# GDMCF/GDMCF

Measured on AMD Instinct MI355X. Metric: training users/sec, higher is better.
Workload: dtype f32; 1 GPU; yelp-shape synthetic rows, batch=400/GPU, dims=[1000], T=5, noise_scale=0.01, linear-var, mean_type=x0, reweight, AdamW lr=1e-5 (BASELINE configs[1]); n_items=34395, global_batch=400, parallelism=dp1, batch_rows=device CSR rows (CsrBatch)

## Files before the change

gdmcf_amd/_lib.py:

```python
import ctypes
import os
import re
from ctypes import c_char_p, c_double, c_float, c_int, c_int64, c_size_t, c_uint64, c_void_p

_HERE = os.path.dirname(os.path.abspath(__file__))
LIB_PATH = os.path.join(_HERE, "csrc", "libgdmcf_hip.so")
HEADER_PATH = os.path.normpath(os.path.join(_HERE, "..", "include", "gdmcf_hip.h"))

P = c_void_p
_CTYPES = {"int": c_int, "int64_t": c_int64, "uint64_t": c_uint64, "size_t": c_size_t, "float": c_float, "double": c_double}


def _uncomment(text):
    return re.sub(r"/\*.*?\*/", " ", text, flags=re.S)


def _code(text):
    return re.sub(r'^[ \t]*(#.*|extern\s+"C"\s*\{|\})[ \t]*$', "", _uncomment(text), flags=re.M)


def _ctype(ctype, where):
    words = re.sub(r"\bconst\b", " ", ctype).replace("*", " * ").split()
    if "*" in words:
        return c_char_p if words == ["char", "*"] else c_void_p
    if " ".join(words) not in _CTYPES:
        raise ImportError(f"gdmcf_hip.h: no ctypes type for '{' '.join(ctype.split())}' in the declaration of {where}")
    return _CTYPES[" ".join(words)]


def _declarator(decl, where):
    m = re.fullmatch(r"\s*(.*[\s*])(\w+)\s*", decl, flags=re.S)
    if not m:
        raise ImportError(f"gdmcf_hip.h: cannot read '{decl.strip()}' in the declaration of {where}")
    return m.groups()


def parse_functions(text):
    code = _code(text)
    out = {}
    for ret, name, params in re.findall(r"([\w\s*]+?)\b(gdmcf_\w+)\s*\(([^()]*)\)\s*;", code):
        params = [] if params.strip() in ("", "void") else params.split(",")
        out[name] = (_ctype(ret, name), [_ctype(_declarator(p, name)[0], name) for p in params])
    mentioned = re.findall(r"(gdmcf_\w+)\s*\(", code)
    if len(mentioned) != len(out):
        raise ImportError(f"gdmcf_hip.h: {len(mentioned)} gdmcf_*( but {len(out)} declarations read; unreadable: "
                          f"{sorted(set(mentioned) - set(out)) or 'none, a name is repeated'}")
    return out


def parse_constants(text):
    text = _uncomment(text)
    out = {n: int(v) for n, v in re.findall(r"^\s*#\s*define\s+(GDMCF_\w+)\s+\(?\s*(-?\d+)\s*\)?\s*$", text, flags=re.M)}
    for body in re.findall(r"\benum\s*\{([^}]*)\}", text):
        for member in filter(str.strip, body.split(",")):
            m = re.fullmatch(r"\s*(\w+)\s*=\s*(-?\d+)\s*", member)
            if not m:
                raise ImportError(f"gdmcf_hip.h: enum member '{member.strip()}' is not `NAME = integer`")
            out[m.group(1)] = int(m.group(2))
    return out


def parse_structs(text):
    out = {}
    for name, body in re.findall(r"\btypedef\s+struct\s+(\w+)\s*\{([^}]*)\}\s*\1\s*;", _code(text)):
        out[name] = []
        for line in filter(str.strip, body.split(";")):
            first, *more = line.split(",")
            ctype, member = _declarator(first, "struct " + name)
            if more and "*" in line:
                raise ImportError(f"gdmcf_hip.h: struct {name}: '{line.strip()}' must declare one pointer member per line")
            out[name] += [(m.strip(), _ctype(ctype, "struct " + name)) for m in [member] + more]
    return out


try:
    with open(HEADER_PATH) as _f:
        _HEADER = _f.read()
except OSError as e:
    raise ImportError(f"{HEADER_PATH} is missing: gdmcf_amd._lib derives its ctypes binding from the C header, which sits "
                      "beside the package in the source tree.") from e
_SIGNATURES = parse_functions(_HEADER)
EXPORTED_SYMBOLS = tuple(_SIGNATURES)
CONSTANTS = parse_constants(_HEADER)
GDMCF_OK, E_SHAPE, E_ARG, E_UNSUPPORTED, E_HIP, E_WORKSPACE, N_TABLES = (
    CONSTANTS["GDMCF_" + n] for n in ("OK", "E_SHAPE", "E_ARG", "E_UNSUPPORTED", "E_HIP", "E_WORKSPACE", "N_TABLES"))
TABLE_NAMES = (
    "betas", "alphas_cumprod", "alphas_cumprod_prev", "alphas_cumprod_next", "sqrt_alphas_cumprod",
    "sqrt_one_minus_alphas_cumprod", "log_one_minus_alphas_cumprod", "sqrt_recip_alphas_cumprod",
    "sqrt_recipm1_alphas_cumprod", "posterior_variance", "posterior_log_variance_clipped",
    "posterior_mean_coef1", "posterior_mean_coef2",
)


class GdDwAdamw(ctypes.Structure):
    _fields_ = parse_structs(_HEADER)["GdDwAdamw"]


class GdKnTail(ctypes.Structure):
    _fields_ = parse_structs(_HEADER)["GdKnTail"]


_lib = None


def load():
    global _lib
    if _lib is not None:
        return _lib
    if not os.path.exists(LIB_PATH):
        raise ImportError(
            f"{LIB_PATH} is missing: build it with `python -m gdmcf_amd.build` (hipcc, gfx950). "
            "gdmcf_amd has no CPU / PyTorch fallback.")
    lib = ctypes.CDLL(LIB_PATH)
    for name, (res, args) in _SIGNATURES.items():
        fn = getattr(lib, name)
        fn.restype = res
        fn.argtypes = args
    if lib.gdmcf_version() != 1:
        raise ImportError("libgdmcf_hip.so ABI version mismatch; rebuild with `python -m gdmcf_amd.build --force`")
    _lib = lib
    return lib


_EXC = {E_SHAPE: AssertionError, E_ARG: ValueError, E_UNSUPPORTED: NotImplementedError, E_HIP: RuntimeError,
        E_WORKSPACE: RuntimeError}


def check(rc):
    if rc != GDMCF_OK:
        msg = load().gdmcf_last_error().decode(errors="replace")
        raise _EXC.get(rc, RuntimeError)(msg or f"gdmcf error {rc}")


def ptr(t):
    return None if t is None else t.data_ptr()


def require_gpu(t, what):
    if not t.is_cuda:
        raise RuntimeError(f"gdmcf_amd: {what} must live on the MI355X (got device '{t.device}'); "
                           "the HIP path has no CPU fallback")


def shadow_info(data_ptr):
    p16 = ctypes.c_void_p()
    rows, cols, ld = ctypes.c_int64(), ctypes.c_int64(), ctypes.c_int64()
    if not load().gdmcf_bf16_shadow_info(data_ptr, ctypes.byref(p16), ctypes.byref(rows), ctypes.byref(cols), ctypes.byref(ld)):
        return None
    return int(p16.value), int(rows.value), int(cols.value), int(ld.value)


def stream_ptr():
    import torch
    return torch.cuda.current_stream().cuda_stream


def philox_randn(shape, device, seed, offset, stream_id=4, out=None):
    import torch
    rows, cols = int(shape[0]), int(shape[1])
    if out is None:
        out = torch.empty(rows, cols, dtype=torch.float32, device=device)
    require_gpu(out, "philox_randn output")
    check(load().gdmcf_randn_f32(out.data_ptr(), out.stride(0), rows, cols, int(stream_id), int(seed) & (2 ** 64 - 1),
                                 int(offset) & (2 ** 64 - 1), stream_ptr()))
    return out


def schedule_tables(kind, noise_scale, noise_min, noise_max, steps, beta_fixed=True):
    import numpy as np
    out = np.zeros((N_TABLES, steps), dtype=np.float64)
    rc = load().gdmcf_schedule_build(kind, float(noise_scale), float(noise_min), float(noise_max), int(steps),
                                     int(bool(beta_fixed)), out.ctypes.data_as(c_void_p))
    check(rc)
    return out


class Bf16Shadow:

    def __init__(self, t, sync=True):
        import weakref

        import torch
        require_gpu(t, "bf16 shadow source")
        if t.dim() != 2 or t.dtype != torch.float32 or t.stride(1) != 1:
            raise RuntimeError("gdmcf_amd: a bf16 shadow needs a 2-D float32 tensor with unit column stride")
        self.rows, self.cols = t.shape
        self.ptr = t.data_ptr()
        self.ld = t.stride(0)
        self.buf = torch.zeros((self.rows + 63) // 64 * 64, (self.cols + 63) // 64 * 64, dtype=torch.bfloat16,
                               device=t.device)
        self._lib = load()
        self._fin = weakref.finalize(self, self._lib.gdmcf_bf16_shadow_clear, self.ptr)
        self.register()
        if sync:
            self.sync()

    def register(self):
        check(self._lib.gdmcf_bf16_shadow_set(self.ptr, self.buf.data_ptr(), self.rows, self.cols, self.buf.stride(0)))

    def unregister(self):
        self._lib.gdmcf_bf16_shadow_clear(self.ptr)

    def sync(self):
        check(self._lib.gdmcf_bf16_shadow_sync(self.ptr, self.ld, stream_ptr()))

    def close(self):
        self._fin()
```

gdmcf_amd/csrc/gemm_dr_kn.hip:

```cpp
#include <stdlib.h>

#include "gemm_dr.h"
#include "tail_job.h"

namespace {

#ifndef GD_KN_EVERY
#define GD_KN_EVERY 4
#endif
template <int NL>
__global__ __launch_bounds__(256, 1) void dr_kn_kernel(const DrArgs d, const GdTailJob job) {
    constexpr int TMB = 5;
    const GdGemm& g = d.g;
    const int lane = threadIdx.x & 63;
    const int wave = __builtin_amdgcn_readfirstlane(threadIdx.x >> 6);
    const int r = lane & 15, q = lane >> 4;
    const int nblk = gridDim.x, per = nblk >> 3;
    const int slot = (nblk & 7) == 0 ? ((int)(blockIdx.x & 7) * per + (int)(blockIdx.x >> 3)) : (int)blockIdx.x;
    const int wl = slot * 4 + wave;
    const int n_waves = nblk * 4;
    const int ntiles = d.tiles_m * d.tiles_n;
    const int CPS = d.ksp;
    const int total_chunks = (g.K + 15) >> 4;
    const int ntasks = ntiles * g.splits;
    if (job.on && slot == (ntasks + 3) >> 2) {
        extern __shared__ __attribute__((aligned(16))) unsigned char kn_lds[];
        gd_tail_job_run(job, kn_lds);
        return;
    }
    const __amdgpu_buffer_rsrc_t srdA = __builtin_amdgcn_make_buffer_rsrc(const_cast<float*>(g.A), 0, (int)(((int64_t)(g.M - 1) * g.lda + g.K) * 4), 0x00020000);
    const __amdgpu_buffer_rsrc_t srdB = __builtin_amdgcn_make_buffer_rsrc(const_cast<float*>(g.B), 0, (int)(((int64_t)(g.K - 1) * g.ldb + g.N) * 4), 0x00020000);
    const uint32_t ldb16 = (uint32_t)g.ldb * 64u;
    for (int task = wl; task < ntasks; task += n_waves) {
        const int split = task / ntiles, tile = task - split * ntiles;
        const int tm = tile % d.tiles_m, tn = tile / d.tiles_m;
        const int m0 = tm * (16 * TMB), n0 = tn * (64 * NL);
        const int c_lo = split * CPS;
        uint32_t offA[TMB], offB[4][NL];
#pragma unroll
        for (int a = 0; a < TMB; ++a) offA[a] = (uint32_t)(((int64_t)min(m0 + 16 * a + r, g.M - 1) * g.lda + 4 * q) * 4);
#pragma unroll
        for (int s = 0; s < 4; ++s)
#pragma unroll
            for (int l = 0; l < NL; ++l) {
                const int n = n0 + 64 * l + 4 * r;
                offB[s][l] = n < g.N ? (uint32_t)(((int64_t)(4 * q + s) * g.ldb + n) * 4) : 0x80000000u;
            }
        f32x4 acc[TMB][NL][4];
#pragma unroll
        for (int a = 0; a < TMB; ++a)
#pragma unroll
            for (int l = 0; l < NL; ++l)
#pragma unroll
                for (int e = 0; e < 4; ++e) acc[a][l][e] = f32x4{0.f, 0.f, 0.f, 0.f};
        f32x4 xa[2][TMB], xb[2][4][NL];
        {
            const uint32_t ka = (uint32_t)c_lo * 64u, kb = (uint32_t)c_lo * ldb16;
#pragma unroll
            for (int a = 0; a < TMB; ++a) xa[0][a] = __builtin_bit_cast(f32x4, __builtin_amdgcn_raw_buffer_load_b128(srdA, offA[a], ka, 0));
#pragma unroll
            for (int s = 0; s < 4; ++s)
#pragma unroll
                for (int l = 0; l < NL; ++l)
                    xb[0][s][l] = __builtin_bit_cast(f32x4, __builtin_amdgcn_raw_buffer_load_b128(srdB, offB[s][l], kb, 0));
        }
#define GD_KN_CHUNK(PAR, c)                                                                                            \
        {                                                                                                              \
            const bool more = (c) + 1 < c_lo + CPS && (c) + 1 < total_chunks;                                          \
            const uint32_t ka = more ? (uint32_t)((c) + 1) * 64u : 0x80000000u;                                        \
            const uint32_t kb = more ? (uint32_t)((c) + 1) * ldb16 : 0x80000000u;                                      \
            if ((c) * 16 + 15 >= g.K) {  \
                _Pragma("unroll") for (int e = 0; e < 4; ++e) {                                                        \
                    const bool keep = (c) * 16 + 4 * q + e < g.K;                                                      \
                    _Pragma("unroll") for (int a = 0; a < TMB; ++a) xa[PAR][a][e] = keep ? xa[PAR][a][e] : 0.f;        \
                }                                                                                                      \
            }                                                                                                          \
                    \
            _Pragma("unroll") for (int a = 0; a < TMB; ++a) asm volatile("" : "+v"(xa[PAR][a]));                       \
            _Pragma("unroll") for (int s = 0; s < 4; ++s)                                                              \
                _Pragma("unroll") for (int l = 0; l < NL; ++l) asm volatile("" : "+v"(xb[PAR][s][l]));                 \
            __builtin_amdgcn_sched_barrier(0);                                                                         \
            _Pragma("unroll") for (int s = 0; s < 4; ++s) {                                                            \
                _Pragma("unroll") for (int n = 0; n < TMB * NL * 4; ++n) {                                             \
                    const int a = n / (NL * 4), l = (n / 4) % NL, e = n % 4;                                           \
                    acc[a][l][e] = __builtin_amdgcn_mfma_f32_16x16x4f32(xa[PAR][a][s], xb[PAR][s][l][e], acc[a][l][e], 0, 0, 0); \
                    const int idx = s * (TMB * NL * 4) + n;                                                            \
                    if (idx % GD_KN_EVERY == 2 && idx / GD_KN_EVERY < TMB + 4 * NL) {                                  \
                        const int ld = idx / GD_KN_EVERY;                                                              \
                        __builtin_amdgcn_sched_barrier(0);                                                             \
                        if (ld < TMB)                                                                                  \
                            xa[(PAR) ^ 1][ld] = __builtin_bit_cast(f32x4, __builtin_amdgcn_raw_buffer_load_b128(srdA, offA[ld], ka, 0)); \
                        else                                                                                           \
                            xb[(PAR) ^ 1][(ld - TMB) / NL][(ld - TMB) % NL] = __builtin_bit_cast(                      \
                                f32x4, __builtin_amdgcn_raw_buffer_load_b128(srdB, offB[(ld - TMB) / NL][(ld - TMB) % NL], kb, 0)); \
                        __builtin_amdgcn_sched_barrier(0);                                                             \
                    }                                                                                                  \
                }                                                                                                      \
                __builtin_amdgcn_sched_barrier(0);                                                                     \
            }                                                                                                          \
        }
        for (int c = c_lo; c < c_lo + CPS && c < total_chunks; c += 2) {
            GD_KN_CHUNK(0, c);
            GD_KN_CHUNK(1, c + 1);
        }
#undef GD_KN_CHUNK
        float* __restrict__ slab = g.C + (int64_t)split * g.slab_stride;
#pragma unroll
        for (int a = 0; a < TMB; ++a)
#pragma unroll
            for (int t = 0; t < 4; ++t) {
                const int m = m0 + 16 * a + 4 * q + t;
                if (m >= g.M) continue;
#pragma unroll
                for (int l = 0; l < NL; ++l) {
                    const int n = n0 + 64 * l + 4 * r;
                    const f32x4 v = {acc[a][l][0][t], acc[a][l][1][t], acc[a][l][2][t], acc[a][l][3][t]};
                    if (n + 3 < g.ldc) {
                        *reinterpret_cast<f32x4*>(slab + (int64_t)m * g.ldc + n) = v;
                    } else {
                        for (int e = 0; e < 4; ++e)
                            if (n + e < g.N) slab[(int64_t)m * g.ldc + n + e] = v[e];
                    }
                }
            }
    }
}

}

int gd_dr_kn_splits(int M, int N, int K) {
    if (!dr_routes().kn || M < 16 || N < 64 || K < 4096) return 0;
    const long tiles = (long)gd_cdiv(M, 80) * gd_cdiv(N, 128);
    if ((long)gd_cdiv(M, 80) * 80 * 100 > (long)M * 112) return 0;
    if ((long)gd_cdiv(N, 128) * 128 * 100 > (long)N * 112) return 0;
    const long slots = 4L * dr_cu_count();
    if (tiles > slots) return 0;
    int splits = (int)(slots / tiles);
    const int total_chunks = gd_cdiv(K, 16);
    if (splits > total_chunks / 8) splits = total_chunks / 8;
    if (splits < 2 || splits > 64) return splits > 64 ? 64 : 0;
    return splits;
}

static bool kn_idle_workgroup(int ntasks, int n_cu) { return gd_cdiv(ntasks, 4) < n_cu; }

#ifndef GD_KN_TAIL_DEFAULT
#define GD_KN_TAIL_DEFAULT 1
#endif

static int kn_launch(GdGemm& g, const GdTailJob* job, hipStream_t s) {
    if (!dr_routes().kn) return GD_DR_NOT_TAKEN;
    const int splits = gd_dr_kn_splits(g.M, g.N, g.K);
    const size_t need = (size_t)splits * g.M * g.ldc * sizeof(float);
    const bool ok = splits > 0 && g.ldc >= g.N && (g.ldc & 3) == 0 && g.ws_cap >= need && g.slab_stride >= (int64_t)g.M * g.ldc &&
                (int64_t)g.M * g.lda * 4 < ((int64_t)1 << 31) && (int64_t)g.K * g.ldb * 4 < ((int64_t)1 << 31) && g.lda >= g.K && g.ldb >= g.N &&
                (reinterpret_cast<uintptr_t>(g.B) & 15) == 0 && (g.ldb & 3) == 0 && (reinterpret_cast<uintptr_t>(g.C) & 15) == 0;
    if (!ok) return GD_DR_NOT_TAKEN;
    DrArgs d = {};
    const int n_cu = dr_cu_count();
    const int total_chunks = gd_cdiv(g.K, 16);
    const int cps = (gd_cdiv(total_chunks, splits) + 1) & ~1;
    const int real_splits = gd_cdiv(total_chunks, cps);
    d.tiles_m = gd_cdiv(g.M, 80);
    d.tiles_n = gd_cdiv(g.N, 128);
    d.ksp = cps;
    GdTailJob none = {};
    size_t lds = 0;
    if (job) {
        const char* env = getenv("GDMCF_KN_TAIL");
        const bool tail_on = env ? atoi(env) != 0 : GD_KN_TAIL_DEFAULT != 0;
        lds = lt_lds_bytes(job->T, job->H, job->B);
        if (!tail_on || !job->on || !kn_idle_workgroup(d.tiles_m * d.tiles_n * real_splits, n_cu) || lds > GD_LT_LDS_MAX)
            return GD_DR_NOT_TAKEN;
        static bool attr_set = false;
        if (!gd_allow_big_lds(dr_kn_kernel<2>, lds, &attr_set, "gemm_dr_kn")) return GDMCF_E_HIP;
    }
    g.splits = real_splits;
    g.kchunk = cps * 16;
    g.tiles_m = d.tiles_m;
    g.tiles_n = d.tiles_n;
    d.g = g;
    {
        GdProfScope prof(g.prof_tag, 2.0 * g.M * g.N * g.K, s);
        hipLaunchKernelGGL((dr_kn_kernel<2>), dim3(n_cu), dim3(256), lds, s, d, job ? *job : none);
    }
    t_gd_last_gemm = 5;
    return gd_launch_status("gemm_dr_kn");
}

int gd_dr_kn_launch(GdGemm& g, hipStream_t s) { return kn_launch(g, nullptr, s); }
int gd_dr_kn_launch_tail(GdGemm& g, const GdTailJob& job, hipStream_t s) { return kn_launch(g, &job, s); }

int gdmcf_debug_kn_tail_rides(int M, int N, int K) {
    const int splits = gd_dr_kn_splits(M, N, K);
    if (splits <= 0) return 0;
    const int total_chunks = gd_cdiv(K, 16);
    const int cps = (gd_cdiv(total_chunks, splits) + 1) & ~1;
    return kn_idle_workgroup(gd_cdiv(M, 80) * gd_cdiv(N, 128) * gd_cdiv(total_chunks, cps), dr_cu_count()) ? 1 : 0;
}
```

gdmcf_amd/csrc/linear.hip:

```cpp
#include <stdlib.h>

#include "common.h"
#include "tail_job.h"

int gd_splitk_reduce(const float* slabs, int64_t slab_stride, int splits, int64_t ld_slab, int M, int N, int mode,
                     const float* bias, const float* rowscale, const float* aact, int64_t ldact, int act, float* out,
                     int64_t ldo, hipStream_t s);
int gd_colsum(const float* dZ, int64_t ld, const float* rs, int M, int N, float* db, hipStream_t s);
int gd_rowpart_reduce(const float* rowpart, int ld, int M, int nt, float* rowsum, hipStream_t s);

namespace {

static const int TARGET_WGS = getenv("GDMCF_TARGET_WGS") ? atoi(getenv("GDMCF_TARGET_WGS")) : 760;

thread_local int t_gemm_prec = GDMCF_GEMM_F32;
thread_local int t_loss_parts = 0;

int pick_class(int M, int N, bool fused, int prec) {
    if (prec == GDMCF_GEMM_BF16 && M > 128) {
        const long pad = (long)gd_cdiv(M, 208) * 208;
        const long tiles = (pad / 208) * gd_cdiv(N, 256);
        const long rounds = (tiles + 255) / 256;
        if (pad * 10 <= (long)M * 11 && pad / 208 <= 2 && (!fused || tiles * 100 >= rounds * 256 * 85)) return 3;
    }
    if (prec == GDMCF_GEMM_F32X3 && M > 128 && N >= 128) {
        const long pad = (long)gd_cdiv(M, 208) * 208;
        if (pad * 10 <= (long)M * 11) return 4;
    }
    return gd_pick_shape_class(M, N);
}

int pick_class_dw(int M, int N, int prec, bool fused_adamw = false) {
    static const int forced = getenv("GDMCF_BF16_DW_CLASS") ? atoi(getenv("GDMCF_BF16_DW_CLASS")) : -1;
    if (prec == GDMCF_GEMM_BF16 && forced >= 0) return forced;
    if (prec == GDMCF_GEMM_BF16 && fused_adamw && M >= 160 && N >= 256) return 0;
    if (prec == GDMCF_GEMM_BF16 && M >= 416 && N >= 512) {
        const long tiles = (long)gd_cdiv(M, 208) * gd_cdiv(N, 256);
        const long rounds = (tiles + 255) / 256;
        if (tiles * 100 >= rounds * 256 * 85) return 3;
    }
    return gd_pick_shape_class(M, N);
}

void attach_result_shadow(GdGemm& g) {
    GdShadow c;
    if (g.bf16 == 1 && gd_shadow_lookup(g.C, &c) && c.rows == g.M && c.cols >= g.N) {
        g.C16 = c.p16;
        g.ldc16 = c.ld16;
    }
}

void attach_shadows(GdGemm& g, int layA, int layB) {
    if (g.bf16 != 1) return;
    GdShadow a, b;
    if (!gd_shadow_lookup(g.A, &a) || !gd_shadow_lookup(g.B, &b)) return;
    const bool okA = layA == GD_LAY_KC ? (a.rows == g.M && a.cols == g.K) : (a.rows == g.K && a.cols == g.M);
    const bool okB = layB == GD_LAY_KC ? (b.rows == g.N && b.cols == g.K) : (b.rows == g.K && b.cols == g.N);
    if (!okA || !okB) return;
    g.A16 = a.p16; g.lda16 = a.ld16;
    g.B16 = b.p16; g.ldb16 = b.ld16;
}

int pick_splits(int M, int N, int K, int cls, int prec) {
    const int bk = prec == GDMCF_GEMM_BF16 ? 64 : 32;
    const int tiles = gd_cdiv(M, gd_gemm_tile_m(cls)) * gd_cdiv(N, gd_gemm_tile_n(cls));
    int s = (cls >= 3 ? 256 : TARGET_WGS) / tiles;
    const int max_by_k = K / (8 * bk);
    if (s > max_by_k) s = max_by_k;
    if (s < 1) s = 1;
    if (s > 64) s = 64;
    return s;
}

inline int64_t round4(int64_t x) { return (x + 3) & ~(int64_t)3; }

float* bias_col_request(int a_scale_col, int64_t lda, const float* rowscale, int K, float* db) {
    static const int on = getenv("GDMCF_BIAS_COL") ? atoi(getenv("GDMCF_BIAS_COL")) : 1;
    if (!on || !a_scale_col || db == nullptr || t_gemm_prec != GDMCF_GEMM_F32 || lda <= K) return nullptr;
    return db;
}

int dw_adamw_setup(const GdDwAdamw& e, GdGemm& g, int& cls) {
    GD_CHECK_SHAPE(e.M > 0 && e.N > 0 && e.K > 0 && e.lddz >= e.N && e.lda >= e.K && e.ldw >= e.K, "linear_bwd_weight_adamw: bad shape");
    GD_CHECK_ARG(e.W && e.exp_avg && e.exp_avg_sq && e.step >= 1, "linear_bwd_weight_adamw: optimizer state missing");
    const int M = e.M, N = e.N, K = e.K;
    cls = pick_class_dw(N, K, t_gemm_prec, true);
    g = GdGemm{};
    g.bf16 = t_gemm_prec;
    g.A = e.dZ; g.lda = e.lddz; g.B = e.A; g.ldb = e.lda; g.M = N; g.N = K; g.K = M; g.splits = 1;
    g.m_fastest = gd_cdiv(N, gd_gemm_tile_m(cls)) <= gd_cdiv(K, gd_gemm_tile_n(cls));
    g.C = e.W; g.ldc = e.ldw; g.aux = e.exp_avg; g.aux2 = e.exp_avg_sq; g.prof_tag = 5;
    g.adam = gd_adam_hyper(e.lr, e.beta1, e.beta2, e.eps, e.weight_decay, e.step, e.grad_scale);
    g.adam_dev = t_gd_step_state ? &t_gd_step_state->hyper : nullptr;
    attach_result_shadow(g);
    attach_shadows(g, GD_LAY_MC, GD_LAY_MC);
    g.out2 = bias_col_request(e.a_scale_col, e.lda, e.rowscale, K, e.db);
    return GDMCF_OK;
}

int dw_adamw_finish(const GdDwAdamw& e, bool asked, const GdGemm& g, hipStream_t s) {
    if (asked && g.out2 == nullptr) return GDMCF_OK;
    if (e.db) return gd_colsum(e.dZ, e.lddz, e.rowscale, e.M, e.N, e.db, s);
    return GDMCF_OK;
}

}

extern "C" {

int gdmcf_gemm_precision(int mode) {
    const int prev = t_gemm_prec;
    if (mode == GDMCF_GEMM_F32 || mode == GDMCF_GEMM_BF16 || mode == GDMCF_GEMM_F32X3) t_gemm_prec = mode;
    return prev;
}

size_t gdmcf_linear_ws_bytes(int M, int N, int K) {
    if (M <= 0 || N <= 0 || K <= 0) return 0;
    size_t need = 0;
    for (int prec = GDMCF_GEMM_F32; prec <= GDMCF_GEMM_F32X3; ++prec) {
        const int cf = pick_class(M, N, false, prec), cb = pick_class(M, K, false, prec);
        size_t f = (size_t)pick_splits(M, N, K, cf, prec) * M * round4(N);
        if (prec == GDMCF_GEMM_F32) {
            const size_t fk = (size_t)gd_dr_kn_splits(M, N, K) * M * round4(N);
            f = f > fk ? f : fk;
            const size_t ff = (size_t)gd_dr_fat_slab_plan(M, N, K, nullptr, nullptr) * M * round4(N);
            f = f > ff ? f : ff;
        }
        size_t b = (size_t)pick_splits(M, K, N, cb, prec) * M * round4(K);
        if (prec == GDMCF_GEMM_F32) {
            const size_t bk = (size_t)gd_dr_kn_splits(M, K, N) * M * round4(K);
            b = b > bk ? b : bk;
        }
        need = need > f ? need : f;
        need = need > b ? need : b;
    }
    return need * sizeof(float) + 256;
}

int gdmcf_debug_fat_slab_plan(int M, int N, int K, int* nb, int* splits, int* cps) {
    int nb_ = 0, cps_ = 0;
    const int sp = (t_gemm_prec == GDMCF_GEMM_F32 && M > 0 && N > 0 && K > 0) ? gd_dr_fat_slab_plan(M, N, K, &nb_, &cps_) : 0;
    if (nb) *nb = nb_;
    if (splits) *splits = sp;
    if (cps) *cps = cps_;
    return sp > 0;
}

int gdmcf_loss_tiles(int N) { return gd_cdiv(N, 16); }

int gdmcf_linear_fwd_f32(const float* A, int64_t lda, const float* W, int64_t ldw, const float* bias, int act, int M,
                         int N, int K, float* C, int64_t ldc, void* ws, size_t ws_bytes, void* stream) {
    GD_CHECK_SHAPE(M > 0 && N > 0 && K > 0 && lda >= K && ldw >= K && ldc >= N, "linear_fwd: bad shape");
    GD_CHECK_ARG(act == 0 || act == 1, "linear_fwd: bad activation");
    hipStream_t s = (hipStream_t)stream;
    const int cls = pick_class(M, N, false, t_gemm_prec);
    const int splits = pick_splits(M, N, K, cls, t_gemm_prec);
    GdGemm g = {};
    g.bf16 = t_gemm_prec;
    g.A = A; g.lda = lda; g.B = W; g.ldb = ldw; g.M = M; g.N = N; g.K = K;
    g.m_fastest = gd_cdiv(M, gd_gemm_tile_m(cls)) <= gd_cdiv(N, gd_gemm_tile_n(cls));
    g.bias = bias; g.act = act; g.prof_tag = 1;
    if (splits == 1) {
        g.splits = 1; g.C = C; g.ldc = ldc;
        attach_result_shadow(g);
        attach_shadows(g, GD_LAY_KC, GD_LAY_KC);
        return gd_gemm_launch(GD_LAY_KC, GD_LAY_KC, GD_EPI_BIAS_ACT, cls, g, s);
    }
    const int64_t lds_ = round4(N);
    const size_t need = (size_t)splits * M * lds_ * sizeof(float);
    if (ws == nullptr || ws_bytes < need) {
        gdmcf_set_error("linear_fwd: workspace %zu < %zu bytes", ws_bytes, need);
        return GDMCF_E_WORKSPACE;
    }
    g.splits = splits; g.C = (float*)ws; g.ldc = lds_; g.slab_stride = (int64_t)M * lds_;
    g.ws_cap = ws_bytes;
    attach_shadows(g, GD_LAY_KC, GD_LAY_KC);
    int rc = gd_gemm_launch(GD_LAY_KC, GD_LAY_KC, GD_EPI_SLAB, cls, g, s);
    if (rc) return rc;
    const int real_splits = gd_cdiv(K, g.kchunk);
    return gd_splitk_reduce((const float*)ws, g.slab_stride, real_splits, lds_, M, N, 0, bias, nullptr, nullptr, 0,
                            act, C, ldc, s);
}

int gdmcf_linear_fwd_wt_f32(const float* A, int64_t lda, const float* Wt, int64_t ldwt, const float* bias, int act, int M, int N,
                            int K, float* C, int64_t ldc, void* ws, size_t ws_bytes, void* stream) {
    GD_CHECK_SHAPE(M > 0 && N > 0 && K > 0 && lda >= K && ldwt >= N && ldc >= N, "linear_fwd_wt: bad shape");
    GD_CHECK_ARG(act == 0 || act == 1, "linear_fwd_wt: bad activation");
    if (t_gemm_prec != GDMCF_GEMM_F32) {
        gdmcf_set_error("linear_fwd_wt: float32 GEMM mode only (the bf16 / f32x3 modes keep the weight in its own orientation)");
        return GDMCF_E_UNSUPPORTED;
    }
    hipStream_t s = (hipStream_t)stream;
    const int cls = pick_class(M, N, false, t_gemm_prec);
    const int splits = pick_splits(M, N, K, cls, t_gemm_prec);
    const int64_t lds_ = round4(N);
    const size_t need = (size_t)splits * M * lds_ * sizeof(float);
    if (ws == nullptr || ws_bytes < need) {
        gdmcf_set_error("linear_fwd_wt: workspace %zu < %zu bytes", ws_bytes, need);
        return GDMCF_E_WORKSPACE;
    }
    GdGemm g = {};
    g.A = A; g.lda = lda; g.B = Wt; g.ldb = ldwt; g.M = M; g.N = N; g.K = K;
    g.m_fastest = gd_cdiv(M, gd_gemm_tile_m(cls)) <= gd_cdiv(N, gd_gemm_tile_n(cls));
    g.splits = splits; g.C = (float*)ws; g.ldc = lds_; g.slab_stride = (int64_t)M * lds_; g.prof_tag = 1;
    g.ws_cap = ws_bytes;
    int rc = gd_gemm_launch(GD_LAY_KC, GD_LAY_MC, GD_EPI_SLAB, cls, g, s);
    if (rc) return rc;
    const int real_splits = gd_cdiv(K, g.kchunk);
    return gd_splitk_reduce((const float*)ws, g.slab_stride, real_splits, lds_, M, N, 0, bias, nullptr, nullptr, 0, act, C, ldc, s);
}

int gdmcf_linear_loss_fwd_f32(const float* A, int64_t lda, const float* W, int64_t ldw, const float* bias,
                              const float* target, int64_t ldt, const float* alpha, int M, int N, int K, float* out,
                              int64_t ldo, float* diff, int64_t ldd, float* rowpart, float* rowsum, void* stream) {
    GD_CHECK_SHAPE(M > 0 && N > 0 && K > 0 && lda >= K && ldw >= K && ldt >= N && ldd >= N, "linear_loss_fwd: bad shape");
    GD_CHECK_SHAPE(out == nullptr || ldo >= N, "linear_loss_fwd: ldo < N");
    hipStream_t s = (hipStream_t)stream;
    const int cls = pick_class(M, N, true, t_gemm_prec);
    GdGemm g = {};
    g.bf16 = t_gemm_prec;
    g.A = A; g.lda = lda; g.B = W; g.ldb = ldw; g.M = M; g.N = N; g.K = K; g.splits = 1;
    g.m_fastest = gd_cdiv(M, gd_gemm_tile_m(cls)) <= gd_cdiv(N, gd_gemm_tile_n(cls));
    g.bias = bias; g.aux = target; g.ldaux = ldt; g.r0 = alpha; g.out2 = out; g.ldout2 = ldo;
    g.prof_tag = 2;
    g.C = diff; g.ldc = ldd; g.rowpart = rowpart; g.ld_rowpart = gdmcf_loss_tiles(N);
    attach_result_shadow(g);
    attach_shadows(g, GD_LAY_KC, GD_LAY_KC);
    int rc = gd_gemm_launch(GD_LAY_KC, GD_LAY_KC, GD_EPI_LOSS, cls, g, s);
    if (rc) return rc;
    t_loss_parts = g.tiles_n;
    if (rowsum == nullptr) return GDMCF_OK;
    return gd_rowpart_reduce(rowpart, g.ld_rowpart, M, g.tiles_n, rowsum, s);
}

int gdmcf_linear_loss_fwd_bits_f32(const float* A, int64_t lda, const float* W, int64_t ldw, const float* bias,
                                   const uint32_t* target_bits, int64_t ldbits, const float* alpha, int M, int N, int K,
                                   float* out, int64_t ldo, float* diff, int64_t ldd, float* rowpart, float* rowsum,
                                   void* stream) {
    GD_CHECK_SHAPE(M > 0 && N > 0 && K > 0 && lda >= K && ldw >= K && ldd >= N, "linear_loss_fwd_bits: bad shape");
    GD_CHECK_SHAPE(out == nullptr || ldo >= N, "linear_loss_fwd_bits: ldo < N");
    GD_CHECK_ARG(target_bits && ldbits >= (N + 31) / 32, "linear_loss_fwd_bits: target bitmap missing / ldbits < ceil(N/32)");
    hipStream_t s = (hipStream_t)stream;
    const int cls = pick_class(M, N, true, t_gemm_prec);
    GdGemm g = {};
    g.bf16 = t_gemm_prec;
    g.A = A; g.lda = lda; g.B = W; g.ldb = ldw; g.M = M; g.N = N; g.K = K; g.splits = 1;
    g.m_fastest = gd_cdiv(M, gd_gemm_tile_m(cls)) <= gd_cdiv(N, gd_gemm_tile_n(cls));
    g.bias = bias; g.aux = nullptr; g.ldaux = 0; g.aux_bits = target_bits; g.ldbits = ldbits; g.r0 = alpha; g.out2 = out;
    g.ldout2 = ldo; g.prof_tag = 2;
    g.C = diff; g.ldc = ldd; g.rowpart = rowpart; g.ld_rowpart = gdmcf_loss_tiles(N);
    attach_result_shadow(g);
    attach_shadows(g, GD_LAY_KC, GD_LAY_KC);
    int rc = gd_gemm_launch(GD_LAY_KC, GD_LAY_KC, GD_EPI_LOSS, cls, g, s);
    if (rc) return rc;
    t_loss_parts = g.tiles_n;
    if (rowsum == nullptr) return GDMCF_OK;
    return gd_rowpart_reduce(rowpart, g.ld_rowpart, M, g.tiles_n, rowsum, s);
}

int gdmcf_linear_posterior_fwd_f32(const float* A, int64_t lda, const float* W, int64_t ldw, const float* bias,
                                   const float* x_t, int64_t ldxt, const float* c1, const float* c2, const float* r1,
                                   const float* r2, const float* sigma, const float* z, int64_t ldz, int M, int N,
                                   int K, float* x_next, int64_t ldxn, float* pred_out, int64_t ldp, void* stream) {
    GD_CHECK_SHAPE(M > 0 && N > 0 && K > 0 && lda >= K && ldw >= K && ldxt >= N && ldxn >= N, "linear_posterior_fwd: bad shape");
    GD_CHECK_ARG(c1 && c2, "linear_posterior_fwd: c1/c2 missing");
    GD_CHECK_ARG((r1 == nullptr) == (r2 == nullptr), "linear_posterior_fwd: r1/r2 must both be set or both NULL");
    GD_CHECK_ARG(z == nullptr || (sigma != nullptr && ldz >= N), "linear_posterior_fwd: sigma missing");
    hipStream_t s = (hipStream_t)stream;
    const int cls = pick_class(M, N, true, t_gemm_prec);
    GdGemm g = {};
    g.bf16 = t_gemm_prec;
    g.A = A; g.lda = lda; g.B = W; g.ldb = ldw; g.M = M; g.N = N; g.K = K; g.splits = 1;
    g.m_fastest = gd_cdiv(M, gd_gemm_tile_m(cls)) <= gd_cdiv(N, gd_gemm_tile_n(cls));
    g.bias = bias; g.aux = x_t; g.ldaux = ldxt; g.aux2 = z; g.ldaux2 = ldz;
    g.r0 = c1; g.r1 = c2; g.r2 = r1; g.r3 = r2; g.r4 = sigma;
    g.out2 = pred_out; g.ldout2 = ldp; g.C = x_next; g.ldc = ldxn; g.prof_tag = 3;
    attach_result_shadow(g);
    attach_shadows(g, GD_LAY_KC, GD_LAY_KC);
    return gd_gemm_launch(GD_LAY_KC, GD_LAY_KC, GD_EPI_POST, cls, g, s);
}

int gdmcf_linear_bwd_input_f32(const float* dZ, int64_t lddz, const float* W, int64_t ldw, const float* rowscale,
                               const float* Aact, int64_t ldact, int act, int M, int N, int K, float* dA,
                               int64_t ldda, void* ws, size_t ws_bytes, void* stream) {
    GD_CHECK_SHAPE(M > 0 && N > 0 && K > 0 && lddz >= N && ldw >= K && ldda >= K, "linear_bwd_input: bad shape");
    GD_CHECK_ARG(act == 0 || (act == 1 && Aact && ldact >= K), "linear_bwd_input: activation output missing");
    hipStream_t s = (hipStream_t)stream;
    const int cls = pick_class(M, K, false, t_gemm_prec);
    const int splits = pick_splits(M, K, N, cls, t_gemm_prec);
    const int64_t lds_ = round4(K);
    const size_t need = (size_t)splits * M * lds_ * sizeof(float);
    if (ws == nullptr || ws_bytes < need) {
        gdmcf_set_error("linear_bwd_input: workspace %zu < %zu bytes", ws_bytes, need);
        return GDMCF_E_WORKSPACE;
    }
    GdGemm g = {};
    g.bf16 = t_gemm_prec;
    g.A = dZ; g.lda = lddz; g.B = W; g.ldb = ldw; g.M = M; g.N = K; g.K = N;
    g.m_fastest = gd_cdiv(M, gd_gemm_tile_m(cls)) <= gd_cdiv(K, gd_gemm_tile_n(cls));
    g.splits = splits; g.C = (float*)ws; g.ldc = lds_; g.slab_stride = (int64_t)M * lds_; g.prof_tag = 4;
    g.ws_cap = ws_bytes;
    attach_shadows(g, GD_LAY_KC, GD_LAY_MC);
    int rc = gd_gemm_launch(GD_LAY_KC, GD_LAY_MC, GD_EPI_SLAB, cls, g, s);
    if (rc) return rc;
    const int real_splits = gd_cdiv(N, g.kchunk);
    return gd_splitk_reduce((const float*)ws, g.slab_stride, real_splits, lds_, M, K, 1, nullptr, rowscale, Aact,
                            ldact, act, dA, ldda, s);
}

int gdmcf_loss_parts_last(void) { return t_loss_parts; }

int gdmcf_kn_tail_run(const GdKnTail* tail, int M, void* stream) {
    GD_CHECK_ARG(tail != nullptr, "kn_tail_run: tail missing");
    const GdKnTail& t = *tail;
    GD_CHECK_SHAPE(M > 0 && t.nt > 0 && t.ld_rowpart >= t.nt, "kn_tail_run: bad shape");
    GD_CHECK_ARG(t.rowpart && t.rowsum, "kn_tail_run: null pointer");
    int rc = gd_rowpart_reduce(t.rowpart, t.ld_rowpart, M, t.nt, t.rowsum, (hipStream_t)stream);
    if (rc) return rc;
    rc = gdmcf_row_loss_finish_mean_f64(t.rowsum, t.rowdiv, t.alpha, t.ts, t.weight_t, t.pt, M, t.T, t.H, t.Lt_history, t.Lt_count,
                                        t.update_history, t.loss_unscaled, t.loss, t.gradcoef, t.loss_mean, t.rowscale_mean, stream);
    if (rc) return rc;
    return gdmcf_rowscale_f32(t.A, t.lda, t.rowscale, M, t.Ka, t.out, t.ldo, stream);
}

int gdmcf_linear_bwd_input_tail_f32(const float* dZ, int64_t lddz, const float* W, int64_t ldw, const float* rowscale,
                                    const float* Aact, int64_t ldact, int act, int M, int N, int K, float* dA, int64_t ldda,
                                    void* ws, size_t ws_bytes, const GdKnTail* tail, void* stream) {
    GD_CHECK_SHAPE(M > 0 && N > 0 && K > 0 && lddz >= N && ldw >= K && ldda >= K, "linear_bwd_input_tail: bad shape");
    GD_CHECK_ARG(act == 0 || (act == 1 && Aact && ldact >= K), "linear_bwd_input_tail: activation output missing");
    GD_CHECK_ARG(tail != nullptr, "linear_bwd_input_tail: tail missing");
    const GdKnTail& t = *tail;
    GD_CHECK_SHAPE(t.nt > 0 && t.ld_rowpart >= t.nt && t.T > 0 && t.H > 0 && t.Ka > 0 && t.lda >= t.Ka && t.ldo >= t.Ka,
                   "linear_bwd_input_tail: bad tail shape");
    GD_CHECK_ARG(t.rowpart && t.rowsum && t.rowdiv && t.ts && t.weight_t && t.pt && t.loss_unscaled && t.loss && t.A && t.rowscale && t.out,
                 "linear_bwd_input_tail: null pointer");
    GD_CHECK_ARG(!t.update_history || (t.Lt_history && t.Lt_count), "linear_bwd_input_tail: update_history without the history");
    GD_CHECK_ARG(!t.rowscale_mean || t.gradcoef, "linear_bwd_input_tail: rowscale_mean needs gradcoef");
    GD_CHECK_ARG(lt_lds_bytes(t.T, t.H, M) <= GD_LT_LDS_MAX, "linear_bwd_input_tail: T*H and B too large for the LDS-resident FIFO update (150 KiB)");
    hipStream_t s = (hipStream_t)stream;
    const int64_t lds_ = round4(K);
    if (t_gemm_prec == GDMCF_GEMM_F32 && ws != nullptr) {
        GdGemm g = {};
        g.A = dZ; g.lda = lddz; g.B = W; g.ldb = ldw; g.M = M; g.N = K; g.K = N;
        g.C = (float*)ws; g.ldc = lds_; g.slab_stride = (int64_t)M * lds_; g.prof_tag = 4;
        g.ws_cap = ws_bytes;
        GdShadow sh;
        const bool has16 = gd_shadow_lookup(t.out, &sh) && sh.rows == M && sh.cols == t.Ka;
        GdTailJob j = {};
        j.on = 1; j.B = M;
        j.rowpart = t.rowpart; j.ld_rowpart = t.ld_rowpart; j.nt = t.nt; j.rowsum = t.rowsum;
        j.rowdiv = t.rowdiv; j.alpha = t.alpha; j.gradcoef = t.gradcoef; j.ts = t.ts; j.weight_t = t.weight_t; j.pt = t.pt;
        j.T = t.T; j.H = t.H; j.update = t.update_history; j.hist = t.Lt_history; j.cnt = t.Lt_count; j.lu = t.loss_unscaled;
        j.loss = t.loss; j.loss_mean = t.loss_mean; j.rowscale_mean = t.rowscale_mean; j.inv_b = 1.0f / (float)M;
        j.K = t.Ka; j.A = t.A; j.lda = t.lda; j.rs = t.rowscale; j.out = t.out; j.ldo = t.ldo;
        j.out16 = has16 ? (unsigned short*)sh.p16 : nullptr; j.ldo16 = has16 ? sh.ld16 : 0; j.bias_col = t.ldo > t.Ka;
        const int rc = gd_dr_kn_launch_tail(g, j, s);
        if (rc != GD_DR_NOT_TAKEN) {
            if (rc) return rc;
            return gd_splitk_reduce((const float*)ws, g.slab_stride, gd_cdiv(N, g.kchunk), lds_, M, K, 1, nullptr, rowscale, Aact, ldact,
                                    act, dA, ldda, s);
        }
    }
    const int rc = gdmcf_kn_tail_run(tail, M, stream);
    if (rc) return rc;
    return gdmcf_linear_bwd_input_f32(dZ, lddz, W, ldw, rowscale, Aact, ldact, act, M, N, K, dA, ldda, ws, ws_bytes, stream);
}

int gdmcf_linear_bwd_weight_f32(const float* dZ, int64_t lddz, const float* A, int64_t lda, const float* rowscale,
                                int a_scale_col, int M, int N, int K, float* dW, int64_t lddw, float* db, int accumulate,
                                void* stream) {
    GD_CHECK_SHAPE(M > 0 && N > 0 && K > 0 && lddz >= N && lda >= K && lddw >= K, "linear_bwd_weight: bad shape");
    hipStream_t s = (hipStream_t)stream;
    const int cls = pick_class_dw(N, K, t_gemm_prec);
    GdGemm g = {};
    g.bf16 = t_gemm_prec;
    g.A = dZ; g.lda = lddz; g.B = A; g.ldb = lda; g.M = N; g.N = K; g.K = M; g.splits = 1;
    g.m_fastest = gd_cdiv(N, gd_gemm_tile_m(cls)) <= gd_cdiv(K, gd_gemm_tile_n(cls));
    g.C = dW; g.ldc = lddw; g.accumulate = accumulate; g.prof_tag = 5;
    attach_shadows(g, GD_LAY_MC, GD_LAY_MC);
    g.out2 = bias_col_request(a_scale_col, lda, rowscale, K, db);
    const bool asked = g.out2 != nullptr;
    int rc = gd_gemm_launch(GD_LAY_MC, GD_LAY_MC, GD_EPI_STORE, cls, g, s);
    if (rc) return rc;
    if (asked && g.out2 == nullptr) return GDMCF_OK;
    if (db) return gd_colsum(dZ, lddz, rowscale, M, N, db, s);
    return GDMCF_OK;
}

int gdmcf_linear_bwd_weight_adamw_f32(const float* dZ, int64_t lddz, const float* A, int64_t lda, const float* rowscale,
                                      int a_scale_col, int M, int N, int K, float* W, int64_t ldw, float* exp_avg, float* exp_avg_sq,
                                      float* db, float lr, float beta1, float beta2, float eps, float weight_decay,
                                      int step, float grad_scale, void* stream) {
    const GdDwAdamw e = {dZ, lddz, A, lda, rowscale, a_scale_col, M, N, K, W, ldw, exp_avg, exp_avg_sq, db,
                         lr, beta1, beta2, eps, weight_decay, step, grad_scale};
    GdGemm g;
    int cls;
    int rc = dw_adamw_setup(e, g, cls);
    if (rc) return rc;
    const bool asked = g.out2 != nullptr;
    rc = gd_gemm_launch(GD_LAY_MC, GD_LAY_MC, GD_EPI_ADAMW, cls, g, (hipStream_t)stream);
    if (rc) return rc;
    return dw_adamw_finish(e, asked, g, (hipStream_t)stream);
}

int gdmcf_linear_bwd_weight_adamw_multi_f32(const GdDwAdamw* list, int n, void* stream) {
    GD_CHECK_ARG(n >= 0 && (n == 0 || list), "linear_bwd_weight_adamw_multi: bad list");
    hipStream_t s = (hipStream_t)stream;
    constexpr int MAXN = 4;
    for (int i0 = 0; i0 < n; i0 += MAXN) {
        const int k = n - i0 < MAXN ? n - i0 : MAXN;
        GdGemm g[MAXN];
        bool asked[MAXN];
        int cls;
        for (int j = 0; j < k; ++j) {
            const int rc = dw_adamw_setup(list[i0 + j], g[j], cls);
            if (rc) return rc;
            asked[j] = g[j].out2 != nullptr;
        }
        int rc = gd_gemm_dr_adamw_multi(g, k, s);
        if (rc == GD_DR_NOT_TAKEN) {
            for (int j = 0; j < k; ++j) {
                const GdDwAdamw& e = list[i0 + j];
                rc = gdmcf_linear_bwd_weight_adamw_f32(e.dZ, e.lddz, e.A, e.lda, e.rowscale, e.a_scale_col, e.M, e.N, e.K, e.W,
                                                       e.ldw, e.exp_avg, e.exp_avg_sq, e.db, e.lr, e.beta1, e.beta2, e.eps,
                                                       e.weight_decay, e.step, e.grad_scale, stream);
                if (rc) return rc;
            }
            continue;
        }
        if (rc) return rc;
        for (int j = 0; j < k; ++j) {
            rc = dw_adamw_finish(list[i0 + j], asked[j], g[j], s);
            if (rc) return rc;
        }
    }
    return GDMCF_OK;
}

}
```

gdmcf_amd/csrc/reduce.hip:

```cpp
#include "tail_job.h"

namespace {

__global__ __launch_bounds__(256) void splitk_reduce_kernel(const float* __restrict__ slabs, int64_t slab_stride,
                                                            int splits, int64_t ld_slab, int M, int N, int mode,
                                                            const float* __restrict__ bias,
                                                            const float* __restrict__ rowscale,
                                                            const float* __restrict__ aact, int64_t ldact, int act,
                                                            float* __restrict__ out, int64_t ldo,
                                                            unsigned short* __restrict__ out16, int64_t ldo16, int vec) {
    const int m = blockIdx.y;
    const int n0 = (blockIdx.x * 256 + threadIdx.x) * 4;
    if (n0 >= N) return;
    float sv[4] = {0.f, 0.f, 0.f, 0.f};
    const float* p = slabs + (int64_t)m * ld_slab + n0;
    if (vec && n0 + 3 < N) {
        for (int k0 = 0; k0 < splits; k0 += 8) {
            f32x4 t[8];
#pragma unroll
            for (int u = 0; u < 8; ++u)
                t[u] = (k0 + u < splits) ? *reinterpret_cast<const f32x4*>(p + (int64_t)(k0 + u) * slab_stride)
                                         : f32x4{0.f, 0.f, 0.f, 0.f};
#pragma unroll
            for (int u = 0; u < 8; ++u)
                if (k0 + u < splits) { sv[0] += t[u].x; sv[1] += t[u].y; sv[2] += t[u].z; sv[3] += t[u].w; }
        }
    } else {
        for (int k = 0; k < splits; ++k)
            for (int j = 0; j < 4; ++j)
                if (n0 + j < N) sv[j] += p[(int64_t)k * slab_stride + j];
    }
    const float rs = (mode != 0 && rowscale) ? rowscale[m] : 1.f;
#pragma unroll
    for (int j = 0; j < 4; ++j) {
        const int n = n0 + j;
        if (n >= N) break;
        float s = sv[j];
        if (mode == 0) {
            if (bias) s += bias[n];
            if (act == 1) s = tanhf(s);
        } else {
            if (rowscale) s *= rs;
            if (act == 1) {
                const float h = aact[(int64_t)m * ldact + n];
                s *= (1.f - h * h);
            }
        }
        out[(int64_t)m * ldo + n] = s;
        if (out16) out16[(int64_t)m * ldo16 + n] = gd_bf16_bits(s);
    }
}

__global__ __launch_bounds__(256) void rowscale_kernel(const float* __restrict__ A, int64_t lda,
                                                       const float* __restrict__ rs, int M, int K,
                                                       float* __restrict__ out, int64_t ldo,
                                                       unsigned short* __restrict__ out16, int64_t ldo16, int bias_col) {
    gd_rowscale_rows<1>(A, lda, rs, M, K, out, ldo, out16, ldo16, bias_col, blockIdx.x, gridDim.x, blockIdx.y, gridDim.y);
}

__global__ __launch_bounds__(256) void colsum_kernel(const float* __restrict__ dZ, int64_t ld,
                                                     const float* __restrict__ rs, int M, int N,
                                                     float* __restrict__ db) {
    __shared__ float part[4][64];
    const int lane = threadIdx.x & 63, wave = threadIdx.x >> 6;
    const int n = blockIdx.x * 64 + lane;
    const int nc = min(n, N - 1);
    float s = 0.f;
    int m = wave;
    for (; m + 28 < M; m += 32) {
        float v[8];
#pragma unroll
        for (int j = 0; j < 8; ++j) v[j] = dZ[(int64_t)(m + 4 * j) * ld + nc] * (rs ? rs[m + 4 * j] : 1.f);
#pragma unroll
        for (int j = 0; j < 8; ++j) s += v[j];
    }
    for (; m < M; m += 4) s += dZ[(int64_t)m * ld + nc] * (rs ? rs[m] : 1.f);
    part[wave][lane] = s;
    __syncthreads();
    if (wave == 0 && n < N) db[n] = ((part[0][lane] + part[1][lane]) + part[2][lane]) + part[3][lane];
}

__global__ __launch_bounds__(256) void rowpart_reduce_kernel(const float* __restrict__ rowpart, int ld, int M, int nt,
                                                             float* __restrict__ rowsum) {
    gd_rowpart_reduce_rows<1>(rowpart, ld, M, nt, rowsum, blockIdx.x, gridDim.x);
}

typedef __bf16 gd_bf16x2 __attribute__((ext_vector_type(2)));
__device__ __forceinline__ unsigned gd_pack_bf16(float lo, float hi) {
    gd_bf16x2 v;
    v[0] = (__bf16)lo;
    v[1] = (__bf16)hi;
    return __builtin_bit_cast(unsigned, v);
}
typedef unsigned int gd_u32x4 __attribute__((ext_vector_type(4)));

__global__ __launch_bounds__(256) void cast_bf16_kernel(const float* __restrict__ src, int64_t ld, unsigned short* __restrict__ dst,
                                                        int64_t ld16, int64_t rows, int64_t cols) {
    const int64_t groups = (cols + 7) / 8;
    const int64_t total = rows * groups;
    for (int64_t u = (int64_t)blockIdx.x * blockDim.x + threadIdx.x; u < total; u += (int64_t)gridDim.x * blockDim.x) {
        const int64_t r = u / groups, c = (u - r * groups) * 8;
        const float* p = src + r * ld + c;
        float e[8];
#pragma unroll
        for (int i = 0; i < 8; ++i) e[i] = (c + i < cols) ? p[i] : 0.f;
        gd_u32x4 w;
        w.x = gd_pack_bf16(e[0], e[1]);
        w.y = gd_pack_bf16(e[2], e[3]);
        w.z = gd_pack_bf16(e[4], e[5]);
        w.w = gd_pack_bf16(e[6], e[7]);
        *reinterpret_cast<gd_u32x4*>(dst + r * ld16 + c) = w;
    }
}
}

extern "C" {

int gdmcf_rowscale_f32(const float* A, int64_t lda, const float* rowscale, int M, int K, float* out, int64_t ldo,
                       void* stream) {
    GD_CHECK_SHAPE(M > 0 && K > 0 && lda >= K && ldo >= K, "rowscale: bad shape");
    GdShadow sh;
    const bool has16 = gd_shadow_lookup(out, &sh) && sh.rows == M && sh.cols == K;
    const int bias_col = ldo > K;
    hipLaunchKernelGGL(rowscale_kernel, dim3(gd_cdiv(K, 1024), M), dim3(256), 0, (hipStream_t)stream, A, lda,
                       rowscale, M, K, out, ldo, has16 ? (unsigned short*)sh.p16 : nullptr, has16 ? sh.ld16 : 0, bias_col);
    return gd_launch_status("rowscale");
}

}

int gd_splitk_reduce(const float* slabs, int64_t slab_stride, int splits, int64_t ld_slab, int M, int N, int mode,
                     const float* bias, const float* rowscale, const float* aact, int64_t ldact, int act, float* out,
                     int64_t ldo, hipStream_t s) {
    GdShadow sh;
    const bool has16 = gd_shadow_lookup(out, &sh) && sh.rows == M && sh.cols == N;
    const int vec = (ld_slab % 4 == 0) && (slab_stride % 4 == 0) && gd_aligned16(slabs);
    hipLaunchKernelGGL(splitk_reduce_kernel, dim3(gd_cdiv(N, 1024), M), dim3(256), 0, s, slabs, slab_stride,
                       splits, ld_slab, M, N, mode, bias, rowscale, aact, ldact, act, out, ldo,
                       has16 ? (unsigned short*)sh.p16 : nullptr, has16 ? sh.ld16 : 0, vec);
    return gd_launch_status("splitk_reduce");
}

int gd_colsum(const float* dZ, int64_t ld, const float* rs, int M, int N, float* db, hipStream_t s) {
    hipLaunchKernelGGL(colsum_kernel, dim3(gd_cdiv(N, 64)), dim3(256), 0, s, dZ, ld, rs, M, N, db);
    return gd_launch_status("colsum");
}

int gd_rowpart_reduce(const float* rowpart, int ld, int M, int nt, float* rowsum, hipStream_t s) {
    hipLaunchKernelGGL(rowpart_reduce_kernel, dim3(gd_cdiv(M, 4)), dim3(256), 0, s, rowpart, ld, M, nt, rowsum);
    return gd_launch_status("rowpart_reduce");
}

int gd_cast_bf16(const float* src, int64_t ld, void* dst, int64_t ld16, int64_t rows, int64_t cols, hipStream_t s) {
    const int64_t total = rows * ((cols + 7) / 8);
    const int64_t blocks = (total + 255) / 256;
    hipLaunchKernelGGL(cast_bf16_kernel, dim3((unsigned)(blocks < 16384 ? blocks : 16384)), dim3(256), 0, s, src, ld,
                       (unsigned short*)dst, ld16, rows, cols);
    return gd_launch_status("cast_bf16");
}
```

gdmcf_amd/csrc/rows.hip:

```cpp
#include "common.h"

namespace {

__device__ __forceinline__ float block_sum_256(float v, float* red) {
#pragma unroll
    for (int o = 32; o > 0; o >>= 1) v += __shfl_down(v, o, 64);
    __syncthreads();
    if ((threadIdx.x & 63) == 0) red[threadIdx.x >> 6] = v;
    __syncthreads();
    return red[0] + red[1] + red[2] + red[3];
}

__global__ __launch_bounds__(256) void row_norms_kernel(const float* __restrict__ X, int64_t ld, int cols,
                                                       float* __restrict__ norm, float* __restrict__ inv_norm) {
    __shared__ float red[4];
    const float* x = X + (int64_t)blockIdx.x * ld;
    float ss = 0.f;
    const int c4 = cols & ~3;
    for (int c = threadIdx.x * 4; c < c4; c += 1024) {
        const f32x4 t = *reinterpret_cast<const f32x4_u4*>(x + c);
        ss += t.x * t.x + t.y * t.y + t.z * t.z + t.w * t.w;
    }
    if (threadIdx.x < cols - c4) ss += x[c4 + threadIdx.x] * x[c4 + threadIdx.x];
    const float n = sqrtf(block_sum_256(ss, red));
    if (threadIdx.x == 0) {
        if (norm) norm[blockIdx.x] = n;
        if (inv_norm) inv_norm[blockIdx.x] = 1.f / n;
    }
}

template <bool ADAM_>
__global__ __launch_bounds__(256) void normalize_rows_bwd_kernel(const float* __restrict__ dY, int64_t lddy,
                                                                const float* __restrict__ Y, int64_t ldy,
                                                                const float* __restrict__ inv_norm, int cols,
                                                                float* __restrict__ dX, int64_t lddx,
                                                                float* __restrict__ exp_avg, float* __restrict__ exp_avg_sq,
                                                                GdAdamHyper h, const GdStepState* step_state) {
    __shared__ float red[4];
    if (ADAM_ && step_state) h = step_state->hyper;
    const float* dy = dY + (int64_t)blockIdx.x * lddy;
    const float* y = Y + (int64_t)blockIdx.x * ldy;
    float* dx = dX + (int64_t)blockIdx.x * lddx;
    float* mr = ADAM_ ? exp_avg + (int64_t)blockIdx.x * lddx : nullptr;
    float* vr = ADAM_ ? exp_avg_sq + (int64_t)blockIdx.x * lddx : nullptr;
    const float rn = inv_norm[blockIdx.x];
    if (cols <= 4096 && (cols & 3) == 0) {
        f32x4 a[4], b[4];
        float dot = 0.f;
#pragma unroll
        for (int k = 0; k < 4; ++k) {
            const int c = (threadIdx.x + 256 * k) * 4;
            a[k] = b[k] = f32x4{0.f, 0.f, 0.f, 0.f};
            if (c < cols) {
                a[k] = *reinterpret_cast<const f32x4_u4*>(dy + c);
                b[k] = *reinterpret_cast<const f32x4_u4*>(y + c);
            }
            dot += a[k].x * b[k].x + a[k].y * b[k].y + a[k].z * b[k].z + a[k].w * b[k].w;
        }
        dot = block_sum_256(dot, red);
#pragma unroll
        for (int k = 0; k < 4; ++k) {
            const int c = (threadIdx.x + 256 * k) * 4;
            if (c >= cols) continue;
            const f32x4 g = (a[k] - b[k] * dot) * rn;
            if (!ADAM_) {
                *reinterpret_cast<f32x4_u4*>(dx + c) = g;
                continue;
            }
            f32x4 pp = *reinterpret_cast<const f32x4_u4*>(dx + c);
            f32x4 mm = *reinterpret_cast<const f32x4_u4*>(mr + c);
            f32x4 vv = *reinterpret_cast<const f32x4_u4*>(vr + c);
#pragma unroll
            for (int j = 0; j < 4; ++j) {
                float pj = pp[j], mj = mm[j], vj = vv[j];
                gd_adam_elem(pj, g[j], mj, vj, h);
                pp[j] = pj;
                mm[j] = mj;
                vv[j] = vj;
            }
            *reinterpret_cast<f32x4_u4*>(dx + c) = pp;
            *reinterpret_cast<f32x4_u4*>(mr + c) = mm;
            *reinterpret_cast<f32x4_u4*>(vr + c) = vv;
        }
        return;
    }
    float dot = 0.f;
    for (int c = threadIdx.x; c < cols; c += 256) dot += dy[c] * y[c];
    dot = block_sum_256(dot, red);
    for (int c = threadIdx.x; c < cols; c += 256) {
        const float g = (dy[c] - y[c] * dot) * rn;
        if (ADAM_)
            gd_adam_elem(dx[c], g, mr[c], vr[c], h);
        else
            dx[c] = g;
    }
}

__global__ __launch_bounds__(256) void tanh_bwd_kernel(const float* __restrict__ dA, int64_t ldd, const float* __restrict__ A,
                                                      int64_t lda, const float* __restrict__ extra, int64_t lde,
                                                      const float* __restrict__ scale, int N, float* __restrict__ out,
                                                      int64_t ldo) {
    const int m = blockIdx.y, n = blockIdx.x * 256 + threadIdx.x;
    if (n >= N) return;
    float g = dA[(int64_t)m * ldd + n];
    if (extra) g += scale[0] * extra[(int64_t)m * lde + n];
    const float a = A[(int64_t)m * lda + n];
    out[(int64_t)m * ldo + n] = g * (1.f - a * a);
}

__global__ __launch_bounds__(256) void gather_rows_kernel(const float* __restrict__ src, int64_t lds,
                                                         const int64_t* __restrict__ index, int cols,
                                                         float* __restrict__ dst, int64_t ldd) {
    const float* s = src + index[blockIdx.x] * lds;
    float* d = dst + (int64_t)blockIdx.x * ldd;
    for (int c = threadIdx.x; c < cols; c += 256) d[c] = s[c];
}

__global__ __launch_bounds__(256) void scatter_add_rows_kernel(const float* __restrict__ src, int64_t lds,
                                                              const int64_t* __restrict__ index, int cols,
                                                              float* __restrict__ dst, int64_t ldd) {
    const float* s = src + (int64_t)blockIdx.x * lds;
    float* d = dst + index[blockIdx.x] * ldd;
    for (int c = threadIdx.x; c < cols; c += 256) atomicAdd(d + c, s[c]);
}

constexpr int SCATTER_ADAM_ROWS = 16;

__global__ __launch_bounds__(256) void scatter_rows_adamw_kernel(const float* __restrict__ src, int64_t lds,
                                                                const int64_t* __restrict__ index, int n, int rows, int cols,
                                                                float* __restrict__ W, int64_t ldw, float* __restrict__ exp_avg,
                                                                float* __restrict__ exp_avg_sq, GdAdamHyper h,
                                                                const GdStepState* step_state) {
    __shared__ int slot[SCATTER_ADAM_ROWS];
    if (step_state) h = step_state->hyper;
    const int64_t r0 = (int64_t)blockIdx.x * SCATTER_ADAM_ROWS;
    if (threadIdx.x < SCATTER_ADAM_ROWS) slot[threadIdx.x] = -1;
    __syncthreads();
    for (int j = threadIdx.x; j < n; j += 256) {
        const int64_t r = index[j] - r0;
        if (r >= 0 && r < SCATTER_ADAM_ROWS) slot[r] = j;
    }
    __syncthreads();
    const int nr = (int)min((int64_t)SCATTER_ADAM_ROWS, rows - r0);
    const bool vec = ((cols | ldw | lds) & 3) == 0 &&
                     ((reinterpret_cast<uintptr_t>(W) | reinterpret_cast<uintptr_t>(exp_avg) |
                       reinterpret_cast<uintptr_t>(exp_avg_sq) | reinterpret_cast<uintptr_t>(src)) & 15u) == 0;
    if (vec) {
        const int c4 = cols >> 2;
        for (int it = threadIdx.x; it < nr * c4; it += 256) {
            const int rr = it / c4, c = (it - rr * c4) * 4;
            const int j = slot[rr];
            const int64_t o = (r0 + rr) * ldw + c;
            f32x4 gg = {0.f, 0.f, 0.f, 0.f};
            if (j >= 0) gg = gg + *reinterpret_cast<const f32x4*>(src + (int64_t)j * lds + c);
            f32x4 pp = __builtin_nontemporal_load(reinterpret_cast<f32x4*>(W + o));
            f32x4 mm = __builtin_nontemporal_load(reinterpret_cast<f32x4*>(exp_avg + o));
            f32x4 vv = __builtin_nontemporal_load(reinterpret_cast<f32x4*>(exp_avg_sq + o));
#pragma unroll
            for (int q = 0; q < 4; ++q) {
                float pq = pp[q], mq = mm[q], vq = vv[q];
                gd_adam_elem(pq, gg[q], mq, vq, h);
                pp[q] = pq;
                mm[q] = mq;
                vv[q] = vq;
            }
            __builtin_nontemporal_store(pp, reinterpret_cast<f32x4*>(W + o));
            __builtin_nontemporal_store(mm, reinterpret_cast<f32x4*>(exp_avg + o));
            __builtin_nontemporal_store(vv, reinterpret_cast<f32x4*>(exp_avg_sq + o));
        }
        return;
    }
    for (int it = threadIdx.x; it < nr * cols; it += 256) {
        const int rr = it / cols, c = it - rr * cols;
        const int j = slot[rr];
        const int64_t o = (r0 + rr) * ldw + c;
        float g = 0.f;
        if (j >= 0) g = g + src[(int64_t)j * lds + c];
        gd_adam_elem(W[o], g, exp_avg[o], exp_avg_sq[o], h);
    }
}

__global__ __launch_bounds__(256) void emb_gather_w_kernel(const float* __restrict__ W1, int64_t ldw, int I, int E, int N,
                                                           float* __restrict__ W1e) {
    const int idx = blockIdx.x * 256 + threadIdx.x;
    if (idx < N * E) W1e[idx] = W1[(int64_t)(idx / E) * ldw + I + (idx % E)];
}

__global__ __launch_bounds__(256) void emb_bwd_demb_kernel(const float* __restrict__ dZ1, int64_t lddz,
                                                           const float* __restrict__ W1e, int E, int N,
                                                           float* __restrict__ demb) {
    const int m = blockIdx.x;
    const int lane = threadIdx.x & 63, wave = threadIdx.x >> 6;
    for (int e = wave; e < E; e += 4) {
        float s = 0.f;
        for (int n = lane; n < N; n += 64) s += dZ1[(int64_t)m * lddz + n] * W1e[(int64_t)n * E + e];
        for (int o = 32; o > 0; o >>= 1) s += __shfl_xor(s, o);
        if (lane == 0) demb[(int64_t)m * E + e] = s;
    }
}

__global__ __launch_bounds__(64) void emb_bwd_w_kernel(const float* __restrict__ demb, const float* __restrict__ temb,
                                                       int M, int E, float* __restrict__ dWe,
                                                       float* __restrict__ dbe) {
    const int idx = blockIdx.x, lane = threadIdx.x;
    float s = 0.f;
    if (idx < E * E) {
        const int e = idx / E, f = idx % E;
        for (int m = lane; m < M; m += 64) s += demb[(int64_t)m * E + e] * temb[(int64_t)m * E + f];
    } else {
        const int e = idx - E * E;
        for (int m = lane; m < M; m += 64) s += demb[(int64_t)m * E + e];
    }
    for (int o = 32; o > 0; o >>= 1) s += __shfl_xor(s, o);
    if (lane == 0) {
        if (idx < E * E) dWe[idx] = s;
        else dbe[idx - E * E] = s;
    }
}

__global__ __launch_bounds__(256) void densify_rows_kernel(const int64_t* __restrict__ indptr,
                                                           const int32_t* __restrict__ indices,
                                                           const float* __restrict__ values,
                                                           const int64_t* __restrict__ row_ids, int I,
                                                           float* __restrict__ out, int64_t ldo) {
    const int b = blockIdx.x;
    float* row = out + (int64_t)b * ldo;
    const bool al = ((reinterpret_cast<uintptr_t>(row) & 15u) == 0);
    if (al) {
        for (int i = threadIdx.x * 4; i + 3 < I; i += 1024) *reinterpret_cast<f32x4*>(row + i) = f32x4{0.f, 0.f, 0.f, 0.f};
        for (int i = (I & ~3) + threadIdx.x; i < I; i += 256) row[i] = 0.f;
    } else {
        for (int i = threadIdx.x; i < I; i += 256) row[i] = 0.f;
    }
    __syncthreads();
    const int64_t u = row_ids ? row_ids[b] : b;
    for (int64_t j = indptr[u] + threadIdx.x; j < indptr[u + 1]; j += 256) {
        const int c = indices[j];
        if (c >= 0 && c < I) row[c] = values ? values[j] : 1.f;
    }
}

__global__ __launch_bounds__(256) void scale_kernel(const float* __restrict__ a, int64_t n, float s,
                                                    float* __restrict__ out) {
    const int64_t i = (int64_t)blockIdx.x * 256 + threadIdx.x;
    if (i < n) out[i] = a[i] * s;
}

}

extern "C" {

int gdmcf_row_norms_f32(const float* X, int64_t ld, int rows, int cols, float* norm, float* inv_norm, void* stream) {
    GD_CHECK_SHAPE(rows > 0 && cols > 0 && ld >= cols, "row_norms: bad shape");
    GD_CHECK_ARG(X && (norm || inv_norm), "row_norms: null pointer");
    hipLaunchKernelGGL(row_norms_kernel, dim3(rows), dim3(256), 0, (hipStream_t)stream, X, ld, cols, norm, inv_norm);
    return gd_launch_status("row_norms");
}

int gdmcf_normalize_rows_bwd_f32(const float* dY, int64_t lddy, const float* Y, int64_t ldy, const float* inv_norm, int rows,
                                 int cols, float* dX, int64_t lddx, void* stream) {
    GD_CHECK_SHAPE(rows > 0 && cols > 0 && lddy >= cols && ldy >= cols && lddx >= cols, "normalize_rows_bwd: bad shape");
    GD_CHECK_ARG(dY && Y && inv_norm && dX, "normalize_rows_bwd: null pointer");
    hipLaunchKernelGGL(normalize_rows_bwd_kernel<false>, dim3(rows), dim3(256), 0, (hipStream_t)stream, dY, lddy, Y, ldy,
                       inv_norm, cols, dX, lddx, nullptr, nullptr, GdAdamHyper{}, nullptr);
    return gd_launch_status("normalize_rows_bwd");
}

int gdmcf_normalize_rows_bwd_adamw_f32(const float* dY, int64_t lddy, const float* Y, int64_t ldy, const float* inv_norm,
                                       int rows, int cols, float* X, int64_t ldx, float* exp_avg, float* exp_avg_sq, float lr,
                                       float beta1, float beta2, float eps, float weight_decay, int step, float grad_scale,
                                       void* stream) {
    GD_CHECK_SHAPE(rows > 0 && cols > 0 && lddy >= cols && ldy >= cols && ldx >= cols, "normalize_rows_bwd_adamw: bad shape");
    GD_CHECK_ARG(dY && Y && inv_norm && X && exp_avg && exp_avg_sq && step >= 1, "normalize_rows_bwd_adamw: null pointer");
    const GdAdamHyper h = gd_adam_hyper(lr, beta1, beta2, eps, weight_decay, step, grad_scale);
    {
        GdProfScope prof(6, 32.0 * (double)rows * cols, (hipStream_t)stream);
        hipLaunchKernelGGL(normalize_rows_bwd_kernel<true>, dim3(rows), dim3(256), 0, (hipStream_t)stream, dY, lddy, Y, ldy,
                           inv_norm, cols, X, ldx, exp_avg, exp_avg_sq, h, t_gd_step_state);
    }
    return gd_launch_status("normalize_rows_bwd_adamw");
}

int gdmcf_tanh_bwd_f32(const float* dA, int64_t ldd, const float* A, int64_t lda, const float* extra, int64_t lde,
                       const float* scale, int M, int N, float* out, int64_t ldo, void* stream) {
    GD_CHECK_SHAPE(M > 0 && N > 0 && ldd >= N && lda >= N && ldo >= N && (!extra || lde >= N), "tanh_bwd: bad shape");
    GD_CHECK_ARG(dA && A && out && (!extra || scale), "tanh_bwd: null pointer");
    hipLaunchKernelGGL(tanh_bwd_kernel, dim3(gd_cdiv(N, 256), M), dim3(256), 0, (hipStream_t)stream, dA, ldd, A, lda, extra, lde,
                       scale, N, out, ldo);
    return gd_launch_status("tanh_bwd");
}

int gdmcf_gather_rows_f32(const float* src, int64_t lds, const int64_t* index, int n, int cols, float* dst, int64_t ldd,
                          void* stream) {
    GD_CHECK_SHAPE(n > 0 && cols > 0 && lds >= cols && ldd >= cols, "gather_rows: bad shape");
    GD_CHECK_ARG(src && index && dst, "gather_rows: null pointer");
    hipLaunchKernelGGL(gather_rows_kernel, dim3(n), dim3(256), 0, (hipStream_t)stream, src, lds, index, cols, dst, ldd);
    return gd_launch_status("gather_rows");
}

int gdmcf_scatter_add_rows_f32(const float* src, int64_t lds, const int64_t* index, int n, int cols, float* dst, int64_t ldd,
                               void* stream) {
    GD_CHECK_SHAPE(n > 0 && cols > 0 && lds >= cols && ldd >= cols, "scatter_add_rows: bad shape");
    GD_CHECK_ARG(src && index && dst, "scatter_add_rows: null pointer");
    hipLaunchKernelGGL(scatter_add_rows_kernel, dim3(n), dim3(256), 0, (hipStream_t)stream, src, lds, index, cols, dst, ldd);
    return gd_launch_status("scatter_add_rows");
}

int gdmcf_scatter_rows_adamw_f32(const float* src, int64_t lds, const int64_t* index, int n, int rows, int cols, float* W,
                                 int64_t ldw, float* exp_avg, float* exp_avg_sq, float lr, float beta1, float beta2, float eps,
                                 float weight_decay, int step, float grad_scale, void* stream) {
    GD_CHECK_SHAPE(n >= 0 && rows > 0 && cols > 0 && ldw >= cols && (n == 0 || lds >= cols), "scatter_rows_adamw: bad shape");
    GD_CHECK_ARG(W && exp_avg && exp_avg_sq && (n == 0 || (src && index)) && step >= 1, "scatter_rows_adamw: null pointer");
    const GdAdamHyper h = gd_adam_hyper(lr, beta1, beta2, eps, weight_decay, step, grad_scale);
    {
        GdProfScope prof(6, 24.0 * (double)rows * cols, (hipStream_t)stream);
        hipLaunchKernelGGL(scatter_rows_adamw_kernel, dim3(gd_cdiv(rows, SCATTER_ADAM_ROWS)), dim3(256), 0, (hipStream_t)stream,
                           src, lds, index, n, rows, cols, W, ldw, exp_avg, exp_avg_sq, h, t_gd_step_state);
    }
    return gd_launch_status("scatter_rows_adamw");
}

int gdmcf_emb_bwd_f32(const float* dZ1, int64_t lddz, const float* W1, int64_t ldw, int I, int E, const float* temb,
                      int M, int N, float* demb_ws, float* dWe, float* dbe, void* stream) {
    GD_CHECK_SHAPE(M > 0 && N > 0 && E > 0 && I >= 0 && ldw >= I + E && lddz >= N, "emb_bwd: bad shape");
    GD_CHECK_ARG(dZ1 && W1 && temb && demb_ws && dWe && dbe, "emb_bwd: null pointer");
    hipStream_t s = (hipStream_t)stream;
    float* W1e = demb_ws + (size_t)M * E;
    hipLaunchKernelGGL(emb_gather_w_kernel, dim3(gd_cdiv(N * E, 256)), dim3(256), 0, s, W1, ldw, I, E, N, W1e);
    hipLaunchKernelGGL(emb_bwd_demb_kernel, dim3(M), dim3(256), 0, s, dZ1, lddz, W1e, E, N, demb_ws);
    hipLaunchKernelGGL(emb_bwd_w_kernel, dim3(E * E + E), dim3(64), 0, s, demb_ws, temb, M, E, dWe, dbe);
    return gd_launch_status("emb_bwd");
}

int gdmcf_densify_rows_f32(const int64_t* indptr, const int32_t* indices, const float* values, const int64_t* row_ids,
                           int B, int I, float* out, int64_t ldo, void* stream) {
    GD_CHECK_SHAPE(B > 0 && I > 0 && ldo >= I, "densify_rows: bad shape");
    GD_CHECK_ARG(indptr && indices && out, "densify_rows: null pointer");
    hipLaunchKernelGGL(densify_rows_kernel, dim3(B), dim3(256), 0, (hipStream_t)stream, indptr, indices, values, row_ids,
                       I, out, ldo);
    return gd_launch_status("densify_rows");
}

int gdmcf_scale_f32(const float* acc, int64_t n, float scale, float* out, void* stream) {
    GD_CHECK_SHAPE(n > 0, "scale: empty");
    GD_CHECK_ARG(acc && out, "scale: null pointer");
    hipLaunchKernelGGL(scale_kernel, dim3((unsigned)((n + 255) / 256)), dim3(256), 0, (hipStream_t)stream, acc, n,
                       scale, out);
    return gd_launch_status("scale");
}

}
```

gdmcf_amd/csrc/tail_job.h:

```cpp
#pragma once

#include "common.h"

namespace {

template <int U>
__device__ __forceinline__ void gd_rowpart_reduce_rows(const float* __restrict__ rowpart, int ld, int M, int nt,
                                                       float* __restrict__ rowsum, int blk, int nblk) {
    const int lane = threadIdx.x & 63, step = nblk * 4;
    for (int m0 = blk * 4 + (int)(threadIdx.x >> 6); m0 < M; m0 += step * U) {
        float s[U];
#pragma unroll
        for (int u = 0; u < U; ++u) s[u] = 0.f;
        for (int j = lane; j < nt; j += 64) {
#pragma unroll
            for (int u = 0; u < U; ++u) s[u] += rowpart[(int64_t)min(m0 + u * step, M - 1) * ld + j];
        }
#pragma unroll
        for (int u = 0; u < U; ++u) {
            for (int o = 32; o > 0; o >>= 1) s[u] += __shfl_xor(s[u], o);
            if (lane == 0 && m0 + u * step < M) rowsum[m0 + u * step] = s[u];
        }
    }
}

template <int U>
__device__ __forceinline__ void gd_rowscale_rows(const float* __restrict__ A, int64_t lda, const float* __restrict__ rs, int M, int K,
                                                 float* __restrict__ out, int64_t ldo, unsigned short* __restrict__ out16,
                                                 int64_t ldo16, int bias_col, int bx, int nbx, int by, int nby) {
    for (int kb = bx; kb * 1024 < K; kb += nbx) {
        const int k = (kb * 256 + (int)threadIdx.x) * 4;
        for (int m0 = by; m0 < M; m0 += nby * U) {
            float r[U];
            f32x4 t[U];
#pragma unroll
            for (int u = 0; u < U; ++u) {
                const int m = min(m0 + u * nby, M - 1);
                r[u] = rs[m];
                const float* a = A + (int64_t)m * lda + k;
                if (k + 3 < K) {
                    t[u] = *reinterpret_cast<const f32x4_u4*>(a);
                } else {
                    for (int j = 0; j < 4; ++j) t[u][j] = k + j < K ? a[j] : 0.f;
                }
            }
#pragma unroll
            for (int u = 0; u < U; ++u) {
                const int m = m0 + u * nby;
                if (m >= M) break;
                if (bias_col && kb == 0 && threadIdx.x == 0) out[(int64_t)m * ldo + K] = r[u];
                if (k >= K) continue;
                float* o = out + (int64_t)m * ldo + k;
                const float v[4] = {t[u].x * r[u], t[u].y * r[u], t[u].z * r[u], t[u].w * r[u]};
                if (k + 3 < K) {
                    *reinterpret_cast<f32x4_u4*>(o) = f32x4{v[0], v[1], v[2], v[3]};
                } else {
                    for (int j = 0; j < 4; ++j)
                        if (k + j < K) o[j] = v[j];
                }
                if (out16)
                    for (int j = 0; j < 4; ++j)
                        if (k + j < K) out16[(int64_t)m * ldo16 + k + j] = gd_bf16_bits(v[j]);
            }
        }
    }
}

__device__ __forceinline__ void lt_history_parallel(const int64_t* __restrict__ ts, const double* __restrict__ lu, int B, int T, int H,
                                                    double* hist, int64_t* cnt, unsigned char* lds_raw) {
    double* old = reinterpret_cast<double*>(lds_raw);
    int* n_t = reinterpret_cast<int*>(old + (size_t)T * H);
    int* c0 = n_t + T;
    int* tsl = c0 + T;
    const int tid = threadIdx.x, nth = blockDim.x;
    for (int i = tid; i < T * H; i += nth) old[i] = hist[i];
    for (int t = tid; t < T; t += nth) {
        n_t[t] = 0;
        c0[t] = (int)cnt[t];
    }
    for (int b = tid; b < B; b += nth) tsl[b] = (int)ts[b];
    __syncthreads();
    for (int b = tid; b < B; b += nth) atomicAdd(&n_t[tsl[b]], 1);
    __syncthreads();
    for (int i = tid; i < T * H; i += nth) {
        const int t = i / H, j = i % H;
        const int drop = max(0, c0[t] + n_t[t] - H);
        if (j < c0[t] && j - drop >= 0) hist[(int64_t)t * H + (j - drop)] = old[i];
    }
    for (int b = tid; b < B; b += nth) {
        const int t = tsl[b];
        int rank = 0;
        for (int p = 0; p < b; ++p) rank += (tsl[p] == t);
        const int drop = max(0, c0[t] + n_t[t] - H);
        const int pos = c0[t] + rank - drop;
        if (pos >= 0) hist[(int64_t)t * H + pos] = lu[b];
    }
    for (int t = tid; t < T; t += nth) cnt[t] = (int64_t)min(H, c0[t] + n_t[t]);
}

__device__ __forceinline__ void gd_row_loss_finish_block(const float* __restrict__ rowsum, const float* __restrict__ rowdiv,
                                                         const float* __restrict__ alpha, float* __restrict__ gradcoef,
                                                         const int64_t* __restrict__ ts, const double* __restrict__ weight_t,
                                                         const double* __restrict__ pt, int B, int T, int H, double* hist,
                                                         int64_t* cnt, int update, double* __restrict__ lu, double* __restrict__ loss,
                                                         double* __restrict__ loss_mean, float* __restrict__ rowscale_mean,
                                                         float inv_b, unsigned char* fin_lds) {
    double part = 0.0;
    for (int b = threadIdx.x; b < B; b += 256) {
        const float mse = rowsum[b] / rowdiv[b];
        const double l = weight_t[ts[b]] * (double)mse;
        lu[b] = l;
        const double lb = l / pt[b];
        loss[b] = lb;
        part += lb;
        if (gradcoef) {
            const float gc = (float)(2.0 * (alpha ? (double)alpha[b] : 1.0) * weight_t[ts[b]] / (pt[b] * (double)rowdiv[b]));
            gradcoef[b] = gc;
            if (rowscale_mean) rowscale_mean[b] = gc * inv_b;
        }
    }
    if (loss_mean) {
        double* s_part = reinterpret_cast<double*>(fin_lds);
        for (int o = 32; o > 0; o >>= 1) part += __shfl_xor(part, o);
        if ((threadIdx.x & 63) == 0) s_part[threadIdx.x >> 6] = part;
        __syncthreads();
        if (threadIdx.x == 0) *loss_mean = (((s_part[0] + s_part[1]) + s_part[2]) + s_part[3]) / (double)B;
    }
    __syncthreads();
    if (update) lt_history_parallel(ts, lu, B, T, H, hist, cnt, fin_lds);
}

}

struct GdTailJob {
    int on;
    int B;
    const float* rowpart;
    int ld_rowpart, nt;
    float* rowsum;
    const float* rowdiv;
    const float* alpha;
    float* gradcoef;
    const int64_t* ts;
    const double* weight_t;
    const double* pt;
    int T, H, update;
    double* hist;
    int64_t* cnt;
    double* lu;
    double* loss;
    double* loss_mean;
    float* rowscale_mean;
    float inv_b;
    int K;
    const float* A;
    int64_t lda;
    const float* rs;
    float* out;
    int64_t ldo;
    unsigned short* out16;
    int64_t ldo16;
    int bias_col;
};

namespace {

__device__ __forceinline__ void gd_tail_job_run(const GdTailJob& j, unsigned char* lds) {
    gd_rowpart_reduce_rows<8>(j.rowpart, j.ld_rowpart, j.B, j.nt, j.rowsum, 0, 1);
    __syncthreads();
    gd_row_loss_finish_block(j.rowsum, j.rowdiv, j.alpha, j.gradcoef, j.ts, j.weight_t, j.pt, j.B, j.T, j.H, j.hist, j.cnt, j.update,
                             j.lu, j.loss, j.loss_mean, j.rowscale_mean, j.inv_b, lds);
    __syncthreads();
    gd_rowscale_rows<8>(j.A, j.lda, j.rs, j.B, j.K, j.out, j.ldo, j.out16, j.ldo16, j.bias_col, 0, 1, 0, 1);
}

inline size_t lt_lds_bytes(int T, int H, int B) { return (size_t)T * H * 8 + (size_t)T * 8 + (size_t)B * 4 + 16; }
constexpr size_t GD_LT_LDS_MAX = 150 * 1024;

template <class K>
bool gd_allow_big_lds(K* kernel, size_t lds, bool* done, const char* who) {
    if (*done || lds <= 48 * 1024) return true;
    *done = hipFuncSetAttribute(reinterpret_cast<const void*>(kernel), hipFuncAttributeMaxDynamicSharedMemorySize, 160 * 1024) == hipSuccess;
    if (!*done) gdmcf_set_error("%s: hipFuncSetAttribute failed", who);
    return *done;
}

}

int gd_dr_kn_launch_tail(GdGemm& g, const GdTailJob& job, hipStream_t s);
```

gdmcf_amd/engine.py:

```python

import ctypes
import os

import torch

from . import _lib
from . import engine_core as core
from .engine_core import EngineBase, _Bufs, _ceil64, with_precision


class DenoiserEngine(EngineBase):
    def __init__(self, model):
        super().__init__(model)
        self._wshadow = {}
        self.input_grad_first = False
        self.weight_waiters = {}
        self.static_grads = False
        self._grad_bufs = {}
        self._gemm_side = os.environ.get("GDMCF_GEMM_SIDE", "0") == "1"
        self._side2 = None
        self._side2_used = False
        self._wt_on = os.environ.get("GDMCF_FWD_WT", "1") == "1"
        self.defer_tail = False
        self._pending_tail = None

    def _grad_like(self, p):
        if not self.static_grads:
            return torch.empty_like(p)
        g = self._grad_bufs.get(id(p))
        if g is None or g.shape != p.shape or g.device != p.device:
            g = self._grad_bufs[id(p)] = torch.empty_like(p)
        return g

    def _use_weight(self, w):
        fn = self.weight_waiters.pop(id(w), None) if self.weight_waiters else None
        if fn is not None:
            fn()
            rec = self._wshadow.get(id(w))
            if rec is not None and rec[1] != w._version:
                rec[0].sync()
                rec[1] = w._version

    def flush_weight_waiters(self):
        self._flush_tail()
        while self.weight_waiters:
            self.weight_waiters.popitem()[1]()

    def _defers_tail(self, spec, layers, B):
        if not self.defer_tail or type(self) is not DenoiserEngine or self.gemm_dtype != "f32" or spec["eps_mode"]:
            return False
        if (self.grad_sink is not None and not self.input_grad_first) or len(layers) < 2:
            return False
        n, k = layers[-1][0].shape
        return bool(self.lib.gdmcf_debug_kn_tail_rides(B, k, n))

    def _flush_tail(self):
        pend, self._pending_tail = self._pending_tail, None
        if pend is not None:
            core.tail_job_run(self.lib, pend[0], pend[1], _lib.stream_ptr())

    def _shadows_on(self, bufs, layers):
        if self.gemm_dtype != "bf16":
            if bufs.shadows is not None:
                for sh in bufs.shadows:
                    sh.close()
                bufs.shadows = None
                bufs.sh_xin2 = None
            for sh, _ in self._wshadow.values():
                sh.close()
            self._wshadow = {}
            return
        if bufs.shadows is None:
            I, E = self.I, self.E
            mk = lambda t, cols: _lib.Bf16Shadow(t[:, :cols], sync=False)
            sh = [mk(bufs.xin, I + E), mk(bufs.diff, I)]
            for (w, _, _), a, d in zip(layers[:-1], bufs.acts, bufs.dzs):
                sh += [mk(a, w.shape[0]), mk(d, w.shape[0])]
            sh.append(mk(bufs.hs, layers[-1][0].shape[1]))
            bufs.shadows = sh
            bufs.sh_xin = sh[0]
        live = {id(w) for w, _, _ in layers}
        for key in [k for k in self._wshadow if k not in live]:
            self._wshadow.pop(key)[0].close()
        for w, _, _ in layers:
            rec = self._wshadow.get(id(w))
            if rec is None or rec[0].ptr != w.data_ptr():
                self._use_weight(w)
                if rec is not None:
                    rec[0].close()
                self._wshadow[id(w)] = [_lib.Bf16Shadow(w.detach()), w._version]
            elif id(w) in self.weight_waiters:
                continue
            elif rec[1] != w._version:
                rec[0].sync()
                rec[1] = w._version

    def _layers(self):
        layers = self.model.layer_list()
        self._check_params(layers)
        return layers

    def buffers(self, B, device):
        key = (B, str(device))
        b = self._bufs.get(key)
        if b is not None:
            return b
        layers = self.model.layer_list()
        f32 = dict(dtype=torch.float32, device=device)
        b = _Bufs()
        b.ldk = _ceil64(self.I + self.E)
        b.xin = torch.zeros(B, b.ldk, **f32)
        b.xin2 = None
        b.acts = [torch.zeros(B, _ceil64(w.shape[0]), **f32) for (w, _, _) in layers[:-1]]
        b.dzs = [torch.zeros(B, _ceil64(w.shape[0]), **f32) for (w, _, _) in layers[:-1]]
        b.hs = torch.zeros(B, _ceil64(layers[-1][0].shape[1]), **f32)
        b.shadows = None
        self._shared_buffers(b, B, device, layers[-1][0].shape[0], layers[0][0].shape[0], [w for w, _, _ in layers])
        self._bufs[key] = b
        return b

    def _prep(self, bufs, x, ts, ca, cb, noise, drop_mask, training, xt_out=None, xin=None):
        xin = bufs.xin if xin is None else xin
        keepalive = self._prep_input(bufs, x, self.I, xin, ts, ca, cb, noise, drop_mask, training, xt_out=xt_out)
        if xin is bufs.xin:
            bufs.xin_ones = True
        return keepalive

    def _train_input(self, bufs, spec, xt_out):
        return self._prep(bufs, spec["x_start"], spec["ts"], spec["ca"], spec["cb"], spec["noise"], spec["drop_mask"],
                          self.model.training, xt_out=xt_out)

    def _prep_csr(self, bufs, batch, ts, ca, cb, noise, drop_mask, training):
        m = self.model
        B, I = batch.shape
        if getattr(bufs, "x0bits", None) is None:
            bufs.x0bits = torch.zeros(B, (I + 31) // 32, dtype=torch.int32, device=batch.device)
        self.offset += 1
        keepalive = core.prep_input_csr(self.lib, batch, ts, ca, cb, noise, drop_mask, float(m.drop.p), training, self.seed,
                                        self.offset, m.emb_layer, self.E, bufs.xin, bufs.temb, bufs.x0bits, _lib.stream_ptr())
        bufs.xin_ones = True
        return keepalive

    def _train_input_csr(self, bufs, spec):
        return self._prep_csr(bufs, spec["csr"], spec["ts"], spec["ca"], spec["cb"], spec["noise"], spec["drop_mask"],
                              self.model.training)

    def _hidden_forward(self, bufs, layers, B, xin=None, frozen=False, csr=None):
        lib, st = self.lib, _lib.stream_ptr()
        A = bufs.xin if xin is None else xin
        for li, (w, bias, act) in enumerate(layers[:-1]):
            N, K = w.shape
            out = bufs.acts[li]
            self._use_weight(w)
            if li == 0 and csr is not None:
                self._gather_first_layer(bufs, csr, w, bias, act, A, B, out, st)
            elif frozen and self._wt_on and self.gemm_dtype == "f32" and K >= 4096 and w.numel() >= (1 << 20):
                wt = self._transposed(w)
                _lib.check(lib.gdmcf_linear_fwd_wt_f32(A.data_ptr(), A.stride(0), wt.data_ptr(), wt.stride(0), bias.data_ptr(), act, B, N, K,
                                                       out.data_ptr(), out.stride(0), bufs.ws.data_ptr(), bufs.ws_bytes, st))
            else:
                core.linear_fwd(lib, bufs, A, w, bias, act, B, N, K, out, st)
            A = out
        return A

    @with_precision
    def train_forward(self, spec):
        self._flush_tail()
        x0, ts = spec["x_start"], spec["ts"]
        csr = spec.get("csr")
        B, dev = (csr.shape[0], csr.device) if csr is not None else (x0.shape[0], x0.device)
        layers = self._layers()
        bufs = self.buffers(B, dev)
        self._shadows_on(bufs, layers)
        lib, st = self.lib, _lib.stream_ptr()
        self.version += 1
        eps_mode = spec["eps_mode"]
        xt_out = None
        if eps_mode:
            if bufs.xt is None:
                bufs.xt = torch.zeros(B, bufs.ldi, dtype=torch.float32, device=dev)
            xt_out = bufs.xt
        if csr is not None:
            keepalive = self._train_input_csr(bufs, spec)
        else:
            keepalive = self._train_input(bufs, spec, xt_out)
        x0c = keepalive[0]
        alpha = None
        if eps_mode:
            target, alpha, rowdiv = self._eps_target(bufs, spec, ts, x0c, keepalive[1])
        else:
            target = x0c
            rowdiv = bufs.rowdiv_mse
        A = self._hidden_forward(bufs, layers, B)
        w, bias, _ = layers[-1]
        N, K = w.shape
        self._use_weight(w)
        defer = self._defers_tail(spec, layers, B)
        if csr is not None:
            nt = core.loss_layer_bits(lib, bufs, A, w, bias, bufs.x0bits, None, B, N, K, st, reduce=not defer)
        else:
            nt = core.loss_layer(lib, bufs, A, w, bias, target, alpha, B, N, K, st, reduce=not defer)
        tail = None
        if defer:
            loss, self.last_loss_mean, tail = core.loss_tail_job(lib, bufs, spec, B, rowdiv, alpha, nt, A, K)
            self._pending_tail = (tail, B)
        else:
            loss, self.last_loss_mean = core.loss_tail(lib, bufs, spec, B, rowdiv, alpha, st, mean=True)
        self._saved = dict(kind="train", B=B, bufs=bufs, layers=layers, tail=tail,
                           keepalive=(keepalive, target, alpha, rowdiv, spec["pt"]))
        return loss

    @with_precision
    def train_backward(self, gloss):
        sv = self._saved
        if sv is None or sv.get("kind") != "train":
            raise RuntimeError("gdmcf_amd: train_backward without a preceding training_losses")
        bufs = sv["bufs"]
        tail = sv.get("tail")
        if tail is not None and self._pending_tail is not None and self._pending_tail[0] is tail:
            if isinstance(gloss, float) and gloss == 1.0 / sv["B"]:
                self._pending_tail = None
                return self._backward(sv, bufs.diff, bufs.rowscale_mean, tail=tail)
            self._flush_tail()
        if isinstance(gloss, float) and gloss == 1.0 / sv["B"] and getattr(bufs, "rowscale_mean", None) is not None:
            rowscale = bufs.rowscale_mean
        else:
            rowscale = self._rowscale_of(bufs, gloss)
        return self._backward(sv, bufs.diff, rowscale)

    @with_precision
    def forward_plain(self, x, timesteps, training, drop_mask=None):
        self.flush_weight_waiters()
        B, dev = x.shape[0], x.device
        layers = self._layers()
        bufs = self.buffers(B, dev)
        self._shadows_on(bufs, layers)
        lib, st = self.lib, _lib.stream_ptr()
        self.version += 1
        ts = timesteps.to(device=dev, dtype=torch.int64).contiguous()
        keepalive = self._prep(bufs, x, ts, None, None, None, drop_mask, training)
        A = self._hidden_forward(bufs, layers, B)
        w, bias, act = layers[-1]
        N, K = w.shape
        out = torch.empty(B, N, dtype=torch.float32, device=dev)
        core.linear_fwd(lib, bufs, A, w, bias, act, B, N, K, out, st)
        self._saved = dict(kind="plain", B=B, bufs=bufs, layers=layers, keepalive=(keepalive, ts))
        return out

    @with_precision
    def backward_plain(self, gout):
        sv = self._saved
        g = gout.to(torch.float32)
        if g.stride(-1) != 1:
            g = g.contiguous()
        return self._backward(sv, g, None)

    def _backward(self, sv, dz_last, rowscale, tail=None):
        lib, st = self.lib, _lib.stream_ptr()
        bufs, layers, B = sv["bufs"], sv["layers"], sv["B"]
        m = self.model
        L = len(layers)
        grads_w = [None] * L
        grads_b = [None] * L
        dWe = dbe = None
        fused = self.fused_opt if self.grad_sink is None else None
        dz, rs = dz_last, rowscale
        dw_queue = [] if (fused is not None and self.gemm_dtype == "f32" and os.environ.get("GDMCF_DW_MULTI", "1") != "0") else None

        def input_grad(li, w, A_prev):
            nonlocal dWe, dbe
            N, K = w.shape
            if li > 0:
                dprev = bufs.dzs[li - 1]
                if tail is not None and li == L - 1:
                    core.linear_bwd_input_tail(lib, bufs, dz, w, rs, A_prev, layers[li - 1][2], B, N, K, dprev, tail, st)
                else:
                    self._input_grad(bufs, B, w, N, K, dz, rs, A_prev, layers[li - 1][2], dprev, st)
                return dprev
            dWe = self._grad_like(m.emb_layer.weight)
            dbe = self._grad_like(m.emb_layer.bias)
            core.emb_bwd(lib, bufs, dz, w, self.I, self.E, B, N, dWe, dbe, st)
            return None

        def weight_grad(li, w, bias, A_prev):
            db = self._grad_like(bias)
            scol = int(rs is None and li == 0 and getattr(bufs, "xin_ones", False) and A_prev.stride(0) > w.shape[1])
            if tail is not None and li == L - 1:
                A_use, scol = bufs.hs, int(bufs.hs.stride(0) > w.shape[1])
            else:
                A_use, scol = self._row_scaled(bufs, B, w.shape[1], A_prev, rs, scol, st)
            fs = fused.fused_state(w) if fused is not None else None
            dW = self._grad_like(w) if fs is None else None
            if fs is None and self._gemm_side and self.grad_sink is None and li == L - 1 and L > 1:
                if self._side2 is None:
                    self._side2 = torch.cuda.Stream()
                self._side2.wait_stream(torch.cuda.current_stream())
                with torch.cuda.stream(self._side2):
                    self._weight_grad(bufs, B, w, dz, rs, A_use, scol, dW, db, None, _lib.stream_ptr())
                self._side2_used = True
            else:
                self._weight_grad(bufs, B, w, dz, rs, A_use, scol, dW, db, fs, st, queue=dw_queue)
            grads_w[li], grads_b[li] = dW, db
            if self.grad_sink is not None:
                self.grad_sink(w, dW)
                self.grad_sink(bias, db)
                grads_w[li] = grads_b[li] = None

        for li in range(L - 1, -1, -1):
            w, bias, _ = layers[li]
            A_prev = bufs.acts[li - 1] if li > 0 else bufs.xin
            if fused is not None or self.input_grad_first or (tail is not None and li == L - 1):
                nxt = input_grad(li, w, A_prev)
                weight_grad(li, w, bias, A_prev)
            else:
                weight_grad(li, w, bias, A_prev)
                nxt = input_grad(li, w, A_prev)
            dz, rs = nxt, None
        if dw_queue:
            arr = (_lib.GdDwAdamw * len(dw_queue))(*[e for e, _ in dw_queue])
            _lib.check(lib.gdmcf_linear_bwd_weight_adamw_multi_f32(ctypes.addressof(arr), len(dw_queue), st))
            for _, w in dw_queue:
                torch.autograd.graph.increment_version(w)
        if self._side2_used:
            torch.cuda.current_stream().wait_stream(self._side2)
            self._side2_used = False
        if self.grad_sink is not None:
            self.grad_sink(m.emb_layer.weight, dWe)
            self.grad_sink(m.emb_layer.bias, dbe)
            dWe = dbe = None
        out = [dWe, dbe]
        for li in range(L):
            out += [grads_w[li], grads_b[li]]
        return out

    @with_precision
    def p_sample_loop(self, x_start, steps, T, tabs32, eps_mode, sampling_noise, noise0=None, step_noise=None,
                      capture=None, draw_noise=None, latent=False, stop=False, eps=None):
        m, lib = self.model, self.lib
        if draw_noise is None:
            def draw_noise(like):
                self.offset += 1
                return _lib.philox_randn(like.shape, like.device, self.seed, self.offset, 7)
        self.flush_weight_waiters()
        B, dev, I = x_start.shape[0], x_start.device, self.I
        from .data_utils import CsrBatch
        csr = x_start if isinstance(x_start, CsrBatch) else None
        if csr is not None and (steps != 0 or m.norm or self.gemm_dtype != "f32" or csr.csr.values is not None):
            raise RuntimeError("gdmcf_amd: the reverse loop takes CSR rows only for steps == 0, binary rows, norm=False and "
                               "float32 products (GaussianDiffusion.p_sample densifies the rest)")
        layers = self._layers()
        bufs = self.buffers(B, dev)
        self._shadows_on(bufs, layers)
        st = _lib.stream_ptr()
        self.version += 1
        if latent:
            if (eps_mode and eps is None) or sampling_noise or capture is not None or m.norm or self.gemm_dtype != "f32":
                raise RuntimeError("gdmcf_amd: the latent reverse loop takes the x0 target without sampling noise, capture or "
                                   "F.normalize, in float32 products (GaussianDiffusion._latent_reverse_ok)")
            return self._latent_loop(bufs, layers, x_start, csr, steps, T, tabs32, noise0, stop=stop, eps=eps if eps_mode else None)
        if bufs.xin2 is None:
            bufs.xin2 = torch.zeros_like(bufs.xin)
        if self.gemm_dtype == "bf16" and getattr(bufs, "sh_xin2", None) is None:
            bufs.sh_xin2 = _lib.Bf16Shadow(bufs.xin2[:, : I + self.E], sync=False)
            bufs.shadows.append(bufs.sh_xin2)
        norm = bool(m.norm)
        keep = []
        t_vec = torch.full((B,), max(steps - 1, 0), dtype=torch.int64, device=dev)
        ca = cb = None
        if steps > 0:
            ca, cb = tabs32["sqrt_ab"], tabs32["sqrt_1mab"]
        w, bias, _ = layers[-1]
        N, K = w.shape
        out = None

        stabs = core.step_tables(tabs32, T, B, ("c1", "c2", "r1", "r2", "sigma"), bufs.tab_cache)
        if getattr(bufs, "step_ts", None) is None or bufs.step_ts.shape[0] != T:
            bufs.step_ts = torch.arange(T, dtype=torch.int64, device=dev)[:, None].expand(T, B).contiguous()
        step_ts = bufs.step_ts

        def posterior(i, n, A, xt, xn):
            c1, c2 = stabs["c1"][i], stabs["c2"][i]
            r1 = r2 = sg = z = None
            if eps_mode:
                r1, r2 = stabs["r1"][i], stabs["r2"][i]
            if sampling_noise and i != 0:
                sg = stabs["sigma"][i]
                z = step_noise[n] if step_noise is not None else draw_noise(xt[:, :I])
                z = z.contiguous()
            pred = torch.empty(B, I, dtype=torch.float32, device=dev) if capture is not None else None
            core.posterior_fwd(lib, A, w, bias, xt, c1, c2, r1, r2, sg, z, B, N, K, xn, pred, st)
            keep.append((c1, c2, r1, r2, sg, z))
            if capture is not None:
                capture.setdefault("pred_xstart", []).append(pred)
                capture.setdefault("mean", []).append(xn[:, :I].clone())

        if not norm:
            cur, nxt = bufs.xin, bufs.xin2
            if csr is not None:
                keep.append(self._prep_csr(bufs, csr, t_vec, None, None, None, None, False))
            else:
                keep.append(self._prep(bufs, x_start, t_vec, ca, cb, noise0, None, False, xin=cur))
            bufs.xin_ones = False
            for n, i in enumerate(range(T - 1, -1, -1)):
                ts = step_ts[i]
                _lib.check(lib.gdmcf_dnn_emb_cols_f32(ts.data_ptr(), m.emb_layer.weight.data_ptr(),
                                                      m.emb_layer.bias.data_ptr(), self.E, B, I, cur.data_ptr(),
                                                      cur.stride(0), bufs.temb.data_ptr(), st))
                keep.append(ts)
                A = self._hidden_forward(bufs, layers, B, xin=cur, frozen=True, csr=csr if n == 0 else None)
                out = torch.empty(B, I, dtype=torch.float32, device=dev) if i == 0 else None
                posterior(i, n, A, cur, out if out is not None else nxt)
                cur, nxt = nxt, cur
        else:
            if bufs.xt is None:
                bufs.xt = torch.zeros(B, bufs.ldi, dtype=torch.float32, device=dev)
            xt = bufs.xt
            keep.append(self._prep(bufs, x_start, t_vec, ca, cb, noise0, None, False, xt_out=xt, xin=bufs.xin2))
            for n, i in enumerate(range(T - 1, -1, -1)):
                ts = step_ts[i]
                keep.append(self._prep(bufs, xt[:, :I], ts, None, None, None, None, False, xin=bufs.xin))
                A = self._hidden_forward(bufs, layers, B, xin=bufs.xin, frozen=True)
                out = torch.empty(B, I, dtype=torch.float32, device=dev) if i == 0 else None
                xn = out if out is not None else (bufs.diff if xt is bufs.xt else bufs.xt)
                posterior(i, n, A, xt, xn)
                xt = xn
        self._saved = None
        del keep
        return out

    def _latent_begin(self, bufs, layers, T, B, tabs32):
        for wl, _, _ in layers:
            self._use_weight(wl)
        (w1, b1, _), (w, bias, _), emb = layers[0], layers[-1], self.model.emb_layer
        ops = self._latent_operands(w1, b1, w, w.shape[1], bias, T, (w1, b1, w, bias, emb.weight, emb.bias))
        ld = _ceil64(w1.shape[0])
        if getattr(bufs, "lat_p", None) is None:
            bufs.lat_p = torch.zeros(B, ld, dtype=torch.float32, device=w1.device)
            bufs.lat_h = torch.zeros_like(bufs.lat_p)
        return ops, core.step_tables(tabs32, T, B, ("c1", "c2"), bufs.tab_cache), bufs.lat_p, ld

    def _latent_run(self, bufs, layers, ops, tabs, T, B, pre, p, e, x_T, **kw):
        (_, _, act1), (w, bias, _), lib, st = layers[0], layers[-1], self.lib, _lib.stream_ptr()

        def middle(n, i, A):
            for li in range(1, len(layers) - 1):
                wl, bl, al = layers[li]
                core.linear_fwd(lib, bufs, A, wl, bl, al, B, wl.shape[0], wl.shape[1], bufs.acts[li], st)
                A = bufs.acts[li]
            return A

        return self._latent_reverse(bufs, ops, T, B, w.shape[1], act1, pre, p, (bufs.acts[0], bufs.lat_h),
                                    middle if len(layers) > 2 else None, e, tabs["c1"], tabs["c2"], w, bias, x_T, **kw)

    def _latent_loop(self, bufs, layers, x_start, csr, steps, T, tabs32, noise0, stop=False, eps=None):
        lib, st, I = self.lib, _lib.stream_ptr(), self.I
        B, dev = x_start.shape[0], x_start.device
        w1 = layers[0][0]
        h1 = w1.shape[0]
        ops, tabs, p, _ = self._latent_begin(bufs, layers, T, B, tabs32)
        t_vec = torch.full((B,), max(steps - 1, 0), dtype=torch.int64, device=dev)
        if csr is not None:
            if stop:
                keep, self.offset = None, self.offset + 1
            else:
                keep = self._prep_csr(bufs, csr, t_vec, None, None, None, None, False)
            wt = self._transposed(w1)
            core.gather_fwd(lib, None, None, csr, wt, I, None, None, 0, None, 0, B, h1, p, st)
        else:
            ca, cb = (tabs32["sqrt_ab"], tabs32["sqrt_1mab"]) if steps > 0 else (None, None)
            keep = self._prep(bufs, x_start, t_vec, ca, cb, noise0, None, False, xin=bufs.xin)
            core.linear_fwd(lib, bufs, (bufs.xin.data_ptr(), bufs.xin.stride(0)), w1, None, 0, B, h1, I, p, st)
        bufs.xin_ones = False
        x0 = self._latent_run(bufs, layers, ops, tabs, T, B, p, p, ops.e, bufs.xin, stop=stop, eps=eps)
        self._saved = None
        del keep
        return x0
```

gdmcf_amd/engine_core.py:

```python
import collections
import ctypes
import functools

import torch

from . import _lib


def _ceil64(n):
    return (int(n) + 63) // 64 * 64


class _Bufs:
    pass


_GEMM_MODES = {k: _lib.CONSTANTS["GDMCF_GEMM_" + k.upper()] for k in ("f32", "bf16", "f32x3")}


def with_precision(fn):
    @functools.wraps(fn)
    def wrapped(self, *a, **kw):
        prev = self.lib.gdmcf_gemm_precision(_GEMM_MODES[self.gemm_dtype])
        try:
            return fn(self, *a, **kw)
        finally:
            self.lib.gdmcf_gemm_precision(prev)
    return wrapped


def _pl(a):
    if type(a) is tuple:
        return a
    return (None, 0) if a is None else (a.data_ptr(), a.stride(0))


def _f32_rows(t):
    return t if t.dtype == torch.float32 and t.stride(-1) == 1 else t.float().contiguous()


def _prep_modes(B, ca, noise, drop_mask, drop_p, training):
    noise_mode = 0
    if ca is not None:
        noise_mode = 1 if noise is not None else 2
        if noise is not None:
            noise = _f32_rows(noise)
    drop_mode, keep = 0, None
    if drop_mask is not None:
        drop_mode = 1
        keep = drop_mask.reshape(B, -1)
        keep = (keep if keep.dtype == torch.uint8 else (keep != 0).to(torch.uint8)).contiguous()
    elif training and drop_p > 0.0:
        drop_mode = 2
    return noise_mode, noise, drop_mode, keep


def prep_input(lib, x, I, ts, ca, cb, noise, drop_mask, drop_p, training, seed, offset, norm, emb, E, xin, xt_out, temb,
               rownorm, st):
    B = x.shape[0]
    x = _f32_rows(x)
    noise_mode, noise, drop_mode, keep = _prep_modes(B, ca, noise, drop_mask, drop_p, training)
    (nz, ldn), (kp, ldkp), (xi, ldx), (xo, ldxo) = _pl(noise), _pl(keep), _pl(xin), _pl(xt_out)
    _lib.check(lib.gdmcf_dnn_prep_input_f32(
        x.data_ptr(), x.stride(0), _lib.ptr(ts), _lib.ptr(ca), _lib.ptr(cb), noise_mode, nz, ldn, drop_mode, kp, ldkp, drop_p,
        seed, offset, int(bool(norm)), emb.weight.data_ptr() if emb is not None else None,
        emb.bias.data_ptr() if emb is not None else None, E, B, I, xi, ldx, xo, ldxo, _lib.ptr(temb), _lib.ptr(rownorm), st))
    return x, noise, keep


def prep_input_csr(lib, batch, ts, ca, cb, noise, drop_mask, drop_p, training, seed, offset, emb, E, xin, temb, x0bits, st):
    B, I = batch.shape
    noise_mode, noise, drop_mode, keep = _prep_modes(B, ca, noise, drop_mask, drop_p, training)
    (nz, ldn), (kp, ldkp) = _pl(noise), _pl(keep)
    c = batch.csr
    _lib.check(lib.gdmcf_dnn_prep_input_csr_f32(
        c.indptr.data_ptr(), c.indices.data_ptr(), batch.row_ids.data_ptr(), _lib.ptr(ts), _lib.ptr(ca), _lib.ptr(cb),
        noise_mode, nz, ldn, drop_mode, kp, ldkp, drop_p, seed, offset, emb.weight.data_ptr(), emb.bias.data_ptr(), E, B, I,
        xin.data_ptr(), xin.stride(0), temb.data_ptr(), x0bits.data_ptr(), x0bits.stride(0), st))
    return batch, noise, keep


def onehot_prep_input_csr(lib, batch, ts_U, discrete, sampled, seed, offset_noise, ts, drop_mask, drop_p, training,
                          offset_prep, emb, E, xin, temb, st, sampled_out=None, x0bits=None):
    B, I = batch.shape
    _, _, drop_mode, keep = _prep_modes(B, None, None, drop_mask, drop_p, training)
    (sp, lds), (kp, ldkp), (so, ldso), (xb, ldb) = _pl(sampled), _pl(keep), _pl(sampled_out), _pl(x0bits)
    c = batch.csr
    _lib.check(lib.gdmcf_onehot_prep_input_csr_f32(
        c.indptr.data_ptr(), c.indices.data_ptr(), batch.row_ids.data_ptr(), _lib.ptr(ts_U), float(discrete), sp, lds, seed,
        offset_noise, so, ldso, _lib.ptr(ts), drop_mode, kp, ldkp, drop_p, offset_prep,
        emb.weight.data_ptr() if emb is not None else None, emb.bias.data_ptr() if emb is not None else None, E, B, I,
        xin.data_ptr(), xin.stride(0), _lib.ptr(temb), xb, ldb, st))
    return batch, sampled, keep


def cat_prep_input_csr(lib, batch, ts_U, discrete, sampled, seed, offset_noise, ts, ca, cb, noise, drop_mask, drop_p, training,
                       offset_prep, cat, emb, E, xin, xt, temb, x0bits, clsbits, st):
    B, I = batch.shape
    noise_mode, noise, drop_mode, keep = _prep_modes(B, ca, noise, drop_mask, drop_p, training)
    (sp, lds), (nz, ldn), (kp, ldkp) = _pl(sampled), _pl(noise), _pl(keep)
    c = batch.csr
    _lib.check(lib.gdmcf_cat_prep_input_csr_f32(
        c.indptr.data_ptr(), c.indices.data_ptr(), batch.row_ids.data_ptr(), _lib.ptr(ts_U), float(discrete), sp, lds,
        offset_noise, ts.data_ptr(), _lib.ptr(ca), _lib.ptr(cb), noise_mode, nz, ldn, drop_mode, kp, ldkp, drop_p, seed,
        offset_prep, cat.weight.data_ptr(), cat.bias.data_ptr(), emb.weight.data_ptr(), emb.bias.data_ptr(), E, B, I,
        xin.data_ptr(), xin.stride(0), xt.data_ptr(), xt.stride(0), temb.data_ptr(), x0bits.data_ptr(), x0bits.stride(0),
        clsbits.data_ptr(), clsbits.stride(0), st))
    return batch, noise, keep, drop_mode


def cat_grad_bits(lib, dxin, xt, x0bits, clsbits, drop_mode, keep, drop_p, seed, offset, B, I, ws, ws_bytes, gw, gb, st):
    (kp, ldkp) = _pl(keep)
    _lib.check(lib.gdmcf_cat_grad_bits_f32(
        dxin.data_ptr(), dxin.stride(0), xt.data_ptr(), xt.stride(0), x0bits.data_ptr(), x0bits.stride(0), clsbits.data_ptr(),
        clsbits.stride(0), drop_mode, kp, ldkp, drop_p, seed, offset, B, I, ws.data_ptr(), ws_bytes, gw.data_ptr(), gb.data_ptr(),
        st))


def linear_fwd(lib, bufs, A, W, bias, act, B, N, K, out, st):
    (a, lda), (w, ldw), (o, ldo) = _pl(A), _pl(W), _pl(out)
    _lib.check(lib.gdmcf_linear_fwd_f32(a, lda, w, ldw, _lib.ptr(bias), act, B, N, K, o, ldo, bufs.ws.data_ptr(),
                                        bufs.ws_bytes, st))


def gather_fwd(lib, pre, base, batch, table, I, a, tblE, E, bias, act, B, N, out, st):
    (p, ldp), (tb, ldt), (ap, lda), (te, ldte), (o, ldo) = _pl(pre), _pl(table), _pl(a), _pl(tblE), _pl(out)
    c = batch.csr if batch is not None else None
    if c is None:
        tb, ldt = None, 0
    if E == 0:
        ap, lda, te, ldte = None, 0, None, 0
    _lib.check(lib.gdmcf_gather_fwd_f32(
        p, ldp, _lib.ptr(base), c.indptr.data_ptr() if c is not None else None, c.indices.data_ptr() if c is not None else None,
        batch.row_ids.data_ptr() if c is not None else None, tb, ldt, I, ap, lda, te, ldte, E, _lib.ptr(bias), act, B, N, o, ldo, st))


def latent_step(lib, A, M, v, p_cur, c1, c2, e, act, B, N, K, p_next, h_next, st):
    (a, lda), (m, ldm), (pc, ldpc), (pn, ldpn), (h, ldh) = _pl(A), _pl(M), _pl(p_cur), _pl(p_next), _pl(h_next)
    _lib.check(lib.gdmcf_latent_step_f32(a, lda, m, ldm, _lib.ptr(v), pc, ldpc, c1.data_ptr(), c2.data_ptr(), _lib.ptr(e), act,
                                         B, N, K, pn, ldpn, h, ldh, None, 0, st))


def latent_step_ex(lib, A, M, v, p_cur, c1, c2, r, e, act, B, N, K, p_next, h_next, acc, st):
    (a, lda), (m, ldm), (pc, ldpc), (pn, ldpn), (h, ldh), (rp, ldr) = _pl(A), _pl(M), _pl(p_cur), _pl(p_next), _pl(h_next), _pl(r)
    (qc, ldqc), (qn, ldqn) = (_pl(acc[0]), _pl(acc[3])) if acc is not None else ((None, 0), (None, 0))
    qa, qb = (acc[1].data_ptr(), acc[2].data_ptr()) if acc is not None else (None, None)
    _lib.check(lib.gdmcf_latent_step_ex_f32(a, lda, m, ldm, _lib.ptr(v), pc, ldpc, c1.data_ptr(), c2.data_ptr(), rp, ldr, _lib.ptr(e),
                                            act, B, N, K, pn, ldpn, h, ldh, qc, ldqc, qa, qb, qn, ldqn, None, 0, st))


def latent_acc(lib, q_cur, qa, A, qb, B, K, q_next, st):
    (qc, ldqc), (a, lda), (qn, ldqn) = _pl(q_cur), _pl(A), _pl(q_next)
    _lib.check(lib.gdmcf_latent_acc_f32(qc, ldqc, qa.data_ptr(), a, lda, qb.data_ptr(), B, K, qn, ldqn, st))


def cand_scores(lib, A, W, I, K, bias, scale, cand, ldcand, B, C, mask_ptrs, rows, out, st):
    (a, lda), (w, ldw), (o, ldo) = _pl(A), _pl(W), _pl(out)
    _lib.check(lib.gdmcf_cand_scores_f32(a, lda, w, ldw, I, K, _lib.ptr(bias), _lib.ptr(scale), cand.data_ptr(), ldcand, B, C,
                                         *mask_ptrs, _lib.ptr(rows), o, ldo, st))


def cand_pick(lib, dense, B, I, scale, cand, ldcand, C, mask_ptrs, rows, out, st):
    (d, ldd), (o, ldo) = _pl(dense), _pl(out)
    _lib.check(lib.gdmcf_cand_pick_f32(d, ldd, B, I, _lib.ptr(scale), cand.data_ptr(), ldcand, C, *mask_ptrs, _lib.ptr(rows), o,
                                       ldo, st))


def step_tables(tabs32, T, B, names, cache=None):
    key = (id(tabs32), int(T), int(B))
    rec = cache.get(names) if cache is not None else None
    if rec is None or rec[0] != key:
        rec = (key, {k: tabs32[k][:T, None].expand(T, B).contiguous() for k in names if k in tabs32})
        if cache is not None:
            cache[names] = rec
    return rec[1]


LatentProduct = collections.namedtuple("LatentProduct", "A second K bias scale")


class EpsTables:

    def __init__(self, c1, c2, r1, r2, T):
        import numpy as np
        c1, c2, r1, r2 = (np.asarray(t, dtype=np.float64)[:T] for t in (c1, c2, r1, r2))
        g, d = c1 * r1 + c2, c1 * r2
        G, D = 1.0, 0.0
        with np.errstate(all="ignore"):
            for t in range(T - 1, -1, -1):
                G, D = g[t] * G, g[t] * D + d[t]
            qa, qb = g.copy(), d.copy()
            qa[T - 1] = 0.0
            qa[0], qb[0] = qa[0] / D, qb[0] / D
        self.g, self.d, self.qa, self.qb = (t.astype(np.float32) for t in (g, d, qa, qb))
        self.G, self.D = float(np.float32(G)), float(np.float32(D))
        self.ok = bool(all(np.isfinite(t).all() for t in (self.g, self.d, self.qa, self.qb)) and np.isfinite(self.G)
                       and np.isfinite(self.D) and self.D > 0)
        self._dev = {}

    def on(self, device, B):
        rec, key = self._dev, (str(device), int(B))
        if key not in rec:
            def tab(a):
                return torch.from_numpy(a).to(device)[:, None].expand(len(a), B).contiguous()
            f = dict(dtype=torch.float32, device=device)
            rec[key] = dict(neg_d=tab(-self.d), g=tab(self.g), qa=tab(self.qa), qb=tab(self.qb), G=torch.full((B,), self.G, **f),
                            D=torch.full((B,), self.D, **f), one=torch.ones(B, **f), zero=torch.zeros(B, **f))
            rec[key]["qa0_neg"], rec[key]["qb0_neg"] = -rec[key]["qa"][0], -rec[key]["qb"][0]
        return rec[key]


def linear_bwd_input(lib, bufs, dz, W, rs, A_prev, act_prev, B, N, K, d_prev, st):
    (z, ldz), (w, ldw), (a, lda), (d, ldd) = _pl(dz), _pl(W), _pl(A_prev), _pl(d_prev)
    _lib.check(lib.gdmcf_linear_bwd_input_f32(z, ldz, w, ldw, _lib.ptr(rs), a, lda, act_prev, B, N, K, d, ldd,
                                              bufs.ws.data_ptr(), bufs.ws_bytes, st))


def linear_bwd_weight(lib, dz, A, rs, scol, B, N, K, dW, db, st):
    (z, ldz), (a, lda) = _pl(dz), _pl(A)
    _lib.check(lib.gdmcf_linear_bwd_weight_f32(z, ldz, a, lda, _lib.ptr(rs), scol, B, N, K, dW.data_ptr(), dW.stride(0),
                                               _lib.ptr(db), 0, st))


def adamw_args(fs, w):
    if fs["exp_avg"].stride() != w.stride() or fs["exp_avg_sq"].stride() != w.stride():
        raise RuntimeError("gdmcf_amd: the moments of a fused weight must share its leading dimension")
    return (fs["exp_avg"].data_ptr(), fs["exp_avg_sq"].data_ptr(), fs["lr"], fs["beta1"], fs["beta2"], fs["eps"],
            fs["weight_decay"], fs["step"], fs["grad_scale"])


def dw_adamw_args(dz, A, rs, scol, B, N, K, w, db, fs):
    (z, ldz), (a, lda) = _pl(dz), _pl(A)
    ad = adamw_args(fs, w)
    return (z, ldz, a, lda, _lib.ptr(rs), scol, B, N, K, w.data_ptr(), w.stride(0), ad[0], ad[1], _lib.ptr(db)) + ad[2:]


def linear_bwd_weight_adamw(lib, args, st):
    _lib.check(lib.gdmcf_linear_bwd_weight_adamw_f32(*args, st))


def rowscale(lib, A, rs, B, K, out, st):
    (a, lda), (o, ldo) = _pl(A), _pl(out)
    _lib.check(lib.gdmcf_rowscale_f32(a, lda, rs.data_ptr(), B, K, o, ldo, st))


def emb_bwd(lib, bufs, dz, W, I_cols, E, B, N, dWe, dbe, st):
    (z, ldz), (w, ldw) = _pl(dz), _pl(W)
    _lib.check(lib.gdmcf_emb_bwd_f32(z, ldz, w, ldw, I_cols, E, bufs.temb.data_ptr(), B, N, bufs.demb.data_ptr(),
                                     dWe.data_ptr(), dbe.data_ptr(), st))


def loss_layer(lib, bufs, A, W, bias, target, alpha, B, N, K, st, reduce=True):
    (a, lda), (w, ldw) = _pl(A), _pl(W)
    _lib.check(lib.gdmcf_linear_loss_fwd_f32(a, lda, w, ldw, _lib.ptr(bias), target.data_ptr(), target.stride(0),
                                             _lib.ptr(alpha), B, N, K, None, 0, bufs.diff.data_ptr(), bufs.ldi,
                                             bufs.rowpart.data_ptr(), bufs.rowsum.data_ptr() if reduce else None, st))
    return int(lib.gdmcf_loss_parts_last())


def loss_layer_bits(lib, bufs, A, W, bias, x0bits, alpha, B, N, K, st, reduce=True):
    (a, lda), (w, ldw) = _pl(A), _pl(W)
    _lib.check(lib.gdmcf_linear_loss_fwd_bits_f32(a, lda, w, ldw, _lib.ptr(bias), x0bits.data_ptr(), x0bits.stride(0),
                                                  _lib.ptr(alpha), B, N, K, None, 0, bufs.diff.data_ptr(), bufs.ldi,
                                                  bufs.rowpart.data_ptr(), bufs.rowsum.data_ptr() if reduce else None, st))
    return int(lib.gdmcf_loss_parts_last())


def loss_tail(lib, bufs, spec, B, rowdiv, alpha, st, mean=False):
    ts = spec["ts"]
    loss = torch.empty(B, dtype=torch.float64, device=ts.device)
    args = (bufs.rowsum.data_ptr(), rowdiv.data_ptr(), _lib.ptr(alpha), ts.data_ptr(), spec["weight_t"].data_ptr(),
            spec["pt"].data_ptr(), B, spec["T"], spec["H"], spec["Lt_history"].data_ptr(), spec["Lt_count"].data_ptr(),
            int(spec["update_history"]), bufs.lu.data_ptr(), loss.data_ptr(), bufs.gradcoef.data_ptr())
    if not mean:
        _lib.check(lib.gdmcf_row_loss_finish_f64(*args, st))
        return loss
    loss_mean = torch.empty((), dtype=torch.float64, device=ts.device)
    if getattr(bufs, "rowscale_mean", None) is None:
        bufs.rowscale_mean = torch.zeros(B, dtype=torch.float32, device=ts.device)
    _lib.check(lib.gdmcf_row_loss_finish_mean_f64(*args, loss_mean.data_ptr(), bufs.rowscale_mean.data_ptr(), st))
    return loss, loss_mean


def loss_tail_job(lib, bufs, spec, B, rowdiv, alpha, nt, A, K):
    ts = spec["ts"]
    loss = torch.empty(B, dtype=torch.float64, device=ts.device)
    loss_mean = torch.empty((), dtype=torch.float64, device=ts.device)
    if getattr(bufs, "rowscale_mean", None) is None:
        bufs.rowscale_mean = torch.zeros(B, dtype=torch.float32, device=ts.device)
    (a, lda) = _pl(A)
    job = _lib.GdKnTail(bufs.rowpart.data_ptr(), bufs.rowpart.stride(0), nt, bufs.rowsum.data_ptr(), rowdiv.data_ptr(),
                        _lib.ptr(alpha), ts.data_ptr(), spec["weight_t"].data_ptr(), spec["pt"].data_ptr(), spec["T"], spec["H"],
                        spec["Lt_history"].data_ptr(), spec["Lt_count"].data_ptr(), int(spec["update_history"]),
                        bufs.lu.data_ptr(), loss.data_ptr(), bufs.gradcoef.data_ptr(), loss_mean.data_ptr(),
                        bufs.rowscale_mean.data_ptr(), a, lda, bufs.rowscale_mean.data_ptr(), K, bufs.hs.data_ptr(),
                        bufs.hs.stride(0))
    job.refs = (loss, loss_mean, rowdiv, alpha, ts, spec["weight_t"], spec["pt"], spec["Lt_history"], spec["Lt_count"], A)
    return loss, loss_mean, job


def tail_job_run(lib, job, B, st):
    _lib.check(lib.gdmcf_kn_tail_run(ctypes.byref(job), B, st))


def linear_bwd_input_tail(lib, bufs, dz, W, rs, A_prev, act_prev, B, N, K, d_prev, job, st):
    (z, ldz), (w, ldw), (a, lda), (d, ldd) = _pl(dz), _pl(W), _pl(A_prev), _pl(d_prev)
    _lib.check(lib.gdmcf_linear_bwd_input_tail_f32(z, ldz, w, ldw, _lib.ptr(rs), a, lda, act_prev, B, N, K, d, ldd,
                                                   bufs.ws.data_ptr(), bufs.ws_bytes, ctypes.byref(job), st))


def posterior_fwd(lib, A, W, bias, x_t, c1, c2, r1, r2, sigma, z, B, N, K, x_next, pred, st):
    (a, lda), (w, ldw), (zp, ldz), (pp, ldp) = _pl(A), _pl(W), _pl(z), _pl(pred)
    _lib.check(lib.gdmcf_linear_posterior_fwd_f32(
        a, lda, w, ldw, _lib.ptr(bias), x_t.data_ptr(), x_t.stride(0), c1.data_ptr(), c2.data_ptr(), _lib.ptr(r1),
        _lib.ptr(r2), _lib.ptr(sigma), zp, ldz, B, N, K, x_next.data_ptr(), x_next.stride(0), pp, ldp, st))


class TrainLoss(torch.autograd.Function):

    @staticmethod
    def forward(ctx, eng, spec, *params):
        loss = eng.train_forward(spec)
        ctx.eng, ctx.version = eng, eng.version
        return loss

    @staticmethod
    def backward(ctx, gloss):
        eng = ctx.eng
        if ctx.version != eng.version:
            raise RuntimeError("gdmcf_amd: activations were overwritten by a later forward; "
                               "call backward before the next training_losses/forward")
        return (None, None, *eng.train_backward(gloss))


class EngineBase:
    supports_grad_sink = True

    def __init__(self, model):
        self.model = model
        self.lib = _lib.load()
        self.E = int(model.time_emb_dim)
        self.I = int(model.in_dims[0])
        self.version = 0
        self.seed = int(torch.initial_seed()) & 0xFFFFFFFFFFFFFFFF
        self.offset = 0
        self._bufs = {}
        self._saved = None
        self._wt = {}
        self._latent = None
        self.grad_sink = None
        self.fused_opt = None

    @property
    def gemm_dtype(self):
        return getattr(self.model, "gemm_dtype", "f32")

    def manual_seed(self, seed):
        self.seed = int(seed) & 0xFFFFFFFFFFFFFFFF
        self.offset = 0

    def _check_params(self, layers):
        what = type(self.model).__name__ + " parameters"
        for w, b, _ in layers:
            _lib.require_gpu(w, what)
            if not (w.stride(1) == 1 and w.stride(0) >= w.shape[1] and b.is_contiguous() and w.dtype == torch.float32):
                raise RuntimeError(f"gdmcf_amd: {what} must be float32 with unit column stride")

    def _transposed(self, w):
        rec = self._wt.get(id(w))
        if rec is None or rec[0] is not w or rec[1] != w._version or rec[2].device != w.device:
            n, k = w.shape
            buf = torch.zeros(k, (n + 31) // 32 * 32, dtype=torch.float32, device=w.device)
            buf[:, :n].copy_(w.detach().t())
            rec = self._wt[id(w)] = (w, w._version, buf)
        return rec[2]

    def _emb_table(self, w, bias, I_cols, T, st):
        m, lib, E, h, dev = self.model, self.lib, self.E, w.shape[0], w.device
        f32 = dict(dtype=torch.float32, device=dev)
        e = torch.zeros(T, _ceil64(h), **f32)
        if E == 0:
            e[:, :h].copy_(bias.detach()[None, :].expand(T, h))
            return e, None
        ew, eb = m.emb_layer.weight, m.emb_layer.bias
        xs = torch.zeros(T, _ceil64(4 + E), **f32)
        ts = torch.arange(T, dtype=torch.int64, device=dev)
        temb = torch.zeros(T, E, **f32)
        _lib.check(lib.gdmcf_dnn_emb_cols_f32(ts.data_ptr(), ew.data_ptr(), eb.data_ptr(), E, T, 4, xs.data_ptr(), xs.stride(0),
                                              temb.data_ptr(), st))
        we_t = torch.zeros(E, (h + 3) // 4 * 4, **f32)
        we_t[:, :h].copy_(w.detach()[:, I_cols:I_cols + E].t())
        gather_fwd(lib, None, None, None, None, I_cols, (xs.data_ptr() + 16, xs.stride(0)), we_t, E, bias, 0, T, h, e, st)
        return e, (xs, ts, temb, we_t)

    def _latent_operands(self, w1, bias1, second, K, b_out, T, entering, tables=()):
        lib, st = self.lib, _lib.stream_ptr()
        key = tuple((t.data_ptr(), t._version, str(t.device)) for t in entering) + (int(T), int(K), b_out is None)
        if self._latent is not None and self._latent[0] == key:
            return self._latent[1]
        h, I, dev = w1.shape[0], self.I, w1.device
        f32 = dict(dtype=torch.float32, device=dev)
        o, ws = _Bufs(), _Bufs()
        ws.ws_bytes = int(max(lib.gdmcf_linear_ws_bytes(h, I, K), lib.gdmcf_linear_ws_bytes(1, h, I)))
        ws.ws = torch.empty(max(ws.ws_bytes, 256), dtype=torch.uint8, device=dev)
        w1x = (w1.data_ptr(), w1.stride(0))
        o.M = torch.zeros(h, _ceil64(K), **f32)
        linear_bwd_input(lib, ws, w1x, second, None, None, 0, h, I, K, o.M, st)
        o.v = o.neg_b = None
        if b_out is not None:
            o.v = torch.zeros(h, **f32)
            linear_fwd(lib, ws, (b_out.data_ptr(), I), w1x, None, 0, 1, h, I, (o.v.data_ptr(), h), st)
            o.neg_b = -b_out.detach()
        ones = torch.ones(I, **f32)
        o.S = torch.zeros(h, **f32)
        linear_fwd(lib, ws, (ones.data_ptr(), I), w1x, None, 0, 1, h, I, (o.S.data_ptr(), h), st)
        o.keep_S = ones
        o.e, o.keep = self._emb_table(w1, bias1, I, T, st)
        o.tabs = [self._emb_table(w, b, cols, T, st) for w, b, cols in tables]
        self._latent = (key, o)
        return o

    def _latent_reverse(self, bufs, ops, T, B, K, act, pre, p, hpair, small, e, c1, c2, second, b_out, x_T, stop=False, eps=None,
                        r=None, c1_of=None, before_step=None):
        lib, st, I, dev, h = self.lib, _lib.stream_ptr(), self.I, p.device, ops.M.shape[0]
        s1, s2, Q = c1, c2, None
        if eps is not None:
            et = eps.on(dev, B)
            s1, s2, qa, qb = et["neg_d"], et["g"], et["qa"], et["qb"]
            if getattr(bufs, "lat_q", None) is None:
                bufs.lat_q = torch.zeros(B, _ceil64(K), dtype=torch.float32, device=dev)
            Q = bufs.lat_q
        if c1_of is not None:
            s1 = c1_of(s1)
        plain = r is None and Q is None
        hcur, hnxt = hpair
        gather_fwd(lib, pre, None, None, None, I, None, None, 0, e[T - 1], act, B, h, hcur, st)
        for n, i in enumerate(range(T - 1, -1, -1)):
            if before_step is not None:
                before_step(n, i)
            A = small(n, i, hcur) if small is not None else hcur
            if i == 0:
                break
            if plain:
                latent_step(lib, A, ops.M, ops.v, p, s1[i], s2[i], e[i - 1], act, B, h, K, p, hnxt, st)
            else:
                latent_step_ex(lib, A, ops.M, ops.v, p, s1[i], s2[i], r, e[i - 1], act, B, h, K, p, hnxt,
                               (Q, qa[i], qb[i], Q) if Q is not None else None, st)
            hcur, hnxt = hnxt, hcur
        if eps is not None:
            qa0, qb0 = (et["qa0_neg"], et["qb0_neg"]) if stop else (qa[0], qb[0])
            latent_acc(lib, Q, qa0, A, qb0, B, K, Q, st)
            if stop:
                return LatentProduct(Q, second, K, ops.neg_b, et["D"])
        elif stop:
            return LatentProduct(A, second, K, b_out, c1[0])
        x0 = torch.empty(B, I, dtype=torch.float32, device=dev)
        if eps is not None:
            posterior_fwd(lib, Q, second, b_out, x_T, et["one"], et["zero"], et["G"], et["D"], None, None, B, I, K, x0, None, st)
        else:
            posterior_fwd(lib, A, second, b_out, x_T, c1[0], c2[0], None, None, None, None, B, I, K, x0, None, st)
        return x0

    @with_precision
    def score_product(self, A, second, K, b_out, B, device):
        bufs = self.buffers(B, device)
        if getattr(bufs, "scores", None) is None:
            bufs.scores = torch.empty(B, self.I, dtype=torch.float32, device=device)
        self._grow_workspace(bufs, B, device, [(self.I, K)])
        linear_fwd(self.lib, bufs, A, second, b_out, 0, B, self.I, K, bufs.scores, _lib.stream_ptr())
        return bufs.scores

    def _gather_first_layer(self, bufs, batch, w, bias, act, xin, B, out, st):
        N, I, E = w.shape[0], self.I, self.E
        wt = self._transposed(w)
        emb_cols = (xin.data_ptr() + 4 * I, xin.stride(0))
        gather_fwd(self.lib, None, None, batch, wt, I, emb_cols, (wt.data_ptr() + 4 * I * wt.stride(0), wt.stride(0)), E, bias, act,
                   B, N, out, st)

    def _shared_buffers(self, b, B, device, n_loss, n_first, weights):
        lib, I, E = self.lib, self.I, self.E
        f32 = dict(dtype=torch.float32, device=device)
        b.temb = torch.zeros(B, max(E, 1), **f32)
        b.rownorm = torch.zeros(B, **f32)
        b.ldi = _ceil64(I)
        b.diff = torch.zeros(B, b.ldi, **f32)
        b.xt = None
        b.rowpart = torch.zeros(B, lib.gdmcf_loss_tiles(n_loss), **f32)
        b.rowsum = torch.zeros(B, **f32)
        b.gradcoef = torch.zeros(B, **f32)
        b.rowdiv_mse = torch.full((B,), float(I), **f32)
        b.lu = torch.zeros(B, dtype=torch.float64, device=device)
        b.demb = torch.zeros((B + n_first) * max(E, 1), **f32)
        b.ws_bytes = 0
        b.tab_cache = {}
        self._grow_workspace(b, B, device, [w.shape for w in weights])

    def _grow_workspace(self, b, B, device, shapes):
        ws = max([b.ws_bytes] + [self.lib.gdmcf_linear_ws_bytes(B, n, k) for n, k in shapes])
        if ws > b.ws_bytes or getattr(b, "ws", None) is None:
            b.ws_bytes = int(ws)
            b.ws = torch.empty(max(ws, 256), dtype=torch.uint8, device=device)

    def _prep_input(self, bufs, x, I, xin, ts, ca, cb, noise, drop_mask, training, xt_out=None):
        m = self.model
        self.offset += 1
        return prep_input(self.lib, x, I, ts, ca, cb, noise, drop_mask, float(m.drop.p), training, self.seed, self.offset,
                          m.norm, m.emb_layer, self.E, xin, xt_out, bufs.temb, bufs.rownorm, _lib.stream_ptr())

    def _eps_target(self, bufs, spec, ts, x0, noise):
        B, dev = ts.shape[0], ts.device
        x0 = _f32_rows(x0)
        target = noise if spec.get("noise_owned", False) else torch.empty(B, self.I, dtype=torch.float32, device=dev)
        alpha = torch.empty(B, dtype=torch.float32, device=dev)
        rowdiv = torch.empty(B, dtype=torch.float32, device=dev)
        _lib.check(self.lib.gdmcf_eps_target_f32(
            noise.data_ptr(), noise.stride(0), bufs.xt.data_ptr(), bufs.xt.stride(0), x0.data_ptr(), x0.stride(0), ts.data_ptr(),
            spec["r1_0"].data_ptr(), spec["r2_0"].data_ptr(), int(bool(spec.get("t0_likelihood", True))), B, self.I,
            target.data_ptr(), target.stride(0), alpha.data_ptr(), rowdiv.data_ptr(), _lib.stream_ptr()))
        return target, alpha, rowdiv

    def _rowscale_of(self, bufs, gloss):
        if isinstance(gloss, float):
            return bufs.gradcoef * gloss
        return (gloss.to(torch.float32) * bufs.gradcoef).contiguous()

    def _fused_state(self, w):
        fused = self.fused_opt if self.grad_sink is None else None
        return fused.fused_state(w) if fused is not None else None

    def _row_scaled(self, bufs, B, K, A, rs, scol, st):
        if rs is None:
            return A, scol
        rowscale(self.lib, A, rs, B, K, bufs.hs, st)
        return bufs.hs, int(bufs.hs.stride(0) > K)

    def _weight_grad(self, bufs, B, w, dz, rs, A, scol, dW, db, fs, st, queue=None):
        N, K = w.shape
        if fs is None:
            linear_bwd_weight(self.lib, dz, A, rs, scol, B, N, K, dW, db, st)
            return
        args = dw_adamw_args(dz, A, rs, scol, B, N, K, w, db, fs)
        if queue is not None:
            queue.append((_lib.GdDwAdamw(*args), w))
            return
        linear_bwd_weight_adamw(self.lib, args, st)
        if not (self.gemm_dtype == "bf16" and _lib.shadow_info(w.data_ptr()) is not None):
            torch.autograd.graph.increment_version(w)

    def _input_grad(self, bufs, B, W, N, K, dz, rs, A_prev, act_prev, d_prev, st):
        linear_bwd_input(self.lib, bufs, dz, W, rs, A_prev, act_prev, B, N, K, d_prev, st)
```

include/gdmcf_hip.h:

```cpp
#ifndef GDMCF_HIP_H
#define GDMCF_HIP_H
#include <stddef.h>
#include <stdint.h>

#ifdef __cplusplus
extern "C" {
#endif

#define GDMCF_OK 0
#define GDMCF_E_SHAPE (-1)
#define GDMCF_E_ARG (-2)
#define GDMCF_E_UNSUPPORTED (-3)
#define GDMCF_E_HIP (-4)
#define GDMCF_E_WORKSPACE (-5)

int gdmcf_version(void);
const char* gdmcf_last_error(void);
int gdmcf_device_info(int* n_cu, int* wave_size, char* arch_host, int arch_len);
int gdmcf_debug_last_gemm(void);
int gdmcf_debug_fat_slab_plan(int M, int N, int K, int* nb, int* splits, int* cps);
int gdmcf_debug_dr_tn_plan(int M, int N, int K, int64_t lddz, int64_t lda, int64_t ldw, int bias_col, int fused, int* depth,
                           int* ksp, int* tiles_m, int* tiles_n, int* m_fastest, int* has_bias);

int gdmcf_prof_enable(int on);
int gdmcf_prof_collect(int cap, int* tags_host, float* ms_host, double* work_host);

#define GDMCF_N_TABLES 13
int gdmcf_schedule_build(int kind, double noise_scale, double noise_min, double noise_max, int T,
                         int beta_fixed, double* out_tables_host);

int gdmcf_densify_rows_f32(const int64_t* indptr, const int32_t* indices, const float* values,
                           const int64_t* row_ids, int B, int I, float* out, int64_t ldo, void* stream);

int gdmcf_dnn_prep_input_f32(const float* x, int64_t ldx, const int64_t* ts, const float* ca,
                             const float* cb, int noise_mode, const float* noise, int64_t ldn,
                             int drop_mode, const uint8_t* keep, int64_t ldkeep, float drop_p,
                             uint64_t seed, uint64_t offset, int normalize, const float* emb_w,
                             const float* emb_b, int E, int B, int I, float* xin, int64_t ldxin,
                             float* xt_out, int64_t ldxt, float* temb_out, float* rownorm_ws,
                             void* stream);
int gdmcf_dnn_prep_input_csr_f32(const int64_t* indptr, const int32_t* indices, const int64_t* rows, const int64_t* ts,
                                 const float* ca, const float* cb, int noise_mode, const float* noise, int64_t ldn,
                                 int drop_mode, const uint8_t* keep, int64_t ldkeep, float drop_p, uint64_t seed,
                                 uint64_t offset, const float* emb_w, const float* emb_b, int E, int B, int I, float* xin,
                                 int64_t ldxin, float* temb_out, uint32_t* bits_out, int64_t ldbits, void* stream);

int gdmcf_onehot_noise_f32(const float* x0, int64_t ldx, const int64_t* ts, int B, int I, float discrete,
                           const uint8_t* sampled, int64_t lds, uint64_t seed, uint64_t offset,
                           float* xU, int64_t ldu, uint8_t* sampled_out, int64_t ldso, void* stream);
int gdmcf_onehot_prep_input_csr_f32(const int64_t* indptr, const int32_t* indices, const int64_t* rows, const int64_t* ts_U,
                                    float discrete, const uint8_t* sampled, int64_t lds, uint64_t seed, uint64_t offset_noise,
                                    uint8_t* sampled_out, int64_t ldso, const int64_t* ts, int drop_mode, const uint8_t* keep,
                                    int64_t ldkeep, float drop_p, uint64_t offset_prep, const float* emb_w, const float* emb_b,
                                    int E, int B, int I, float* xin, int64_t ldxin, float* temb_out, uint32_t* bits_out,
                                    int64_t ldbits, void* stream);

int gdmcf_randn_f32(float* out, int64_t ld, int rows, int cols, int stream_id, uint64_t seed, uint64_t offset, void* stream);

int gdmcf_eps_target_f32(const float* noise, int64_t ldn, const float* xt, int64_t ldxt, const float* x0, int64_t ldx0,
                         const int64_t* ts, const float* r1, const float* r2, int t0_likelihood, int B, int I, float* target,
                         int64_t ldt, float* alpha, float* rowdiv, void* stream);

int gdmcf_graph_guided_step_u8(uint8_t* graph, int64_t ldg, const int64_t* ts, int B, int I, float discrete,
                               const uint8_t* sampled_in, int64_t lds, const uint8_t* pick_in, const float* degree_prob,
                               int user_guided, uint64_t seed, uint64_t offset, uint8_t* sampled_out, int64_t ldso,
                               uint8_t* pick_out, void* stream);

int gdmcf_dnn_emb_cols_f32(const int64_t* ts, const float* emb_w, const float* emb_b, int E, int B,
                           int I, float* xin, int64_t ldxin, float* temb_out, void* stream);

enum { GDMCF_GEMM_F32 = 0, GDMCF_GEMM_BF16 = 1, GDMCF_GEMM_F32X3 = 2 };
int gdmcf_gemm_precision(int mode);
int gdmcf_bf16_shadow_set(const float* f32, void* bf16, int64_t rows, int64_t cols, int64_t ld_bf16);
int gdmcf_bf16_shadow_clear(const float* f32 );
void* gdmcf_bf16_shadow_get(const float* f32);
int gdmcf_bf16_shadow_info(const float* f32, void** bf16, int64_t* rows, int64_t* cols, int64_t* ld_bf16);
int gdmcf_bf16_shadow_sync(const float* f32, int64_t ld, void* stream);
size_t gdmcf_linear_ws_bytes(int M, int N, int K);
int gdmcf_linear_fwd_f32(const float* A, int64_t lda, const float* W, int64_t ldw,
                         const float* bias, int act, int M, int N, int K, float* C, int64_t ldc,
                         void* ws, size_t ws_bytes, void* stream);
int gdmcf_linear_fwd_wt_f32(const float* A, int64_t lda, const float* Wt, int64_t ldwt,
                            const float* bias, int act, int M, int N, int K, float* C, int64_t ldc,
                            void* ws, size_t ws_bytes, void* stream);
int gdmcf_gather_fwd_f32(const float* pre, int64_t ldpre, const float* base, const int64_t* indptr, const int32_t* indices,
                         const int64_t* rows, const float* table, int64_t ldt, int I, const float* a, int64_t lda,
                         const float* tblE, int64_t ldte, int E, const float* bias, int act, int B, int N, float* out, int64_t ldo,
                         void* stream);
int gdmcf_latent_step_f32(const float* A, int64_t lda, const float* M, int64_t ldm, const float* v,
                          const float* p_cur, int64_t ldpc, const float* c1, const float* c2, const float* e, int act,
                          int B, int N, int K, float* p_next, int64_t ldpn, float* h_next, int64_t ldh,
                          void* ws, size_t ws_bytes, void* stream);
size_t gdmcf_latent_step_ws_bytes(int B, int N, int K);
int gdmcf_latent_step_ex_f32(const float* A, int64_t lda, const float* M, int64_t ldm, const float* v,
                             const float* p_cur, int64_t ldpc, const float* c1, const float* c2, const float* r, int64_t ldr,
                             const float* e, int act, int B, int N, int K, float* p_next, int64_t ldpn, float* h_next,
                             int64_t ldh, const float* q_cur, int64_t ldqc, const float* qa, const float* qb, float* q_next,
                             int64_t ldqn, void* ws, size_t ws_bytes, void* stream);
int gdmcf_latent_acc_f32(const float* q_cur, int64_t ldqc, const float* qa, const float* A, int64_t lda, const float* qb,
                         int B, int K, float* q_next, int64_t ldqn, void* stream);
int gdmcf_loss_tiles(int N);
int gdmcf_linear_loss_fwd_f32(const float* A, int64_t lda, const float* W, int64_t ldw,
                              const float* bias, const float* target, int64_t ldt,
                              const float* alpha, int M, int N, int K, float* out, int64_t ldo,
                              float* diff, int64_t ldd, float* rowpart, float* rowsum,
                              void* stream);
int gdmcf_linear_loss_fwd_bits_f32(const float* A, int64_t lda, const float* W, int64_t ldw, const float* bias,
                                   const uint32_t* target_bits, int64_t ldbits, const float* alpha, int M, int N, int K,
                                   float* out, int64_t ldo, float* diff, int64_t ldd, float* rowpart, float* rowsum,
                                   void* stream);
int gdmcf_linear_posterior_fwd_f32(const float* A, int64_t lda, const float* W, int64_t ldw,
                                   const float* bias, const float* x_t, int64_t ldxt,
                                   const float* c1, const float* c2, const float* r1,
                                   const float* r2, const float* sigma, const float* z,
                                   int64_t ldz, int M, int N, int K, float* x_next,
                                   int64_t ldxn, float* pred_out, int64_t ldp, void* stream);
int gdmcf_linear_bwd_input_f32(const float* dZ, int64_t lddz, const float* W, int64_t ldw,
                               const float* rowscale, const float* Aact, int64_t ldact, int act,
                               int M, int N, int K, float* dA, int64_t ldda, void* ws,
                               size_t ws_bytes, void* stream);
typedef struct GdKnTail {
    const float* rowpart;
    int ld_rowpart, nt;
    float* rowsum;
    const float* rowdiv;
    const float* alpha;
    const int64_t* ts;
    const double* weight_t;
    const double* pt;
    int T, H;
    double* Lt_history;
    int64_t* Lt_count;
    int update_history;
    double* loss_unscaled;
    double* loss;
    float* gradcoef;
    double* loss_mean;
    float* rowscale_mean;
    const float* A;
    int64_t lda;
    const float* rowscale;
    int Ka;
    float* out;
    int64_t ldo;
} GdKnTail;
int gdmcf_linear_bwd_input_tail_f32(const float* dZ, int64_t lddz, const float* W, int64_t ldw, const float* rowscale,
                                    const float* Aact, int64_t ldact, int act, int M, int N, int K, float* dA, int64_t ldda,
                                    void* ws, size_t ws_bytes, const GdKnTail* tail, void* stream);
int gdmcf_kn_tail_run(const GdKnTail* tail, int M, void* stream);
int gdmcf_loss_parts_last(void);
int gdmcf_debug_kn_tail_rides(int M, int N, int K);
int gdmcf_linear_bwd_weight_f32(const float* dZ, int64_t lddz, const float* A, int64_t lda,
                                const float* rowscale, int a_scale_col, int M, int N, int K,
                                float* dW, int64_t lddw, float* db, int accumulate, void* stream);
int gdmcf_linear_bwd_weight_adamw_f32(const float* dZ, int64_t lddz, const float* A, int64_t lda,
                                      const float* rowscale, int a_scale_col, int M, int N, int K, float* W,
                                      int64_t ldw, float* exp_avg, float* exp_avg_sq, float* db, float lr,
                                      float beta1, float beta2, float eps, float weight_decay, int step,
                                      float grad_scale, void* stream);
typedef struct GdDwAdamw {
    const float* dZ;
    int64_t lddz;
    const float* A;
    int64_t lda;
    const float* rowscale;
    int a_scale_col, M, N, K;
    float* W;
    int64_t ldw;
    float* exp_avg;
    float* exp_avg_sq;
    float* db;
    float lr, beta1, beta2, eps, weight_decay;
    int step;
    float grad_scale;
} GdDwAdamw;
int gdmcf_linear_bwd_weight_adamw_multi_f32(const GdDwAdamw* list, int n, void* stream);
int gdmcf_rowscale_f32(const float* A, int64_t lda, const float* rowscale, int M, int K, float* out,
                       int64_t ldo, void* stream);
int gdmcf_row_norms_f32(const float* X, int64_t ld, int rows, int cols, float* norm, float* inv_norm,
                        void* stream);
int gdmcf_normalize_rows_bwd_f32(const float* dY, int64_t lddy, const float* Y, int64_t ldy,
                                 const float* inv_norm, int rows, int cols, float* dX, int64_t lddx,
                                 void* stream);
int gdmcf_tanh_bwd_f32(const float* dA, int64_t ldd, const float* A, int64_t lda, const float* extra,
                       int64_t lde, const float* scale, int M, int N, float* out, int64_t ldo,
                       void* stream);
int gdmcf_gather_rows_f32(const float* src, int64_t lds, const int64_t* index, int n, int cols, float* dst,
                          int64_t ldd, void* stream);
int gdmcf_scatter_add_rows_f32(const float* src, int64_t lds, const int64_t* index, int n, int cols,
                               float* dst, int64_t ldd, void* stream);
int gdmcf_normalize_rows_bwd_adamw_f32(const float* dY, int64_t lddy, const float* Y, int64_t ldy,
                                       const float* inv_norm, int rows, int cols, float* X, int64_t ldx,
                                       float* exp_avg, float* exp_avg_sq, float lr, float beta1, float beta2,
                                       float eps, float weight_decay, int step, float grad_scale, void* stream);
int gdmcf_scatter_rows_adamw_f32(const float* src, int64_t lds, const int64_t* index, int n, int rows, int cols,
                                 float* W, int64_t ldw, float* exp_avg, float* exp_avg_sq, float lr, float beta1,
                                 float beta2, float eps, float weight_decay, int step, float grad_scale,
                                 void* stream);
int gdmcf_emb_bwd_f32(const float* dZ1, int64_t lddz, const float* W1, int64_t ldw, int I, int E,
                      const float* temb, int M, int N, float* demb_ws, float* dWe, float* dbe,
                      void* stream);

int gdmcf_row_loss_finish_f64(const float* rowsum, const float* rowdiv, const float* alpha,
                              const int64_t* ts, const double* weight_t, const double* pt, int B,
                              int T, int H, double* Lt_history, int64_t* Lt_count,
                              int update_history, double* loss_unscaled, double* loss,
                              float* gradcoef, void* stream);
int gdmcf_row_loss_finish_mean_f64(const float* rowsum, const float* rowdiv, const float* alpha, const int64_t* ts,
                                   const double* weight_t, const double* pt, int B, int T, int H, double* Lt_history,
                                   int64_t* Lt_count, int update_history, double* loss_unscaled, double* loss,
                                   float* gradcoef, double* loss_mean, float* rowscale_mean, void* stream);
int gdmcf_lt_history_update(const int64_t* ts, const double* loss_unscaled, int B, int T, int H,
                            double* Lt_history, int64_t* Lt_count, void* stream);

int gdmcf_dp_pack_f64(const float* const* grads, const int64_t* counts, int n, const int64_t* ts,
                      const double* loss_unscaled, int B, int rank, int world, double* flat,
                      void* stream);
int gdmcf_dp_unpack_f64(const double* flat, float* const* grads, const int64_t* counts, int n, int B,
                        int world, int64_t* ts_all, double* loss_unscaled_all, void* stream);

int gdmcf_sample_timesteps(const double* Lt_history, const int64_t* Lt_count, int T, int H, int B,
                           double uniform_prob, uint64_t seed, uint64_t offset, int64_t* ts,
                           double* pt, double* p_out, void* stream);

int gdmcf_adamw_f32(const int64_t* table, int n_tensors, int total_blocks, float lr, float beta1,
                    float beta2, float eps, float weight_decay, int step, float grad_scale,
                    void* stream);
int gdmcf_adamw_bf16s_f32(const int64_t* table, const int64_t* shadow_table, int n_tensors, int total_blocks, float lr,
                          float beta1, float beta2, float eps, float weight_decay, int step, float grad_scale,
                          void* stream);

int gdmcf_topk_masked_f32(const float* pred, int64_t ldp, int B, int I, const int64_t* mask_indptr,
                          const int32_t* mask_indices, int k, int64_t* idx_out, float* val_out,
                          void* stream);
int gdmcf_topk_masked_rows_f32(const float* pred, int64_t ldp, int B, int I, const int64_t* indptr, const int32_t* indices,
                               const int64_t* indptr2, const int32_t* indices2, const int64_t* rows, const float* scale, int k,
                               int64_t* idx_out, float* val_out, void* stream);
int gdmcf_rank_targets_f32(const float* pred, int64_t ldp, int B, int I, const int64_t* indptr, const int32_t* indices,
                           const int64_t* indptr2, const int32_t* indices2, const int64_t* tgt_indptr, const int32_t* tgt_indices,
                           const int64_t* rows, int G, int32_t* rank_out, int64_t ldr, int32_t* n_live_out, void* stream);

int gdmcf_cand_scores_f32(const float* A, int64_t lda, const float* W, int64_t ldw, int I, int K, const float* bias,
                          const float* scale, const int64_t* cand, int64_t ldcand, int B, int C, const int64_t* indptr,
                          const int32_t* indices, const int64_t* indptr2, const int32_t* indices2, const int64_t* rows, float* out,
                          int64_t ldo, void* stream);
int gdmcf_cand_pick_f32(const float* dense, int64_t ldd, int B, int I, const float* scale, const int64_t* cand, int64_t ldcand,
                        int C, const int64_t* indptr, const int32_t* indices, const int64_t* indptr2, const int32_t* indices2,
                        const int64_t* rows, float* out, int64_t ldo, void* stream);

size_t gdmcf_score_topk_ws_bytes(int n_rows, int n_items, int d, int k);
int gdmcf_score_topk_f32(const float* user_emb, int64_t ldu, const int64_t* user_ids, int n_rows, const float* item_emb,
                         int64_t ldi, int n_items, int d, const int64_t* mask_indptr, const int32_t* mask_indices, int k,
                         int64_t* out_idx, float* out_val, void* ws, size_t ws_bytes, void* stream);

int gdmcf_debug_score_rank_plan(int n_rows, int n_items, int G, int* tile_rows, int* pass_targets, int* passes, int* slabs);
size_t gdmcf_score_rank_ws_bytes(int n_rows, int n_items, int d, int G);
int gdmcf_score_rank_f32(const float* user_emb, int64_t ldu, const int64_t* user_ids, int n_rows, const float* item_emb,
                         int64_t ldi, int n_items, int d, const int64_t* mask_indptr, const int32_t* mask_indices,
                         const int64_t* tgt_indptr, const int32_t* tgt_indices, int G, int32_t* rank_out, int64_t ldr,
                         int32_t* n_live_out, void* ws, size_t ws_bytes, void* stream);

int gdmcf_topn_metrics_f64(const int64_t* pred_idx, int64_t ldp, int U, const int64_t* gt_indptr, const int32_t* gt_indices,
                           const int* topN_host, int n_topn, double* out, void* stream);
int gdmcf_rank_metrics_f64(const int32_t* ranks, int64_t ldr, int U, int G, const int* topN_host, int n_topn, double* out,
                           void* stream);

int gdmcf_spmm_csr_f32(const int64_t* vbeg, const int64_t* vend, const int32_t* vrow, const int32_t* vslot,
                       int n_virtual, int n_short, const int32_t* lrow, const int32_t* lptr, int n_long, const int32_t* col,
                       const float* val, int n_rows, const float* X, int64_t ldx, int d, float* Y,
                       int64_t ldy, float* partial_ws, const float* const* addends_host, int n_add,
                       int64_t ld_add, float scale, double alg_bytes, void* stream);
int gdmcf_spmm_bundled_f32(const int32_t* wdesc, int n_waves, const int64_t* lbeg, const int32_t* llen, const int32_t* lrow,
                           const int32_t* lslot, int n_pieces, const int64_t* sbeg, const int32_t* slen, const int32_t* srow,
                           const int32_t* smax, int n_bundles, const int32_t* crow, const int32_t* cptr, int n_cut,
                           const int32_t* col, const float* val, int64_t nnz, int n_rows, int n_x_rows, const float* X,
                           int64_t ldx, int d, float* Y, int64_t ldy, float* partial_ws, const float* const* addends_host, int n_add, int64_t ld_add,
                           float scale, double alg_bytes, void* stream);
int gdmcf_spmm_stream_f32(const int32_t* wdesc, int n_waves, const int32_t* cw, int64_t n_entries, const int32_t* ud, int n_units,
                          const int32_t* crow, const int32_t* cptr, int n_cut, int n_rows, int n_x_rows, const float* X,
                          int64_t ldx, int d, float* Y, int64_t ldy, float* partial_ws, const float* const* addends_host,
                          int n_add, int64_t ld_add, float scale, double alg_bytes, void* stream);
int gdmcf_debug_spmm_stamps(int n_waves, long long* host_out);
int gdmcf_graph_state_bytes(void);
int gdmcf_adam_hyper_bytes(void);
int gdmcf_graph_state_init(void* state_host, uint64_t prep_offset, uint64_t ts_offset, int64_t adam_step, int64_t table_first,
                           int64_t table_len, const void* hyper_table_dev);
int gdmcf_adam_hyper_fill(void* out_host, int n, float lr, float beta1, float beta2, float eps, float weight_decay,
                          int64_t first_step, float grad_scale);
int gdmcf_graph_state_bind(const void* state_dev);
int gdmcf_graph_state_tick(void* state_dev, void* stream);
int gdmcf_scale_f32(const float* acc, int64_t n, float scale, float* out, void* stream);

int gdmcf_bpr_sample_f32(const int64_t* indptr, const int32_t* indices, const int64_t* users, int B, int n_users, int n_items,
                         uint64_t seed, uint64_t offset, int64_t* pos, int64_t* neg, int32_t* flag, void* stream);
int gdmcf_bpr_sample_pool_f32(const int64_t* indptr, const int32_t* indices, const int64_t* users, int B, int n_negs, int pool,
                              int n_users, int n_items, const float* M, int64_t ldm, int d, uint64_t seed, uint64_t offset,
                              int64_t* pos, int64_t* neg, int32_t* flag, void* stream);
int gdmcf_bpr_loss_f32(const float* M, int64_t ldm, const float* E0, int64_t lde, int d, const int64_t* users, const int64_t* pos,
                       const int64_t* neg, int B, int n_users, int n_items, float* coef, float* ws, float* mf, float* reg,
                       int32_t* flag, void* stream);
int gdmcf_bpr_grad_f32(int mode, const int32_t* order, const int64_t* users, const int64_t* pos, const int64_t* neg, int B,
                       int n_users, int n_items, const float* coef, const float* src, int64_t ld_src, int d, float* out,
                       int64_t ld_out, float scale, float* zero_rows, int64_t ld_zero, void* stream);

int gdmcf_cat_prep_input_f32(const float* x, int64_t ldx, const float* xU, int64_t ldu, const int64_t* ts, const float* ca,
                             const float* cb, int noise_mode, const float* noise, int64_t ldn, int drop_mode, const uint8_t* keep,
                             int64_t ldkeep, float drop_p, uint64_t seed, uint64_t offset, const float* cat_w, const float* cat_b,
                             const float* emb_w, const float* emb_b, int E, int B, int I, float* xin, int64_t ldxin, float* xt_out,
                             int64_t ldxt, float* temb_out, void* stream);
size_t gdmcf_cat_grad_ws_bytes(int B, int I);
int gdmcf_cat_grad_f32(const float* dxin, int64_t lddx, const float* xt, int64_t ldxt, const float* xU, int64_t ldu, int drop_mode,
                       const uint8_t* keep, int64_t ldkeep, float drop_p, uint64_t seed, uint64_t offset, int B, int I, void* ws,
                       size_t ws_bytes, float* grad_w, float* grad_b, void* stream);
int gdmcf_cat_prep_input_csr_f32(const int64_t* indptr, const int32_t* indices, const int64_t* rows, const int64_t* ts_U,
                                 float discrete, const uint8_t* sampled, int64_t lds, uint64_t offset_noise, const int64_t* ts,
                                 const float* ca, const float* cb, int noise_mode, const float* noise, int64_t ldn, int drop_mode,
                                 const uint8_t* keep, int64_t ldkeep, float drop_p, uint64_t seed, uint64_t offset_prep,
                                 const float* cat_w, const float* cat_b, const float* emb_w, const float* emb_b, int E, int B, int I,
                                 float* xin, int64_t ldxin, float* xt_out, int64_t ldxt, float* temb_out, uint32_t* x0bits_out,
                                 int64_t ldx0bits, uint32_t* clsbits_out, int64_t ldclsbits, void* stream);
int gdmcf_cat_grad_bits_f32(const float* dxin, int64_t lddx, const float* xt, int64_t ldxt, const uint32_t* x0bits, int64_t ldx0bits,
                            const uint32_t* clsbits, int64_t ldclsbits, int drop_mode, const uint8_t* keep, int64_t ldkeep,
                            float drop_p, uint64_t seed, uint64_t offset, int B, int I, void* ws, size_t ws_bytes, float* grad_w,
                            float* grad_b, void* stream);

size_t gdmcf_ntxent_ws_bytes(int B);
int gdmcf_ntxent_fwd_f32(const float* z1, int64_t ld1, const float* z2, int64_t ld2, int B, int d, float temperature, float eps,
                         void* ws, size_t ws_bytes, float* loss_out, void* stream);
int gdmcf_ntxent_bwd_f32(const float* z1, int64_t ld1, const float* z2, int64_t ld2, int B, int d, const void* ws, size_t ws_bytes,
                         const float* scale, float* dz1, int64_t lddz1, float* dz2, int64_t lddz2, void* stream);

#ifdef __cplusplus
}
#endif
#endif
```

Baseline: 332,100 users/s.

## Fuse embedding weight gather and demb reduction into the backward input-grad GEMM path

Moves the gather of W1's embedding columns into an idle workgroup of the persistent KN split-K GEMM, next to the existing tail job. It also computes the per-row embedding gradient (demb) inside the split-K reduce kernel while the reduced row is still in shared memory. emb_bwd is then told these pieces are already done and can skip its own gather and demb kernels. The aim is to cut separate kernel launches and a re-read of dA. The cost is more complex control flow, extra register and LDS pressure in the reduce kernel, and fallbacks when no idle workgroup is free.

```diff
diff --git a/gdmcf_amd/_lib.py b/gdmcf_amd/_lib.py
--- a/gdmcf_amd/_lib.py
+++ b/gdmcf_amd/_lib.py
@@ -100,6 +100,10 @@
     _fields_ = parse_structs(_HEADER)["GdKnTail"]
 
 
+class GdKnGather(ctypes.Structure):
+    _fields_ = parse_structs(_HEADER)["GdKnGather"]
+
+
 _lib = None
 
 
diff --git a/gdmcf_amd/csrc/gemm_dr_kn.hip b/gdmcf_amd/csrc/gemm_dr_kn.hip
--- a/gdmcf_amd/csrc/gemm_dr_kn.hip
+++ b/gdmcf_amd/csrc/gemm_dr_kn.hip
@@ -9,7 +9,7 @@
 #define GD_KN_EVERY 4
 #endif
 template <int NL>
-__global__ __launch_bounds__(256, 1) void dr_kn_kernel(const DrArgs d, const GdTailJob job) {
+__global__ __launch_bounds__(256, 1) void dr_kn_kernel(const DrArgs d, const GdTailJob job, const GdGatherJob gat) {
     constexpr int TMB = 5;
     const GdGemm& g = d.g;
     const int lane = threadIdx.x & 63;
@@ -23,9 +23,13 @@
     const int CPS = d.ksp;
     const int total_chunks = (g.K + 15) >> 4;
     const int ntasks = ntiles * g.splits;
-    if (job.on && slot == (ntasks + 3) >> 2) {
-        extern __shared__ __attribute__((aligned(16))) unsigned char kn_lds[];
-        gd_tail_job_run(job, kn_lds);
+    if (job.on && slot >= (ntasks + 3) >> 2) {
+        if (slot == (ntasks + 3) >> 2) {
+            extern __shared__ __attribute__((aligned(16))) unsigned char kn_lds[];
+            gd_tail_job_run(job, kn_lds);
+        } else if (gat.on && slot == ((ntasks + 3) >> 2) + 1) {
+            gd_emb_gather_w(gat.W1, gat.ldw, gat.I, gat.E, gat.N, gat.W1e, 0, 1);
+        }
         return;
     }
     const __amdgpu_buffer_rsrc_t srdA = __builtin_amdgcn_make_buffer_rsrc(const_cast<float*>(g.A), 0, (int)(((int64_t)(g.M - 1) * g.lda + g.K) * 4), 0x00020000);
@@ -144,11 +148,19 @@
 
 static bool kn_idle_workgroup(int ntasks, int n_cu) { return gd_cdiv(ntasks, 4) < n_cu; }
 
+#ifndef GD_KN_GATHER_DEFAULT
+#define GD_KN_GATHER_DEFAULT 1
+#endif
+static bool kn_gather_on() {
+    const char* env = getenv("GDMCF_KN_GATHER");
+    return env ? atoi(env) != 0 : GD_KN_GATHER_DEFAULT != 0;
+}
+
 #ifndef GD_KN_TAIL_DEFAULT
 #define GD_KN_TAIL_DEFAULT 1
 #endif
 
-static int kn_launch(GdGemm& g, const GdTailJob* job, hipStream_t s) {
+static int kn_launch(GdGemm& g, const GdTailJob* job, const GdGatherJob* gat, hipStream_t s) {
     if (!dr_routes().kn) return GD_DR_NOT_TAKEN;
     const int splits = gd_dr_kn_splits(g.M, g.N, g.K);
     const size_t need = (size_t)splits * g.M * g.ldc * sizeof(float);
@@ -165,6 +177,7 @@
     d.tiles_n = gd_cdiv(g.N, 128);
     d.ksp = cps;
     GdTailJob none = {};
+    GdGatherJob no_gather = {};
     size_t lds = 0;
     if (job) {
         const char* env = getenv("GDMCF_KN_TAIL");
@@ -173,6 +186,7 @@
         if (!tail_on || !job->on || !kn_idle_workgroup(d.tiles_m * d.tiles_n * real_splits, n_cu) || lds > GD_LT_LDS_MAX)
             return GD_DR_NOT_TAKEN;
         static bool attr_set = false;
+        if (gat && (!gat->on || !kn_gather_on() || gd_cdiv(d.tiles_m * d.tiles_n * real_splits, 4) + 1 >= n_cu)) return GD_DR_NOT_TAKEN;
         if (!gd_allow_big_lds(dr_kn_kernel<2>, lds, &attr_set, "gemm_dr_kn")) return GDMCF_E_HIP;
     }
     g.splits = real_splits;
@@ -182,14 +196,26 @@
     d.g = g;
     {
         GdProfScope prof(g.prof_tag, 2.0 * g.M * g.N * g.K, s);
-        hipLaunchKernelGGL((dr_kn_kernel<2>), dim3(n_cu), dim3(256), lds, s, d, job ? *job : none);
+        hipLaunchKernelGGL((dr_kn_kernel<2>), dim3(n_cu), dim3(256), lds, s, d, job ? *job : none, gat ? *gat : no_gather);
     }
     t_gd_last_gemm = 5;
     return gd_launch_status("gemm_dr_kn");
 }
 
-int gd_dr_kn_launch(GdGemm& g, hipStream_t s) { return kn_launch(g, nullptr, s); }
-int gd_dr_kn_launch_tail(GdGemm& g, const GdTailJob& job, hipStream_t s) { return kn_launch(g, &job, s); }
+int gd_dr_kn_launch(GdGemm& g, hipStream_t s) { return kn_launch(g, nullptr, nullptr, s); }
+int gd_dr_kn_launch_tail(GdGemm& g, const GdTailJob& job, hipStream_t s) { return kn_launch(g, &job, nullptr, s); }
+int gd_dr_kn_launch_tail_gather(GdGemm& g, const GdTailJob& job, const GdGatherJob& gat, hipStream_t s) { return kn_launch(g, &job, &gat, s); }
+
+int gdmcf_debug_kn_idle_workgroups(int M, int N, int K) {
+    const int splits = gd_dr_kn_splits(M, N, K);
+    if (splits <= 0) return 0;
+    const int total_chunks = gd_cdiv(K, 16);
+    const int cps = (gd_cdiv(total_chunks, splits) + 1) & ~1;
+    const int idle = dr_cu_count() - gd_cdiv(gd_cdiv(M, 80) * gd_cdiv(N, 128) * gd_cdiv(total_chunks, cps), 4);
+    return idle > 0 ? idle : 0;
+}
+
+bool gd_dr_kn_gather_rides(int M, int N, int K) { return kn_gather_on() && gdmcf_debug_kn_idle_workgroups(M, N, K) >= 2; }
 
 int gdmcf_debug_kn_tail_rides(int M, int N, int K) {
     const int splits = gd_dr_kn_splits(M, N, K);
diff --git a/gdmcf_amd/csrc/linear.hip b/gdmcf_amd/csrc/linear.hip
--- a/gdmcf_amd/csrc/linear.hip
+++ b/gdmcf_amd/csrc/linear.hip
@@ -323,9 +323,9 @@
     return gdmcf_rowscale_f32(t.A, t.lda, t.rowscale, M, t.Ka, t.out, t.ldo, stream);
 }
 
-int gdmcf_linear_bwd_input_tail_f32(const float* dZ, int64_t lddz, const float* W, int64_t ldw, const float* rowscale,
-                                    const float* Aact, int64_t ldact, int act, int M, int N, int K, float* dA, int64_t ldda,
-                                    void* ws, size_t ws_bytes, const GdKnTail* tail, void* stream) {
+static int bwd_input_tail(const float* dZ, int64_t lddz, const float* W, int64_t ldw, const float* rowscale, const float* Aact,
+                          int64_t ldact, int act, int M, int N, int K, float* dA, int64_t ldda, void* ws, size_t ws_bytes,
+                          const GdKnTail* tail, const GdKnGather* gat, void* stream) {
     GD_CHECK_SHAPE(M > 0 && N > 0 && K > 0 && lddz >= N && ldw >= K && ldda >= K, "linear_bwd_input_tail: bad shape");
     GD_CHECK_ARG(act == 0 || (act == 1 && Aact && ldact >= K), "linear_bwd_input_tail: activation output missing");
     GD_CHECK_ARG(tail != nullptr, "linear_bwd_input_tail: tail missing");
@@ -339,6 +339,11 @@
     GD_CHECK_ARG(lt_lds_bytes(t.T, t.H, M) <= GD_LT_LDS_MAX, "linear_bwd_input_tail: T*H and B too large for the LDS-resident FIFO update (150 KiB)");
     hipStream_t s = (hipStream_t)stream;
     const int64_t lds_ = round4(K);
+    bool gathered = gat == nullptr;
+    if (gat) {
+        GD_CHECK_SHAPE(gat->N == K && gat->E > 0 && gat->I >= 0 && gat->ldw >= gat->I + gat->E, "linear_bwd_input_tail_gather: bad gather shape");
+        GD_CHECK_ARG(gat->W1 && gat->W1e, "linear_bwd_input_tail_gather: null pointer");
+    }
     if (t_gemm_prec == GDMCF_GEMM_F32 && ws != nullptr) {
         GdGemm g = {};
         g.A = dZ; g.lda = lddz; g.B = W; g.ldb = ldw; g.M = M; g.N = K; g.K = N;
@@ -354,16 +359,53 @@
         j.loss = t.loss; j.loss_mean = t.loss_mean; j.rowscale_mean = t.rowscale_mean; j.inv_b = 1.0f / (float)M;
         j.K = t.Ka; j.A = t.A; j.lda = t.lda; j.rs = t.rowscale; j.out = t.out; j.ldo = t.ldo;
         j.out16 = has16 ? (unsigned short*)sh.p16 : nullptr; j.ldo16 = has16 ? sh.ld16 : 0; j.bias_col = t.ldo > t.Ka;
-        const int rc = gd_dr_kn_launch_tail(g, j, s);
+        int rc = GD_DR_NOT_TAKEN;
+        if (gat && gd_dr_kn_gather_rides(M, K, N)) {
+            const GdGatherJob gj = {1, gat->I, gat->E, gat->N, gat->W1, gat->ldw, gat->W1e};
+            rc = gd_dr_kn_launch_tail_gather(g, j, gj, s);
+            gathered = rc == GDMCF_OK;
+        }
+        if (rc == GD_DR_NOT_TAKEN) {
+            if (!gathered) {
+                rc = gd_emb_gather_w_launch(gat->W1, gat->ldw, gat->I, gat->E, gat->N, gat->W1e, s);
+                if (rc) return rc;
+                gathered = true;
+            }
+            rc = gd_dr_kn_launch_tail(g, j, s);
+        }
         if (rc != GD_DR_NOT_TAKEN) {
             if (rc) return rc;
-            return gd_splitk_reduce((const float*)ws, g.slab_stride, gd_cdiv(N, g.kchunk), lds_, M, K, 1, nullptr, rowscale, Aact, ldact,
-                                    act, dA, ldda, s);
-        }
-    }
-    const int rc = gdmcf_kn_tail_run(tail, M, stream);
-    if (rc) return rc;
-    return gdmcf_linear_bwd_input_f32(dZ, lddz, W, ldw, rowscale, Aact, ldact, act, M, N, K, dA, ldda, ws, ws_bytes, stream);
+            if (gat && gat->demb) {
+                rc = gd_splitk_reduce_demb((const float*)ws, g.slab_stride, gd_cdiv(N, g.kchunk), lds_, M, K, rowscale, Aact, ldact, act, dA,
+                                           ldda, gat->W1e, gat->E, gat->demb, s);
+                if (rc != GD_DR_NOT_TAKEN) return rc;
+            }
+            rc = gd_splitk_reduce((const float*)ws, g.slab_stride, gd_cdiv(N, g.kchunk), lds_, M, K, 1, nullptr, rowscale, Aact, ldact, act,
+                                  dA, ldda, s);
+            if (rc || !gat || !gat->demb) return rc;
+            return gd_emb_demb_launch(dA, ldda, gat->W1e, gat->E, M, K, gat->demb, s);
+        }
+    }
+    int rc = gathered ? GDMCF_OK : gd_emb_gather_w_launch(gat->W1, gat->ldw, gat->I, gat->E, gat->N, gat->W1e, s);
+    if (rc) return rc;
+    rc = gdmcf_kn_tail_run(tail, M, stream);
+    if (rc) return rc;
+    rc = gdmcf_linear_bwd_input_f32(dZ, lddz, W, ldw, rowscale, Aact, ldact, act, M, N, K, dA, ldda, ws, ws_bytes, stream);
+    if (rc || !gat || !gat->demb) return rc;
+    return gd_emb_demb_launch(dA, ldda, gat->W1e, gat->E, M, K, gat->demb, s);
+}
+
+int gdmcf_linear_bwd_input_tail_f32(const float* dZ, int64_t lddz, const float* W, int64_t ldw, const float* rowscale,
+                                    const float* Aact, int64_t ldact, int act, int M, int N, int K, float* dA, int64_t ldda,
+                                    void* ws, size_t ws_bytes, const GdKnTail* tail, void* stream) {
+    return bwd_input_tail(dZ, lddz, W, ldw, rowscale, Aact, ldact, act, M, N, K, dA, ldda, ws, ws_bytes, tail, nullptr, stream);
+}
+
+int gdmcf_linear_bwd_input_tail_gather_f32(const float* dZ, int64_t lddz, const float* W, int64_t ldw, const float* rowscale,
+                                           const float* Aact, int64_t ldact, int act, int M, int N, int K, float* dA, int64_t ldda,
+                                           void* ws, size_t ws_bytes, const GdKnTail* tail, const GdKnGather* gather, void* stream) {
+    GD_CHECK_ARG(gather != nullptr, "linear_bwd_input_tail_gather: gather missing");
+    return bwd_input_tail(dZ, lddz, W, ldw, rowscale, Aact, ldact, act, M, N, K, dA, ldda, ws, ws_bytes, tail, gather, stream);
 }
 
 int gdmcf_linear_bwd_weight_f32(const float* dZ, int64_t lddz, const float* A, int64_t lda, const float* rowscale,
diff --git a/gdmcf_amd/csrc/reduce.hip b/gdmcf_amd/csrc/reduce.hip
--- a/gdmcf_amd/csrc/reduce.hip
+++ b/gdmcf_amd/csrc/reduce.hip
@@ -1,17 +1,25 @@
+#include <stdlib.h>
+
 #include "tail_job.h"
 
 namespace {
 
+template <bool DEMB>
 __global__ __launch_bounds__(256) void splitk_reduce_kernel(const float* __restrict__ slabs, int64_t slab_stride,
                                                             int splits, int64_t ld_slab, int M, int N, int mode,
                                                             const float* __restrict__ bias,
                                                             const float* __restrict__ rowscale,
                                                             const float* __restrict__ aact, int64_t ldact, int act,
                                                             float* __restrict__ out, int64_t ldo,
-                                                            unsigned short* __restrict__ out16, int64_t ldo16, int vec) {
+                                                            unsigned short* __restrict__ out16, int64_t ldo16, int vec,
+                                                            const float* __restrict__ W1e, int E, float* __restrict__ demb) {
     const int m = blockIdx.y;
     const int n0 = (blockIdx.x * 256 + threadIdx.x) * 4;
-    if (n0 >= N) return;
+    if (!DEMB && n0 >= N) return;
+    __shared__ float zrow[DEMB ? 1024 : 1];
+    if (DEMB && n0 >= N) splits = 0;
+    GdDembW dw;
+    if constexpr (DEMB) gd_emb_demb_load(W1e, E, N, 0, threadIdx.x >> 6, dw);
     float sv[4] = {0.f, 0.f, 0.f, 0.f};
     const float* p = slabs + (int64_t)m * ld_slab + n0;
     if (vec && n0 + 3 < N) {
@@ -48,6 +56,13 @@
         }
         out[(int64_t)m * ldo + n] = s;
         if (out16) out16[(int64_t)m * ldo16 + n] = gd_bf16_bits(s);
+        if constexpr (DEMB) zrow[n] = s;
+    }
+    if constexpr (DEMB) {
+        __syncthreads();
+        float ds[4] = {0.f, 0.f, 0.f, 0.f};
+        gd_emb_demb_acc(zrow, N, 0, dw, ds);
+        gd_emb_demb_store(ds, E, threadIdx.x >> 6, demb + (int64_t)m * E);
     }
 }
 
@@ -135,10 +150,29 @@
     GdShadow sh;
     const bool has16 = gd_shadow_lookup(out, &sh) && sh.rows == M && sh.cols == N;
     const int vec = (ld_slab % 4 == 0) && (slab_stride % 4 == 0) && gd_aligned16(slabs);
-    hipLaunchKernelGGL(splitk_reduce_kernel, dim3(gd_cdiv(N, 1024), M), dim3(256), 0, s, slabs, slab_stride,
+    hipLaunchKernelGGL(splitk_reduce_kernel<false>, dim3(gd_cdiv(N, 1024), M), dim3(256), 0, s, slabs, slab_stride,
                        splits, ld_slab, M, N, mode, bias, rowscale, aact, ldact, act, out, ldo,
-                       has16 ? (unsigned short*)sh.p16 : nullptr, has16 ? sh.ld16 : 0, vec);
+                       has16 ? (unsigned short*)sh.p16 : nullptr, has16 ? sh.ld16 : 0, vec, nullptr, 0, nullptr);
     return gd_launch_status("splitk_reduce");
+}
+
+#ifndef GD_RED_DEMB_DEFAULT
+#define GD_RED_DEMB_DEFAULT 1
+#endif
+
+int gd_splitk_reduce_demb(const float* slabs, int64_t slab_stride, int splits, int64_t ld_slab, int M, int N, const float* rowscale,
+                          const float* aact, int64_t ldact, int act, float* out, int64_t ldo, const float* W1e, int E, float* demb,
+                          hipStream_t s) {
+    const char* env = getenv("GDMCF_RED_DEMB");
+    const bool on = env ? atoi(env) != 0 : GD_RED_DEMB_DEFAULT != 0;
+    if (!on || N > 1024 || E < 1 || E > 16 || !W1e || !demb) return GD_DR_NOT_TAKEN;
+    GdShadow sh;
+    const bool has16 = gd_shadow_lookup(out, &sh) && sh.rows == M && sh.cols == N;
+    const int vec = (ld_slab % 4 == 0) && (slab_stride % 4 == 0) && gd_aligned16(slabs);
+    hipLaunchKernelGGL(splitk_reduce_kernel<true>, dim3(1, M), dim3(256), 0, s, slabs, slab_stride, splits, ld_slab, M, N, 1, nullptr,
+                       rowscale, aact, ldact, act, out, ldo, has16 ? (unsigned short*)sh.p16 : nullptr, has16 ? sh.ld16 : 0, vec, W1e,
+                       E, demb);
+    return gd_launch_status("splitk_reduce_demb");
 }
 
 int gd_colsum(const float* dZ, int64_t ld, const float* rs, int M, int N, float* db, hipStream_t s) {
@@ -149,6 +183,20 @@
 int gd_rowpart_reduce(const float* rowpart, int ld, int M, int nt, float* rowsum, hipStream_t s) {
     hipLaunchKernelGGL(rowpart_reduce_kernel, dim3(gd_cdiv(M, 4)), dim3(256), 0, s, rowpart, ld, M, nt, rowsum);
     return gd_launch_status("rowpart_reduce");
+}
+
+extern "C" int gdmcf_debug_splitk_reduce_demb_f32(const float* slabs, int64_t slab_stride, int splits, int64_t ld_slab, int M, int N,
+                                                  const float* rowscale, const float* aact, int64_t ldact, int act, float* out,
+                                                  int64_t ldo, const float* W1e, int E, float* demb, void* stream) {
+    GD_CHECK_SHAPE(M > 0 && N > 0 && splits > 0 && E > 0 && ld_slab >= N && ldo >= N && slab_stride >= (int64_t)(M - 1) * ld_slab + N,
+                   "debug_splitk_reduce_demb: bad shape");
+    GD_CHECK_ARG(slabs && out && W1e && demb && (act == 0 || (act == 1 && aact && ldact >= N)), "debug_splitk_reduce_demb: null pointer");
+    hipStream_t s = (hipStream_t)stream;
+    int rc = gd_splitk_reduce_demb(slabs, slab_stride, splits, ld_slab, M, N, rowscale, aact, ldact, act, out, ldo, W1e, E, demb, s);
+    if (rc != GD_DR_NOT_TAKEN) return rc ? rc : 1;
+    rc = gd_splitk_reduce(slabs, slab_stride, splits, ld_slab, M, N, 1, nullptr, rowscale, aact, ldact, act, out, ldo, s);
+    if (rc) return rc;
+    return gd_emb_demb_launch(out, ldo, W1e, E, M, N, demb, s);
 }
 
 int gd_cast_bf16(const float* src, int64_t ld, void* dst, int64_t ld16, int64_t rows, int64_t cols, hipStream_t s) {
diff --git a/gdmcf_amd/csrc/rows.hip b/gdmcf_amd/csrc/rows.hip
--- a/gdmcf_amd/csrc/rows.hip
+++ b/gdmcf_amd/csrc/rows.hip
@@ -1,4 +1,4 @@
-#include "common.h"
+#include "tail_job.h"
 
 namespace {
 
@@ -182,21 +182,14 @@
 
 __global__ __launch_bounds__(256) void emb_gather_w_kernel(const float* __restrict__ W1, int64_t ldw, int I, int E, int N,
                                                            float* __restrict__ W1e) {
-    const int idx = blockIdx.x * 256 + threadIdx.x;
-    if (idx < N * E) W1e[idx] = W1[(int64_t)(idx / E) * ldw + I + (idx % E)];
+    gd_emb_gather_w(W1, ldw, I, E, N, W1e, blockIdx.x, gridDim.x);
 }
 
 __global__ __launch_bounds__(256) void emb_bwd_demb_kernel(const float* __restrict__ dZ1, int64_t lddz,
                                                            const float* __restrict__ W1e, int E, int N,
                                                            float* __restrict__ demb) {
     const int m = blockIdx.x;
-    const int lane = threadIdx.x & 63, wave = threadIdx.x >> 6;
-    for (int e = wave; e < E; e += 4) {
-        float s = 0.f;
-        for (int n = lane; n < N; n += 64) s += dZ1[(int64_t)m * lddz + n] * W1e[(int64_t)n * E + e];
-        for (int o = 32; o > 0; o >>= 1) s += __shfl_xor(s, o);
-        if (lane == 0) demb[(int64_t)m * E + e] = s;
-    }
+    gd_emb_demb_row(dZ1 + (int64_t)m * lddz, W1e, E, N, demb + (int64_t)m * E);
 }
 
 __global__ __launch_bounds__(64) void emb_bwd_w_kernel(const float* __restrict__ demb, const float* __restrict__ temb,
@@ -322,12 +315,18 @@
 
 int gdmcf_emb_bwd_f32(const float* dZ1, int64_t lddz, const float* W1, int64_t ldw, int I, int E, const float* temb,
                       int M, int N, float* demb_ws, float* dWe, float* dbe, void* stream) {
+    return gdmcf_emb_bwd_from_f32(dZ1, lddz, W1, ldw, I, E, temb, M, N, demb_ws, dWe, dbe, 0, stream);
+}
+
+int gdmcf_emb_bwd_from_f32(const float* dZ1, int64_t lddz, const float* W1, int64_t ldw, int I, int E, const float* temb,
+                           int M, int N, float* demb_ws, float* dWe, float* dbe, int have, void* stream) {
     GD_CHECK_SHAPE(M > 0 && N > 0 && E > 0 && I >= 0 && ldw >= I + E && lddz >= N, "emb_bwd: bad shape");
     GD_CHECK_ARG(dZ1 && W1 && temb && demb_ws && dWe && dbe, "emb_bwd: null pointer");
+    GD_CHECK_ARG(have >= 0 && have <= 2, "emb_bwd: have must be 0, 1 or 2");
     hipStream_t s = (hipStream_t)stream;
     float* W1e = demb_ws + (size_t)M * E;
-    hipLaunchKernelGGL(emb_gather_w_kernel, dim3(gd_cdiv(N * E, 256)), dim3(256), 0, s, W1, ldw, I, E, N, W1e);
-    hipLaunchKernelGGL(emb_bwd_demb_kernel, dim3(M), dim3(256), 0, s, dZ1, lddz, W1e, E, N, demb_ws);
+    if (have < 1) hipLaunchKernelGGL(emb_gather_w_kernel, dim3(gd_cdiv(N * E, 256)), dim3(256), 0, s, W1, ldw, I, E, N, W1e);
+    if (have < 2) hipLaunchKernelGGL(emb_bwd_demb_kernel, dim3(M), dim3(256), 0, s, dZ1, lddz, W1e, E, N, demb_ws);
     hipLaunchKernelGGL(emb_bwd_w_kernel, dim3(E * E + E), dim3(64), 0, s, demb_ws, temb, M, E, dWe, dbe);
     return gd_launch_status("emb_bwd");
 }
@@ -350,3 +349,13 @@
 }
 
 }
+
+int gd_emb_gather_w_launch(const float* W1, int64_t ldw, int I, int E, int N, float* W1e, hipStream_t s) {
+    hipLaunchKernelGGL(emb_gather_w_kernel, dim3(gd_cdiv(N * E, 256)), dim3(256), 0, s, W1, ldw, I, E, N, W1e);
+    return gd_launch_status("emb_gather_w");
+}
+
+int gd_emb_demb_launch(const float* dZ1, int64_t lddz, const float* W1e, int E, int M, int N, float* demb, hipStream_t s) {
+    hipLaunchKernelGGL(emb_bwd_demb_kernel, dim3(M), dim3(256), 0, s, dZ1, lddz, W1e, E, N, demb);
+    return gd_launch_status("emb_bwd_demb");
+}
diff --git a/gdmcf_amd/csrc/tail_job.h b/gdmcf_amd/csrc/tail_job.h
--- a/gdmcf_amd/csrc/tail_job.h
+++ b/gdmcf_amd/csrc/tail_job.h
@@ -63,6 +63,56 @@
                         if (k + j < K) out16[(int64_t)m * ldo16 + k + j] = gd_bf16_bits(v[j]);
             }
         }
+    }
+}
+
+__device__ __forceinline__ void gd_emb_gather_w(const float* __restrict__ W1, int64_t ldw, int I, int E, int N,
+                                                float* __restrict__ W1e, int blk, int nblk) {
+    for (int idx = blk * 256 + (int)threadIdx.x; idx < N * E; idx += nblk * 256) W1e[idx] = W1[(int64_t)(idx / E) * ldw + I + (idx % E)];
+}
+
+struct GdDembW {
+    float w[4][16];
+};
+__device__ __forceinline__ void gd_emb_demb_load(const float* __restrict__ W1e, int E, int N, int nb, int e0, GdDembW& x) {
+    const int lane = threadIdx.x & 63;
+#pragma unroll
+    for (int k = 0; k < 4; ++k)
+#pragma unroll
+        for (int u = 0; u < 16; ++u) {
+            const int n = nb + lane + 64 * u, e = e0 + 4 * k;
+            x.w[k][u] = (n < N && e < E) ? W1e[(int64_t)n * E + e] : 0.f;
+        }
+}
+__device__ __forceinline__ void gd_emb_demb_acc(const float* __restrict__ z, int N, int nb, const GdDembW& x, float (&s)[4]) {
+    const int lane = threadIdx.x & 63;
+    float zv[16];
+#pragma unroll
+    for (int u = 0; u < 16; ++u) zv[u] = nb + lane + 64 * u < N ? z[nb + lane + 64 * u] : 0.f;
+#pragma unroll
+    for (int u = 0; u < 16; ++u)
+        if (nb + lane + 64 * u < N) {
+#pragma unroll
+            for (int k = 0; k < 4; ++k) s[k] += zv[u] * x.w[k][u];
+        }
+}
+__device__ __forceinline__ void gd_emb_demb_store(float (&s)[4], int E, int e0, float* __restrict__ demb) {
+#pragma unroll
+    for (int k = 0; k < 4; ++k) {
+        for (int o = 32; o > 0; o >>= 1) s[k] += __shfl_xor(s[k], o);
+        if ((threadIdx.x & 63) == 0 && e0 + 4 * k < E) demb[e0 + 4 * k] = s[k];
+    }
+}
+__device__ __forceinline__ void gd_emb_demb_row(const float* __restrict__ z, const float* __restrict__ W1e, int E, int N,
+                                                float* __restrict__ demb) {
+    for (int e0 = threadIdx.x >> 6; e0 < E; e0 += 16) {
+        float s[4] = {0.f, 0.f, 0.f, 0.f};
+        for (int nb = 0; nb < N; nb += 1024) {
+            GdDembW x;
+            gd_emb_demb_load(W1e, E, N, nb, e0, x);
+            gd_emb_demb_acc(z, N, nb, x, s);
+        }
+        gd_emb_demb_store(s, E, e0, demb);
     }
 }
 
@@ -188,3 +238,20 @@
 }
 
 int gd_dr_kn_launch_tail(GdGemm& g, const GdTailJob& job, hipStream_t s);
+
+struct GdGatherJob {
+    int on;
+    int I, E, N;
+    const float* W1;
+    int64_t ldw;
+    float* W1e;
+};
+
+int gd_dr_kn_launch_tail_gather(GdGemm& g, const GdTailJob& job, const GdGatherJob& gat, hipStream_t s);
+bool gd_dr_kn_gather_rides(int M, int N, int K);
+
+int gd_splitk_reduce_demb(const float* slabs, int64_t slab_stride, int splits, int64_t ld_slab, int M, int N, const float* rowscale,
+                          const float* aact, int64_t ldact, int act, float* out, int64_t ldo, const float* W1e, int E, float* demb,
+                          hipStream_t s);
+int gd_emb_gather_w_launch(const float* W1, int64_t ldw, int I, int E, int N, float* W1e, hipStream_t s);
+int gd_emb_demb_launch(const float* dZ1, int64_t lddz, const float* W1e, int E, int M, int N, float* demb, hipStream_t s);
diff --git a/gdmcf_amd/engine.py b/gdmcf_amd/engine.py
--- a/gdmcf_amd/engine.py
+++ b/gdmcf_amd/engine.py
@@ -267,19 +267,22 @@
         dz, rs = dz_last, rowscale
         dw_queue = [] if (fused is not None and self.gemm_dtype == "f32" and os.environ.get("GDMCF_DW_MULTI", "1") != "0") else None
 
+        emb_have = 2 if (tail is not None and L == 2 and self.E > 0) else 0
+
         def input_grad(li, w, A_prev):
             nonlocal dWe, dbe
             N, K = w.shape
             if li > 0:
                 dprev = bufs.dzs[li - 1]
                 if tail is not None and li == L - 1:
-                    core.linear_bwd_input_tail(lib, bufs, dz, w, rs, A_prev, layers[li - 1][2], B, N, K, dprev, tail, st)
+                    core.linear_bwd_input_tail(lib, bufs, dz, w, rs, A_prev, layers[li - 1][2], B, N, K, dprev, tail, st,
+                                               gather=(layers[0][0], self.I, self.E) if emb_have else None)
                 else:
                     self._input_grad(bufs, B, w, N, K, dz, rs, A_prev, layers[li - 1][2], dprev, st)
                 return dprev
             dWe = self._grad_like(m.emb_layer.weight)
             dbe = self._grad_like(m.emb_layer.bias)
-            core.emb_bwd(lib, bufs, dz, w, self.I, self.E, B, N, dWe, dbe, st)
+            core.emb_bwd(lib, bufs, dz, w, self.I, self.E, B, N, dWe, dbe, st, have=emb_have)
             return None
 
         def weight_grad(li, w, bias, A_prev):
diff --git a/gdmcf_amd/engine_core.py b/gdmcf_amd/engine_core.py
--- a/gdmcf_amd/engine_core.py
+++ b/gdmcf_amd/engine_core.py
@@ -244,10 +244,10 @@
     _lib.check(lib.gdmcf_rowscale_f32(a, lda, rs.data_ptr(), B, K, o, ldo, st))
 
 
-def emb_bwd(lib, bufs, dz, W, I_cols, E, B, N, dWe, dbe, st):
+def emb_bwd(lib, bufs, dz, W, I_cols, E, B, N, dWe, dbe, st, have=0):
     (z, ldz), (w, ldw) = _pl(dz), _pl(W)
-    _lib.check(lib.gdmcf_emb_bwd_f32(z, ldz, w, ldw, I_cols, E, bufs.temb.data_ptr(), B, N, bufs.demb.data_ptr(),
-                                     dWe.data_ptr(), dbe.data_ptr(), st))
+    _lib.check(lib.gdmcf_emb_bwd_from_f32(z, ldz, w, ldw, I_cols, E, bufs.temb.data_ptr(), B, N, bufs.demb.data_ptr(),
+                                          dWe.data_ptr(), dbe.data_ptr(), have, st))
 
 
 def loss_layer(lib, bufs, A, W, bias, target, alpha, B, N, K, st, reduce=True):
@@ -303,10 +303,16 @@
     _lib.check(lib.gdmcf_kn_tail_run(ctypes.byref(job), B, st))
 
 
-def linear_bwd_input_tail(lib, bufs, dz, W, rs, A_prev, act_prev, B, N, K, d_prev, job, st):
+def linear_bwd_input_tail(lib, bufs, dz, W, rs, A_prev, act_prev, B, N, K, d_prev, job, st, gather=None):
     (z, ldz), (w, ldw), (a, lda), (d, ldd) = _pl(dz), _pl(W), _pl(A_prev), _pl(d_prev)
-    _lib.check(lib.gdmcf_linear_bwd_input_tail_f32(z, ldz, w, ldw, _lib.ptr(rs), a, lda, act_prev, B, N, K, d, ldd,
-                                                   bufs.ws.data_ptr(), bufs.ws_bytes, ctypes.byref(job), st))
+    args = (z, ldz, w, ldw, _lib.ptr(rs), a, lda, act_prev, B, N, K, d, ldd, bufs.ws.data_ptr(), bufs.ws_bytes, ctypes.byref(job))
+    if gather is None:
+        _lib.check(lib.gdmcf_linear_bwd_input_tail_f32(*args, st))
+        return
+    W1, I_cols, E = gather
+    (w1, ldw1), demb = _pl(W1), bufs.demb.data_ptr()
+    req = _lib.GdKnGather(w1, ldw1, I_cols, E, W1.shape[0], demb + 4 * B * E, demb)
+    _lib.check(lib.gdmcf_linear_bwd_input_tail_gather_f32(*args, ctypes.byref(req), st))
 
 
 def posterior_fwd(lib, A, W, bias, x_t, c1, c2, r1, r2, sigma, z, B, N, K, x_next, pred, st):
diff --git a/include/gdmcf_hip.h b/include/gdmcf_hip.h
--- a/include/gdmcf_hip.h
+++ b/include/gdmcf_hip.h
@@ -150,6 +150,21 @@
 int gdmcf_kn_tail_run(const GdKnTail* tail, int M, void* stream);
 int gdmcf_loss_parts_last(void);
 int gdmcf_debug_kn_tail_rides(int M, int N, int K);
+int gdmcf_debug_kn_idle_workgroups(int M, int N, int K);
+typedef struct GdKnGather {
+    const float* W1;
+    int64_t ldw;
+    int I, E, N;
+    float* W1e;
+    float* demb;
+} GdKnGather;
+int gdmcf_linear_bwd_input_tail_gather_f32(const float* dZ, int64_t lddz, const float* W, int64_t ldw, const float* rowscale,
+                                           const float* Aact, int64_t ldact, int act, int M, int N, int K, float* dA,
+                                           int64_t ldda, void* ws, size_t ws_bytes, const GdKnTail* tail,
+                                           const GdKnGather* gather, void* stream);
+int gdmcf_debug_splitk_reduce_demb_f32(const float* slabs, int64_t slab_stride, int splits, int64_t ld_slab, int M, int N,
+                                       const float* rowscale, const float* aact, int64_t ldact, int act, float* out,
+                                       int64_t ldo, const float* W1e, int E, float* demb, void* stream);
 int gdmcf_linear_bwd_weight_f32(const float* dZ, int64_t lddz, const float* A, int64_t lda,
                                 const float* rowscale, int a_scale_col, int M, int N, int K,
                                 float* dW, int64_t lddw, float* db, int accumulate, void* stream);
@@ -200,6 +215,9 @@
 int gdmcf_emb_bwd_f32(const float* dZ1, int64_t lddz, const float* W1, int64_t ldw, int I, int E,
                       const float* temb, int M, int N, float* demb_ws, float* dWe, float* dbe,
                       void* stream);
+int gdmcf_emb_bwd_from_f32(const float* dZ1, int64_t lddz, const float* W1, int64_t ldw, int I, int E,
+                           const float* temb, int M, int N, float* demb_ws, float* dWe, float* dbe, int have,
+                           void* stream);
 
 int gdmcf_row_loss_finish_f64(const float* rowsum, const float* rowdiv, const float* alpha,
                               const int64_t* ts, const double* weight_t, const double* pt, int B,
```

Measured after the change: 328,800 users/s. -1.0%, worse.
